# BraveGroup/DCD

Hardware: AMD Instinct MI355X
Metric: images/sec DGDE train step (bs=8, 384x1280) (higher is better)
Workload: dtype f32; 1 GPU; DGDE train bs=8 fp32 on 1xMI355X, synthetic KITTI 384x1280 + random kpts_ann (DGDE.yaml, DLA-34+DCNv2, 6 objects/image); global_batch=8, per_gpu_batch=8, input=384x1280, parallelism=dp1, dcn_precision=f32, step_launch=eager, sync_bn=False

## Files before the change

dcd_amd/_ext.py:

```python
import torch

from . import _lib

import threading

PRECISION = {"f32": 0, "bf16x3": 1, "bf16": 2}
_default_precision = "f32"
_scoped = threading.local()


def set_precision(name):
    global _default_precision
    if name not in PRECISION:
        raise ValueError("precision must be one of %s" % sorted(PRECISION))
    _default_precision = name


def get_precision():
    return getattr(_scoped, "name", None) or _default_precision


class precision_scope:

    def __init__(self, name):
        if name is not None and name not in PRECISION:
            raise ValueError("precision must be one of %s" % sorted(PRECISION))
        self.name = name

    def __enter__(self):
        self.saved = getattr(_scoped, "name", None)
        if self.name is not None:
            _scoped.name = self.name
        return self

    def __exit__(self, *exc):
        _scoped.name = self.saved
        return False


HANDOVER = {"never": 0, "always": 1, "auto": 2, None: -1}


def set_handover(mode):
    if mode not in HANDOVER:
        raise ValueError("handover mode must be one of 'never', 'always', 'auto', None")
    _lib.check(_lib.lib().dcd_dcn_v2_set_handover(HANDOVER[mode]), "dcd_dcn_v2_set_handover")


def _check(input, weight, bias, offset, mask, kernel_h, kernel_w):
    _lib.require_cuda(input, weight, bias, offset, mask)
    for name, t in (("input", input), ("weight", weight), ("bias", bias), ("offset", offset), ("mask", mask)):
        if t.dtype != torch.float32:
            raise RuntimeError("%s must be float32 (the op is fp32-only, like the reference)" % name)
    if input.dim() != 4 or weight.dim() != 4:
        raise RuntimeError("input and weight must be 4-D")
    if weight.shape[2] != kernel_h or weight.shape[3] != kernel_w:
        raise RuntimeError("Input shape and kernel shape wont match: (%d x %d vs %d x %d)." % (
            kernel_h, kernel_w, weight.shape[2], weight.shape[3]))
    if input.shape[1] != weight.shape[1]:
        raise RuntimeError("Input shape and kernel channels wont match: (%d vs %d)." % (input.shape[1], weight.shape[1]))
    if bias.numel() != weight.shape[0]:
        raise RuntimeError("bias must have Cout elements")


def _dims(input, weight, kernel_h, kernel_w, stride_h, stride_w, pad_h, pad_w, dilation_h, dilation_w):
    B, C, H, W = input.shape
    Ho = (H + 2 * pad_h - (dilation_h * (kernel_h - 1) + 1)) // stride_h + 1
    Wo = (W + 2 * pad_w - (dilation_w * (kernel_w - 1) + 1)) // stride_w + 1
    return B, C, H, W, weight.shape[0], Ho, Wo


def _workspace(L, input, geom):
    nbytes = L.dcd_dcn_v2_workspace_bytes(*geom)
    if nbytes == 0:
        raise RuntimeError("dcn_v2: unsupported geometry %s" % (geom,))
    return torch.empty(nbytes, dtype=torch.uint8, device=input.device), nbytes


def dcn_v2_forward(input, weight, bias, offset, mask, kernel_h, kernel_w, stride_h, stride_w,
                   pad_h, pad_w, dilation_h, dilation_w, deformable_group, precision=None):
    _check(input, weight, bias, offset, mask, kernel_h, kernel_w)
    L = _lib.lib()
    B, C, H, W, Co, Ho, Wo = _dims(input, weight, kernel_h, kernel_w, stride_h, stride_w, pad_h, pad_w,
                                   dilation_h, dilation_w)
    if tuple(offset.shape) != (B, 2 * deformable_group * kernel_h * kernel_w, Ho, Wo):
        raise RuntimeError("offset shape %s does not match (B, 2*dg*kh*kw, Ho, Wo)" % (tuple(offset.shape),))
    if tuple(mask.shape) != (B, deformable_group * kernel_h * kernel_w, Ho, Wo):
        raise RuntimeError("mask shape %s does not match (B, dg*kh*kw, Ho, Wo)" % (tuple(mask.shape),))
    input, weight, bias, offset, mask = (t.contiguous() for t in (input, weight, bias, offset, mask))
    geom = (B, C, H, W, Co, kernel_h, kernel_w, stride_h, stride_w, pad_h, pad_w, dilation_h, dilation_w,
            deformable_group)
    ws, nbytes = _workspace(L, input, geom)
    output = torch.empty((B, Co, Ho, Wo), dtype=torch.float32, device=input.device)
    prec = PRECISION[precision or get_precision()]
    st = L.dcd_dcn_v2_forward(_lib.stream_of(input), input.data_ptr(), weight.data_ptr(), bias.data_ptr(),
                              offset.data_ptr(), mask.data_ptr(), output.data_ptr(), *geom, prec,
                              ws.data_ptr(), nbytes)
    _lib.check(st, "dcd_dcn_v2_forward")
    return output


def dcn_v2_backward(input, weight, bias, offset, mask, grad_output, kernel_h, kernel_w, stride_h, stride_w,
                    pad_h, pad_w, dilation_h, dilation_w, deformable_group, precision=None):
    _check(input, weight, bias, offset, mask, kernel_h, kernel_w)
    _lib.require_cuda(grad_output)
    if not input.is_contiguous():
        raise RuntimeError("input tensor has to be contiguous")
    if not weight.is_contiguous():
        raise RuntimeError("weight tensor has to be contiguous")
    L = _lib.lib()
    B, C, H, W, Co, Ho, Wo = _dims(input, weight, kernel_h, kernel_w, stride_h, stride_w, pad_h, pad_w,
                                   dilation_h, dilation_w)
    if tuple(grad_output.shape) != (B, Co, Ho, Wo):
        raise RuntimeError("grad_output shape %s does not match the output" % (tuple(grad_output.shape),))
    if grad_output.dtype != torch.float32:
        raise RuntimeError("grad_output must be float32")
    bias, offset, mask, grad_output = (t.contiguous() for t in (bias, offset, mask, grad_output))
    geom = (B, C, H, W, Co, kernel_h, kernel_w, stride_h, stride_w, pad_h, pad_w, dilation_h, dilation_w,
            deformable_group)
    ws, nbytes = _workspace(L, input, geom)
    grad_input = torch.empty_like(input)
    grad_offset = torch.empty_like(offset)
    grad_mask = torch.empty_like(mask)
    grad_weight = torch.empty_like(weight)
    grad_bias = torch.empty_like(bias)
    prec = PRECISION[precision or get_precision()]
    st = L.dcd_dcn_v2_backward(_lib.stream_of(input), input.data_ptr(), weight.data_ptr(), bias.data_ptr(),
                               offset.data_ptr(), mask.data_ptr(), grad_output.data_ptr(),
                               grad_input.data_ptr(), grad_offset.data_ptr(), grad_mask.data_ptr(),
                               grad_weight.data_ptr(), grad_bias.data_ptr(), *geom, prec, ws.data_ptr(), nbytes)
    _lib.check(st, "dcd_dcn_v2_backward")
    return [grad_input, grad_offset, grad_mask, grad_weight, grad_bias]
```

dcd_amd/_lib.py:

```python
import ctypes
import os

_HERE = os.path.dirname(os.path.abspath(__file__))
LIB_PATH = os.path.join(_HERE, "libdcd_hip.so")
_LIB = None

c_void_p, c_int, c_float, c_size_t, c_int64, c_double = (ctypes.c_void_p, ctypes.c_int, ctypes.c_float,
                                                         ctypes.c_size_t, ctypes.c_int64, ctypes.c_double)


class LossRowsArgs(ctypes.Structure):
    _INTS = ("B", "M", "C", "K", "NP", "num_classes", "ch_box2d", "ch_offset", "ch_corner", "ch_corner_unc", "ch_dims",
             "ch_ori_cls", "ch_ori_off", "ch_depth", "ch_depth_unc", "ch_kpts2d", "ch_kpts3d", "trunc_log")
    _FLOATS = ("depth_lo", "depth_hi", "unc_lo", "unc_hi", "depth_weight")
    _POINTERS = ("pois", "reg_mask", "trunc_mask", "find_pcl", "ori_mask", "cls_ids", "centers", "pad_size", "bboxes",
                 "locations", "rotys", "offset_3D", "dimensions", "orientations", "keypoints", "kp_depth_mask", "kpts2d",
                 "kpts3d", "calib_P", "calib", "dim_mean", "kps_pred", "kps_tgt", "kps3d_pred", "kps3d_tgt", "rot", "P_rows",
                 "kmask", "pair_depth", "pair_mask", "cols", "corners_pred", "corners_tgt", "iou3d", "sums", "grad_sums",
                 "grad_pois", "grad_pair", "grad_kps", "grad_kps3d")
    _fields_ = ([(n, c_int) for n in _INTS] + [(n, c_float) for n in _FLOATS] + [("dim_weight", c_float * 3)]
                + [("down_ratio", c_float), ("kd_eps", c_float)] + [(n, c_void_p) for n in _POINTERS])

HEADS_MAX = 16


class HeadRowsArgs(ctypes.Structure):
    _fields_ = ([(n, c_int) for n in ("n_heads", "T", "R", "K", "C")]
                + [(n, c_int * HEADS_MAX) for n in ("trunk", "ch0", "out")]
                + [("weight", c_void_p * HEADS_MAX), ("bias", c_void_p * HEADS_MAX), ("feat", c_void_p), ("y", c_void_p),
                   ("grad_y", c_void_p), ("grad_feat", c_void_p), ("grad_weight", c_void_p * HEADS_MAX),
                   ("grad_bias", c_void_p * HEADS_MAX)])


class EvalMatchArgs(ctypes.Structure):
    _INTS = ("mode", "n_img", "n_comb", "n_rows", "G", "D", "n_dc", "max_dt", "T", "n_slots")
    _POINTERS = ("gt_off", "dt_off", "dc_off", "pair_off", "overlaps", "ign_gt", "ign_dt", "dt_score", "gt_alpha", "dt_alpha",
                 "dt_box2d", "dc_box", "comb", "min_overlap", "thresholds", "n_thresh", "scores", "counts", "sim_part")
    _fields_ = [(n, c_int) for n in _INTS] + [("P", c_int64)] + [(n, c_void_p) for n in _POINTERS]


DECODE_MAX_CLASSES = 8


class DecodeArgs(ctypes.Structure):
    _INTS = ("B", "K", "C", "nk", "n_bins", "num_classes", "ch_box2d", "ch_offset", "ch_corner", "ch_corner_unc", "ch_dims",
             "ch_ori_cls", "ch_ori_off", "ch_depth", "ch_depth_unc", "ch_kpts2d", "ch_kpts3d", "orientation", "dim_mode",
             "dim_std_on", "depth_mode", "uncertainty_as_conf", "records")
    _FLOATS = ("down_ratio", "depth_lo", "depth_hi", "eps")
    _fields_ = ([(n, c_int) for n in _INTS] + [(n, c_float) for n in _FLOATS] + [("depth_ref", c_float * 2)]
                + [("dim_mean", c_float * 3 * DECODE_MAX_CLASSES), ("dim_std", c_float * 3 * DECODE_MAX_CLASSES)])


class RecordsArgs(ctypes.Structure):
    _INTS = ("B", "M", "C", "nk", "n_bins", "ch_offset", "ch_ori_cls", "ch_ori_off", "ch_kpts2d", "ch_kpts3d")
    _fields_ = [(n, c_int) for n in _INTS] + [("down_ratio", c_float)]


SIGNATURES = {
    "dcd_version": (ctypes.c_char_p, []),
    "dcd_dcn_v2_workspace_bytes": (c_size_t, [c_int] * 14),
    "dcd_dcn_v2_forward": (c_int, [c_void_p] * 7 + [c_int] * 15 + [c_void_p, c_size_t]),
    "dcd_dcn_v2_backward": (c_int, [c_void_p] * 12 + [c_int] * 15 + [c_void_p, c_size_t]),
    "dcd_dcn_v2_forget": (c_int, [c_void_p]),
    "dcd_dcn_v2_policy_state": (c_int, [c_void_p, c_void_p]),
    "dcd_dcn_v2_policy_free": (c_int, []),
    "dcd_dcn_v2_set_handover": (c_int, [c_int]),
    "dcd_edge_depth_forward": (c_int, [c_void_p] * 6 + [c_int, c_int, c_int, c_float, c_float, c_int, c_int]
                               + [c_void_p] * 3),
    "dcd_edge_depth_backward": (c_int, [c_void_p] * 7 + [c_int, c_int, c_int, c_float, c_float, c_int]
                                + [c_void_p] * 2),
    "dcd_focal_loss": (c_int, [c_void_p, c_void_p, c_void_p, c_int64, c_float, c_float, c_void_p, c_void_p]),
    "dcd_giou_loss": (c_int, [c_void_p, c_void_p, c_void_p, c_int, c_void_p, c_void_p, c_void_p]),
    "dcd_nms_hm": (c_int, [c_void_p, c_void_p, c_int, c_int, c_int, c_int, c_void_p]),
    "dcd_heatmap_topk": (c_int, [c_void_p, c_void_p] + [c_int] * 6 + [c_void_p] * 5 + [c_void_p, c_size_t]),
    "dcd_heatmap_topk_workspace_bytes": (c_size_t, [c_int] * 5),
    "dcd_poi_gather": (c_int, [c_void_p, c_void_p, c_void_p] + [c_int] * 5 + [c_void_p]),
    "dcd_poi_scatter_add": (c_int, [c_void_p, c_void_p, c_void_p] + [c_int] * 5 + [c_void_p]),
    "dcd_patch_scatter_add": (c_int, [c_void_p, c_void_p, c_void_p, c_int, c_int, c_int64, c_int, c_int, c_void_p]),
    "dcd_iou3d": (c_int, [c_void_p, c_void_p, c_void_p, c_int, c_void_p]),
    "dcd_conv3x3_workspace_bytes": (c_size_t, [c_int] * 5),
    "dcd_conv3x3": (c_int, [c_void_p] * 6 + [c_int] * 6 + [c_void_p, c_size_t]),
    "dcd_conv3x3_weights_bytes": (c_size_t, [c_int] * 3),
    "dcd_conv3x3_transform_weights": (c_int, [c_void_p, c_void_p, c_int, c_int, c_void_p, c_void_p]),
    "dcd_conv3x3_transform_weights_table": (c_int, [c_void_p, c_void_p, c_int]),
    "dcd_conv3x3_prepared": (c_int, [c_void_p] * 6 + [c_int] * 6 + [c_void_p, c_size_t]),
    "dcd_conv3x3_split_weights_bytes": (c_size_t, [c_int] * 3),
    "dcd_conv3x3_split_transform_weights": (c_int, [c_void_p, c_void_p, c_int, c_int, c_void_p, c_void_p]),
    "dcd_conv3x3_split_transform_weights_table": (c_int, [c_void_p, c_void_p, c_int]),
    "dcd_conv3x3_split_workspace_bytes": (c_size_t, [c_int] * 5),
    "dcd_conv3x3_split_prepared": (c_int, [c_void_p] * 6 + [c_int] * 7 + [c_void_p, c_size_t]),
    "dcd_conv1x1_bf16": (c_int, [c_void_p, c_void_p, c_int, c_int, c_int, c_void_p, c_void_p, c_void_p, c_int, c_int, c_int64]),
    "dcd_conv1x1_wrw_bf16_workspace_bytes": (c_size_t, [c_int, c_int, c_int, c_int64]),
    "dcd_conv1x1_wrw_bf16": (c_int, [c_void_p, c_void_p, c_void_p, c_void_p, c_int, c_int, c_int, c_int, c_int64, c_void_p, c_size_t]),
    "dcd_conv3x3_s2_f32": (c_int, [c_void_p, c_void_p, c_void_p, c_void_p, c_int, c_int, c_int, c_int, c_int]),
    "dcd_conv3x3_s2_f32_backward_data": (c_int, [c_void_p, c_void_p, c_void_p, c_void_p, c_int, c_int, c_int, c_int, c_int]),
    "dcd_conv3x3_s2_f32_wrw_workspace_bytes": (c_size_t, [c_int, c_int, c_int, c_int, c_int]),
    "dcd_conv3x3_s2_f32_wrw": (c_int, [c_void_p, c_void_p, c_void_p, c_void_p, c_int, c_int, c_int, c_int, c_int, c_void_p, c_size_t]),
    "dcd_clip_adamw_workspace_bytes": (c_size_t, [c_int, c_void_p]),
    "dcd_clip_grad_norm_scalars": (c_int, [c_void_p, c_int, c_void_p, c_void_p, c_float, c_void_p, c_size_t, c_void_p]),
    "dcd_adamw_apply": (c_int, [c_void_p, c_int] + [c_void_p] * 7 + [c_double] * 4 + [c_void_p]),
    "dcd_conv1x1_f32": (c_int, [c_void_p, c_void_p, c_int, c_int, c_int, c_void_p, c_void_p, c_void_p, c_int, c_int, c_int64]),
    "dcd_conv1x1_wrw_f32_workspace_bytes": (c_size_t, [c_int, c_int, c_int, c_int64]),
    "dcd_conv1x1_wrw_f32": (c_int, [c_void_p, c_void_p, c_void_p, c_void_p, c_int, c_int, c_int, c_int, c_int64, c_void_p, c_size_t]),
    "dcd_conv3x3_bf16_weights_bytes": (c_size_t, [c_int] * 3),
    "dcd_conv3x3_bf16_transform_weights": (c_int, [c_void_p, c_void_p, c_int, c_int, c_void_p, c_void_p]),
    "dcd_conv3x3_bf16_transform_weights_table": (c_int, [c_void_p, c_void_p, c_int]),
    "dcd_conv3x3_bf16_workspace_bytes": (c_size_t, [c_int] * 5),
    "dcd_conv3x3_bf16_prepared": (c_int, [c_void_p] * 6 + [c_int] * 6 + [c_void_p, c_size_t]),
    "dcd_conv_stem_workspace_bytes": (c_size_t, [c_int] * 3),
    "dcd_conv_stem": (c_int, [c_void_p] * 4 + [c_int] * 7 + [c_void_p, c_size_t]),
    "dcd_conv_stem_wrw_workspace_bytes": (c_size_t, [c_int] * 3),
    "dcd_conv_stem_wrw": (c_int, [c_void_p] * 4 + [c_int] * 6 + [c_void_p, c_size_t]),
    "dcd_context_norm_forward": (c_int, [c_void_p] * 4 + [c_int, c_int, c_float]),
    "dcd_context_norm_backward": (c_int, [c_void_p] * 5 + [c_int, c_int]),
    "dcd_context_norm_relu_add_forward": (c_int, [c_void_p] * 4 + [c_int, c_int, c_float]),
    "dcd_gmw_refine": (c_int, [c_void_p] * 5 + [c_int, c_void_p, c_void_p, c_int, c_int, c_int] + [c_void_p] * 3),
    "dcd_gmw_pack_records": (c_int, [c_void_p] * 4 + [c_int, c_int, c_void_p, c_int, c_int, c_int] + [c_void_p] * 9),
    "dcd_sum_tensors": (c_int, [c_void_p, c_void_p, c_int, c_void_p, c_int64]),
    "dcd_conv3x3_wrw_workspace_bytes": (c_size_t, [c_int] * 5),
    "dcd_conv3x3_wrw": (c_int, [c_void_p] * 4 + [c_int] * 6 + [c_void_p, c_size_t]),
    "dcd_upsample_dw_forward": (c_int, [c_void_p] * 4 + [c_int] * 5),
    "dcd_upsample_dw_forward_add": (c_int, [c_void_p] * 5 + [c_int] * 5),
    "dcd_maxpool2x2_forward": (c_int, [c_void_p, c_void_p, c_void_p, c_int64, c_int, c_int]),
    "dcd_maxpool2x2_backward": (c_int, [c_void_p, c_void_p, c_void_p, c_void_p, c_int64, c_int, c_int]),
    "dcd_upsample_dw_backward": (c_int, [c_void_p] * 6 + [c_int] * 5),
    "dcd_bn_workspace_bytes": (c_size_t, [c_int]),
    "dcd_bn_stats": (c_int, [c_void_p, c_void_p, c_int, c_int, c_int64, c_void_p, c_void_p, c_size_t]),
    "dcd_channel_sums": (c_int, [c_void_p, c_void_p, c_int, c_int, c_int64, c_void_p, c_void_p, c_size_t]),
    "dcd_bn_train_apply": (c_int, [c_void_p] * 6 + [c_double] + [c_void_p] * 3 + [c_float, c_float, c_int] + [c_void_p] * 3
                           + [c_int, c_int, c_int64]),
    "dcd_bn_eval_apply": (c_int, [c_void_p] * 7 + [c_float, c_int, c_void_p, c_int, c_int, c_int64]),
    "dcd_bn_backward_stats": (c_int, [c_void_p] * 5 + [c_int, c_int, c_int64, c_void_p, c_void_p, c_size_t]),
    "dcd_trunk_row_sums": (c_int, [c_void_p, c_void_p, c_void_p, c_int, c_int, c_void_p]),
    "dcd_trunk_finalize_forward": (c_int, [c_void_p, c_void_p, c_void_p, c_void_p, c_double, c_double, c_int, c_void_p, c_void_p, c_void_p]),
    "dcd_trunk_finalize_backward": (c_int, [c_void_p, c_void_p, c_void_p, c_void_p, c_void_p, c_double, c_int, c_void_p, c_void_p, c_void_p]),
    "dcd_trunk_grad_wg": (c_int, [c_void_p, c_void_p, c_void_p, c_int, c_int, c_void_p]),
    "dcd_bn_backward_relu_from_x": (c_int, [c_void_p] * 10 + [c_int, c_int, c_int64, c_void_p, c_size_t]),
    "dcd_bn_backward_stats_params_relu_from_x": (c_int, [c_void_p] * 7 + [c_int, c_int, c_int64, c_void_p, c_void_p, c_void_p, c_void_p, c_size_t]),
    "dcd_bn_backward_apply_relu_from_x": (c_int, [c_void_p] * 8 + [c_double, c_void_p, c_int, c_int, c_int64]),
    "dcd_bn_backward_stats_params": (c_int, [c_void_p] * 6 + [c_int, c_int, c_int64, c_void_p, c_void_p, c_void_p, c_void_p, c_size_t]),
    "dcd_bn_backward_apply": (c_int, [c_void_p] * 8 + [c_double] + [c_void_p] * 4 + [c_int, c_int, c_int64]),
    "dcd_bn_at_forward": (c_int, [c_void_p] * 6 + [c_double] + [c_void_p] * 3 + [c_float, c_float, c_int] + [c_void_p] * 4
                          + [c_int, c_int, c_int64, c_int] + [c_void_p, c_size_t]),
    "dcd_bn_at_backward_sums": (c_int, [c_void_p] * 7 + [c_int, c_int, c_int] + [c_void_p, c_void_p]),
    "dcd_bn_train_forward": (c_int, [c_void_p] * 8 + [c_float, c_float, c_int] + [c_void_p] * 3 + [c_int, c_int, c_int64]
                             + [c_void_p, c_size_t]),
    "dcd_bn_backward": (c_int, [c_void_p] * 11 + [c_int, c_int, c_int64] + [c_void_p, c_size_t]),
    "dcd_dcn_offset_mask_split": (c_int, [c_void_p, c_void_p, c_void_p, c_void_p, c_int, c_int, c_int64]),
    "dcd_dcn_offset_mask_merge": (c_int, [c_void_p, c_void_p, c_void_p, c_void_p, c_void_p, c_int, c_int, c_int64]),
    "dcd_sgemm_shifted": (c_int, [c_void_p, c_void_p, c_int, c_int64, c_void_p, c_void_p, c_int64, c_int, c_void_p, c_void_p, c_int,
                                  c_int64, c_int64, c_int, c_int, c_int, c_int, c_int]),
    "dcd_sgemm": (c_int, [c_void_p, c_void_p, c_int, c_int64, c_int, c_void_p, c_int, c_int64, c_int, c_void_p, c_int, c_int64,
                          c_int, c_int, c_int, c_int, c_float, c_int, c_int]),
    "dcd_spd_solve_workspace_bytes": (c_size_t, [c_int, c_int]),
    "dcd_spd_solve": (c_int, [c_void_p, c_void_p, c_void_p, c_int, c_int, c_int, c_void_p, c_void_p, c_size_t]),
    "dcd_head_rows_forward": (c_int, [c_void_p, ctypes.POINTER(HeadRowsArgs)]),
    "dcd_head_rows_backward": (c_int, [c_void_p, ctypes.POINTER(HeadRowsArgs)]),
    "dcd_loss_rows_prepare": (c_int, [c_void_p, ctypes.POINTER(LossRowsArgs)]),
    "dcd_loss_rows_forward": (c_int, [c_void_p, ctypes.POINTER(LossRowsArgs)]),
    "dcd_loss_rows_backward": (c_int, [c_void_p, ctypes.POINTER(LossRowsArgs)]),
    "dcd_loss_rows_finish": (c_int, [c_void_p, ctypes.POINTER(LossRowsArgs)]),
    "dcd_encode_targets": (c_int, [c_void_p] * 6 + [c_int] * 6 + [c_double] * 3 + [c_int, c_int, c_void_p, c_int]),
    "dcd_preprocess_images": (c_int, [c_void_p, c_void_p, c_int64, c_void_p, c_void_p, c_int, c_int, c_int, c_int, c_void_p]),
    "dcd_eval_overlaps": (c_int, [c_void_p, c_int, c_void_p, c_void_p, c_void_p, c_int, c_int, c_int64] + [c_void_p] * 5),
    "dcd_eval_match": (c_int, [c_void_p, ctypes.POINTER(EvalMatchArgs)]),
    "dcd_eval_sum_similarity": (c_int, [c_void_p, c_void_p, c_int, c_int, c_void_p]),
    "dcd_gather_rows": (c_int, [c_void_p, c_int, c_void_p, c_void_p, c_void_p, c_void_p, c_void_p, c_int]),
    "dcd_sinkhorn_workspace_bytes": (c_size_t, [c_int, c_int, c_int]),
    "dcd_sinkhorn": (c_int, [c_void_p] * 5 + [c_int, c_int, c_int, c_float, c_float, c_float, c_int, c_void_p, c_void_p, c_size_t]),
    "dcd_decode_detections": (c_int, [c_void_p] * 7 + [ctypes.POINTER(DecodeArgs)] + [c_void_p] * 4),
    "dcd_gmw_train_records_workspace_bytes": (c_size_t, [c_int] * 3),
    "dcd_gmw_train_records": (c_int, [c_void_p, c_void_p, ctypes.POINTER(RecordsArgs)] + [c_void_p] * 9 + [c_int] + [c_void_p] * 8
                              + [c_int, c_int, c_void_p, c_size_t]),
    "dcd_depth_estimates": (c_int, [c_void_p] * 8 + [ctypes.POINTER(DecodeArgs), c_void_p]),
    "dcd_depth_accumulate": (c_int, [c_void_p, c_void_p, c_int, ctypes.POINTER(c_float), c_int, c_int, c_void_p, c_void_p]),
    "dcd_dis_iou_estimates": (c_int, [c_void_p] * 9 + [ctypes.POINTER(DecodeArgs), c_void_p, c_void_p]),
    "dcd_dis_iou_accumulate": (c_int, [c_void_p, c_void_p, c_int, ctypes.POINTER(c_float), c_int, c_int, ctypes.POINTER(c_double),
                               c_void_p, c_void_p]),
    "dcd_nms_detections": (c_int, [c_void_p] * 5 + [c_int] * 4 + [c_double, c_double, c_int] + [c_void_p] * 5),
    "dcd_tta_merge_detections": (c_int, [c_void_p] * 6 + [c_int] * 4 + [c_double] * 3 + [c_void_p] * 7),
    "dcd_render_slots": (c_int, [c_int] * 3),
    "dcd_render_detections": (c_int, [c_void_p, c_void_p, c_size_t] + [c_void_p] * 8 + [c_int] * 6 + [c_double, c_double]
                              + [c_void_p] * 4),
    "dcd_render_primitives": (c_int, [c_void_p, c_void_p, c_size_t, c_void_p, c_void_p] + [c_int] * 4 + [c_void_p]),
}

STATUS = {1: "bad argument", 2: "workspace too small", 3: "kernel launch failed"}


class DcdHipError(RuntimeError):
    pass


def lib():
    global _LIB
    if _LIB is None:
        if not os.path.exists(LIB_PATH):
            raise DcdHipError(
                "libdcd_hip.so is not built (%s missing). The DGDE hot path has no CPU fallback; "
                "build it with `make -C dcd_amd/csrc` or `__graft_entry__.build()`." % LIB_PATH)
        import torch
        handle = ctypes.CDLL(LIB_PATH)
        for name, (res, args) in SIGNATURES.items():
            fn = getattr(handle, name)
            fn.restype = res
            fn.argtypes = args
        _LIB = handle
    return _LIB


def check(status, what):
    if status != 0:
        raise DcdHipError("%s failed: %s (status %d)" % (what, STATUS.get(status, "unknown"), status))


def ptr(t):
    return None if t is None else t.data_ptr()


def stream_of(t):
    import torch
    return torch._C._cuda_getCurrentRawStream(t.device.index)


def require_cuda(*tensors):
    for t in tensors:
        if t is not None and not t.is_cuda:
            raise DcdHipError("dcd_amd ops run on the GPU only (got a %s tensor); there is no CPU path" % t.device)
```

dcd_amd/csrc/dcn_bwd_sweep.inc:

```

#ifndef SW_ABL_TAPS
#define SW_ABL_TAPS 9
#endif
#ifdef SW_ABL_NOMFMA
__device__ __forceinline__ f32x4 sw_fake_mfma(float a, float b, f32x4 c) { c.x = fmaf(a, b, c.x); c.y += a; c.z += b; c.w = fmaf(a, b, c.w); return c; }
#define SW_MFMA(a, b, c) sw_fake_mfma(a, b, c)
#else
#define SW_MFMA(a, b, c) __builtin_amdgcn_mfma_f32_16x16x4f32(a, b, c, 0, 0, 0)
#endif
constexpr int SW_PX = 16;
constexpr int SW_WW = 24;
constexpr int SW_RING = 9;
constexpr int SW_CH = 16;
constexpr int SW_CELLS = SW_RING * SW_WW;
constexpr int SW_PLANE = SW_CELLS + 3;
constexpr int SW_ZERO = SW_CELLS;
constexpr int SW_W_FLOATS = 9 * 16 * 64;
constexpr int SW_DW_FLOATS = 9 * 64 * SW_CH;
constexpr int SW_PART_FLOATS = SW_DW_FLOATS + 64;

__device__ __forceinline__ void sweep_prep_weights_body(const float *__restrict__ w, float *__restrict__ wp, const Geom &g, int nck, int nob,
                                                        int bid, int nb)
{
    const int n = nck * SW_W_FLOATS * nob;
// ... 560 lines not shown
            }
            __builtin_amdgcn_sched_barrier(0);
            cp_store(16, sw_reduce4(Ph_p, bit0, bit1));
            cp_store(17, sw_reduce4(Pw_p, bit0, bit1));
            cp_store(26, sw_reduce4(Pm_p, bit0, bit1));
        }
        auto add_dw = [&](int t, const float (&colv)[4]) {
            const f32x4 colv4 = {colv[0], colv[1], colv[2], colv[3]};
            const f32x4 cs = ONE ? sw_round4(colv4) : (SPLIT ? sw_split4(colv4) : f32x4{0.f, 0.f, 0.f, 0.f});
#define SW_FIX_CASE(TT)                                                                                                 \
    case TT:                                                                                                            \
        if (SPLIT) {                                                                                                    \
            _Pragma("unroll") for (int ob = 0; ob < 4; ++ob) accw[TT][ob] = sw_dw_split<ONE>(dyo[ob], cs, accw[TT][ob]); \
        } else {                                                                                                        \
            _Pragma("unroll") for (int r = 0; r < 4; ++r) _Pragma("unroll") for (int ob = 0; ob < 4; ++ob)              \
                accw[TT][ob] = __builtin_amdgcn_mfma_f32_16x16x4f32(dyo[ob][r], colv[r], accw[TT][ob], 0, 0, 0);         \
        }                                                                                                               \
        break;
            switch (t) {
                SW_FIX_CASE(0) SW_FIX_CASE(1) SW_FIX_CASE(2) SW_FIX_CASE(3) SW_FIX_CASE(4) SW_FIX_CASE(5) SW_FIX_CASE(6) SW_FIX_CASE(7)
                SW_FIX_CASE(8)
            }
#undef SW_FIX_CASE
        };
        auto full_dcol = [&](int t) {
            float wt[NS];
            load_w(t, wt);
            f32x4 d4 = {0.f, 0.f, 0.f, 0.f};
            if (TWO) {
                f32x4 d4b = {0.f, 0.f, 0.f, 0.f};
                dcol_part2(d4, d4b, dyp, wt, -1);
                d4 += d4b;
            } else {
                d4 = dcol_part(d4, dyp, wt, -1);
            }
            return d4;
        };
        unsigned tapwork = 0u;
#pragma unroll
        for (int t = 0; t < 9; ++t) {
            const unsigned w_ = ((unsigned)(cmask >> (4 * t)) & 15u) | ((unsigned)(fm[t >> 2] >> (16 * (t & 3))) & 0xffffu);
            tapwork |= (w_ != 0u ? 1u : 0u) << t;
        }
#ifdef SW_ABL_NOAFTER
        tapwork = 0u;
#endif
#pragma unroll 1
        for (unsigned tw = tapwork; tw != 0u; tw &= tw - 1u) {
            const int t = __builtin_ctz(tw);
            const unsigned f4 = (unsigned)(cmask >> (4 * t)) & 15u;
            const unsigned pm16 = (unsigned)(fm[t >> 2] >> (16 * (t & 3))) & 0xffffu;
            const unsigned farq = (pm16 >> (4 * q)) & 15u;
            const f32x4 d4 = full_dcol(t);
            float Pm[4], Ph[4], Pw[4], colv[4];
            char *const dummy = lane_plane + SW_ZERO * 8;
            const bool odd = q & 1;
#pragma unroll
            for (int r = 0; r < 4; ++r) {
                Pm[r] = 0.f; Ph[r] = 0.f; Pw[r] = 0.f; colv[r] = 0.f;
                if ((f4 >> r) & 1u) {
                    const f32x4 e = *reinterpret_cast<const f32x4 *>(stt2 + (t * 16 + 4 * q + r) * 4);
                    const bool isf = (farq >> r) & 1u;
                    const unsigned pp = isf ? ((unsigned)(SW_ZERO * 8) | ((unsigned)(SW_ZERO * 8) << 16)) : __float_as_uint(e.x);
                    const float lh = isf ? 0.f : e.y, lw = isf ? 0.f : e.z, m = isf ? 0.f : e.w;
                    char *const pT = lane_plane + (pp & 0xffffu), *const pB = lane_plane + (pp >> 16);
                    const float v1 = reinterpret_cast<const float *>(pT)[0], v2 = reinterpret_cast<const float *>(pT)[2];
                    const float v3 = reinterpret_cast<const float *>(pB)[0], v4 = reinterpret_cast<const float *>(pB)[2];
                    const float d = d4[r], hh = 1.f - lh, hw = 1.f - lw, dm = d * m;
                    const float ex = v2 - v1, fx = v4 - v3, ay = v3 - v1, by = v4 - v2;
                    const float top = v1 + lw * ex, bot = v3 + lw * fx;
                    const float val = top + lh * (bot - top);
                    Pm[r] = d * val;
                    Ph[r] = dm * (hw * ay + lw * by);
                    Pw[r] = dm * (hh * ex + lh * fx);
                    colv[r] = m * val;
                    const float w1 = dm * (hh * hw), w2 = dm * (hh * lw), w3 = dm * (lh * hw), w4 = dm * (lh * lw);
                    {
                        const float g1 = reinterpret_cast<const float *>(pT)[1], g2 = reinterpret_cast<const float *>(pT)[3];
                        const float g3 = reinterpret_cast<const float *>(pB)[1], g4 = reinterpret_cast<const float *>(pB)[3];
                        char *const aT = odd ? dummy : pT, *const aB = odd ? dummy : pB;
                        reinterpret_cast<float *>(aT)[1] = g1 + w1;
                        reinterpret_cast<float *>(aT)[3] = g2 + w2;
                        reinterpret_cast<float *>(aB)[1] = g3 + w3;
                        reinterpret_cast<float *>(aB)[3] = g4 + w4;
                    }
                    __builtin_amdgcn_wave_barrier();
                    {
                        const float g1 = reinterpret_cast<const float *>(pT)[1], g2 = reinterpret_cast<const float *>(pT)[3];
                        const float g3 = reinterpret_cast<const float *>(pB)[1], g4 = reinterpret_cast<const float *>(pB)[3];
                        char *const cT = odd ? pT : dummy, *const cB = odd ? pB : dummy;
                        reinterpret_cast<float *>(cT)[1] = g1 + w1;
                        reinterpret_cast<float *>(cT)[3] = g2 + w2;
                        reinterpret_cast<float *>(cB)[1] = g3 + w3;
                        reinterpret_cast<float *>(cB)[3] = g4 + w4;
                    }
                    __builtin_amdgcn_wave_barrier();
                }
            }
            if (pm16 != 0u) {
                float cv[4][4], lhv[4], lwv[4], mv[4];
                int gofs[4];
                bool ok[4][4];
#pragma unroll
                for (int r = 0; r < 4; ++r) {
                    const f32x4 e = *reinterpret_cast<const f32x4 *>(stt2 + (t * 16 + 4 * q + r) * 4);
                    const bool isf = ((farq >> r) & 1u) && j < cleft;
                    const unsigned pp = __float_as_uint(e.x);
                    const int yl = (int)(pp & 0xffffu) - 1, xl = (int)(pp >> 16) - 1;
                    lhv[r] = isf ? e.y : 0.f; lwv[r] = isf ? e.z : 0.f; mv[r] = isf ? e.w : 0.f;
                    ok[r][0] = isf && yl >= 0 && xl >= 0;
                    ok[r][1] = isf && yl >= 0 && xl + 1 < W;
                    ok[r][2] = isf && yl + 1 < H && xl >= 0;
                    ok[r][3] = isf && yl + 1 < H && xl + 1 < W;
                    gofs[r] = (j * HW + yl * W + xl) * 4;
                    constexpr int DO[4] = {0, 1, 0, 1};
#pragma unroll
                    for (int c_ = 0; c_ < 4; ++c_)
                        cv[r][c_] = __builtin_bit_cast(float, __builtin_amdgcn_raw_buffer_load_b32(
                                                                  r_in, ok[r][c_] ? gofs[r] + (DO[c_] + (c_ >> 1) * W) * 4 : SW_OOB, 0, 0));
                }
#pragma unroll
                for (int r = 0; r < 4; ++r) {
                    const float v1 = cv[r][0], v2 = cv[r][1], v3 = cv[r][2], v4 = cv[r][3];
                    const float lh = lhv[r], lw = lwv[r], m = mv[r];
                    const float d = d4[r], hh = 1.f - lh, hw = 1.f - lw, dm = d * m;
                    const float ex = v2 - v1, fx = v4 - v3, ay = v3 - v1, by = v4 - v2;
                    const float top = v1 + lw * ex, bot = v3 + lw * fx;
                    const float val = top + lh * (bot - top);
                    Pm[r] += d * val;
                    Ph[r] += dm * (hw * ay + lw * by);
                    Pw[r] += dm * (hh * ex + lh * fx);
                    float *gp = reinterpret_cast<float *>(reinterpret_cast<char *>(gin_c) + gofs[r]);
                    if (ok[r][0]) atomicAdd(gp, dm * (hh * hw));
                    if (ok[r][1]) atomicAdd(gp + 1, dm * (hh * lw));
                    if (ok[r][2]) atomicAdd(gp + W, dm * (lh * hw));
                    if (ok[r][3]) atomicAdd(gp + W + 1, dm * (lh * lw));
                    colv[r] += m * val;
                }
            }
            const unsigned redo = f4 | farq;
            const int cpx = (j < 4 && ((redo >> (j & 3)) & 1u) && x0 + 4 * q + j < W) ? (x0 + 4 * q + j) * 4 : SW_OOB;
            auto cpx_store = [&](int plane, float v) {
                __builtin_amdgcn_raw_buffer_store_b32(__builtin_bit_cast(unsigned, v), r_cp, cpx, (plane * HW + y * W) * 4, 0);
            };
            cpx_store(2 * t, sw_reduce4(Ph, bit0, bit1));
            cpx_store(2 * t + 1, sw_reduce4(Pw, bit0, bit1));
            cpx_store(18 + t, sw_reduce4(Pm, bit0, bit1));
            if (!DWK) {
#pragma unroll
                for (int r = 0; r < 4; ++r)
                    __builtin_amdgcn_raw_buffer_store_b32(__builtin_bit_cast(unsigned, colv[r]), r_col,
                                                          (q4v && ((redo >> r) & 1u)) ? (j * 9 * HW + x0 + 4 * q + r) * 4 : SW_OOB,
                                                          (t * HW + y * W) * 4, 0);
            } else {
                add_dw(t, colv);
            }
        }
        if (DWK && !SPLIT) {
#pragma unroll
            for (int ob = 0; ob < 4; ++ob) dyo_p3[ob] = dyo[ob][3];
        }

        SW_STAMP(prof_slot + 12);
        {
            const int yy = y - 4;
            float *gbase = gin_c + (yy * W + x0 - 4);
#pragma unroll
            for (int k = 0; k < 6; ++k) {
                const int e = lane + 64 * k;
                const int ch = e / SW_WW, col = e - ch * SW_WW;
                float *cell = ring + (ch * SW_PLANE + s0 * SW_WW + col) * 2 + 1;
                const float gv = *cell;
                *cell = 0.f;
                const int xx = x0 - 4 + col;
#ifndef SW_ABL_NOFLUSH
                if (gv != 0.f && ch < cleft && yy >= 0 && xx >= 0 && xx < W)
                    atomicAdd(reinterpret_cast<float *>(reinterpret_cast<char *>(gbase) + (unsigned)(ch * HW + col) * 4u), gv);
#endif
            }
            row_store(s0, rx);
        }
        SW_STAMP(prof_slot + 13);
        s0 = s0 + 1 == SW_RING ? 0 : s0 + 1;
#pragma unroll
        for (int s = 0; s < NS; ++s) dyp[s] = dyp_n[s];
        if (DWK) {
            if (ck == 0) {
#pragma unroll
                for (int ob = 0; ob < 4; ++ob) bsum[ob] += (dyo_n[ob].x + dyo_n[ob].y) + (dyo_n[ob].z + dyo_n[ob].w);
            }
#pragma unroll
            for (int ob = 0; ob < 4; ++ob) dyo[ob] = ONE ? sw_round4(dyo_n[ob]) : (SPLIT ? sw_split4(dyo_n[ob]) : dyo_n[ob]);
        }
        raw = raw_n;
    }

    for (int i = 0; i < SW_RING - 1; ++i) {
        const int yy = y1 - 4 + i;
        int sl = s0 + i;
        sl = sl >= SW_RING ? sl - SW_RING : sl;
        for (int k = 0; k < 6; ++k) {
            const int e = lane + 64 * k;
            const int ch = e / SW_WW, col = e - ch * SW_WW;
            const float gv = ring[(ch * SW_PLANE + sl * SW_WW + col) * 2 + 1];
            const int xx = x0 - 4 + col;
            if (gv != 0.f && ch < cleft && yy >= 0 && yy < H && xx >= 0 && xx < W) atomicAdd(gin_c + (size_t)ch * HW + yy * W + xx, gv);
        }
    }

    if (DWK && !SPLIT) {
#pragma unroll
        for (int ob = 0; ob < 4; ++ob)
            accw[8][ob] = __builtin_amdgcn_mfma_f32_16x16x4f32(dyo_p3[ob], pend_col, accw[8][ob], 0, 0, 0);
    }
    }

    if (DWK) {
        float *dst = a.dwpart + ((size_t)ck * (a.nslot / a.nck) + (id0 / (8 * a.nck)) * 8 + (id0 & 7)) * SW_PART_FLOATS;
#pragma unroll
        for (int t = 0; t < 9; ++t)
#pragma unroll
            for (int ob = 0; ob < 4; ++ob)
#pragma unroll
                for (int i = 0; i < 4; ++i) dst[(t * 64 + 16 * ob + 4 * q + i) * SW_CH + j] = accw[t][ob][i];
#pragma unroll
        for (int ob = 0; ob < 4; ++ob) {
            float v_ = bsum[ob];
            v_ += __shfl_xor(v_, 16);
            v_ += __shfl_xor(v_, 32);
            if (q == 0) dst[SW_DW_FLOATS + 16 * ob + j] = v_;
        }
    }
}

__device__ __forceinline__ void sweep_reduce_coord_body(const float *__restrict__ cpart, float *__restrict__ goff,
                                                        float *__restrict__ gmsk, int B, int HW, int nck,
                                                        const unsigned *__restrict__ far_scal, int total_tiles, int bid, int nb)
{
    const bool zero = far_dominated(far_scal, total_tiles);
    const int64_t n4 = (int64_t)B * 27 * HW / 4, per_b4 = (int64_t)27 * HW / 4, off4 = (int64_t)18 * HW / 4;
    const size_t stride4 = (size_t)B * 27 * HW / 4;
    for (int64_t i = (int64_t)bid * blockDim.x + threadIdx.x; i < n4; i += (int64_t)nb * blockDim.x) {
        f32x4 s = {0.f, 0.f, 0.f, 0.f};
        if (!zero) s = reinterpret_cast<const f32x4 *>(cpart)[i];
        for (int ck = 1; ck < nck && !zero; ++ck) {
            const f32x4 v = reinterpret_cast<const f32x4 *>(cpart)[i + ck * stride4];
            s.x += v.x; s.y += v.y; s.z += v.z; s.w += v.w;
        }
        const int64_t b = i / per_b4, r = i - b * per_b4;
        if (r < off4) reinterpret_cast<f32x4 *>(goff)[b * off4 + r] = s;
        else reinterpret_cast<f32x4 *>(gmsk)[b * (per_b4 - off4) + (r - off4)] = s;
    }
}

__device__ __forceinline__ void sweep_reduce_dw_body(const float *__restrict__ part, float *__restrict__ gw, float *__restrict__ gbias,
                                                     const Geom &g, int nck, int nvp, const unsigned *__restrict__ far_scal,
                                                     int total_tiles, int bx, int nbx, int by, int nby)
{
    if (far_dominated(far_scal, total_tiles)) return;
    const int n = nck * SW_DW_FLOATS + 64;
    const int v0 = (int)((int64_t)by * nvp / nby), v1 = (int)((int64_t)(by + 1) * nvp / nby);
    for (int idx = bx * blockDim.x + threadIdx.x; idx < n; idx += nbx * blockDim.x) {
        const bool is_bias = idx >= nck * SW_DW_FLOATS;
        const int ck = is_bias ? 0 : idx / SW_DW_FLOATS, e = is_bias ? SW_DW_FLOATS + (idx - nck * SW_DW_FLOATS) : idx - ck * SW_DW_FLOATS;
        const int c = e & 15, o = is_bias ? e - SW_DW_FLOATS : (e >> 4) & 63, t = e >> 10;
        const int cc = ck * SW_CH + c;
        if (o >= g.Co || (!is_bias && cc >= g.C)) continue;
        const float *src = part + (size_t)ck * nvp * SW_PART_FLOATS + e;
        float s = 0.f;
#pragma unroll 8
        for (int vv = v0; vv < v1; ++vv) s += src[(size_t)vv * SW_PART_FLOATS];
        if (is_bias) atomicAdd(gbias + o, s);
        else atomicAdd(gw + ((size_t)o * g.C + cc) * 9 + t, s);
    }
}

__device__ __forceinline__ void sweep_reduce_gemm_body(const float *__restrict__ part, float *__restrict__ gw, int n, int S,
                                                       const unsigned *__restrict__ far_scal, int total_tiles, int bid, int nb)
{
    if (far_dominated(far_scal, total_tiles)) return;
    for (int i = (bid * blockDim.x + threadIdx.x) * 4; i < n; i += nb * blockDim.x * 4) {
        if (i + 3 < n) {
            f32x4 acc = {0.f, 0.f, 0.f, 0.f};
            for (int s = 0; s < S; ++s) acc += *reinterpret_cast<const f32x4 *>(part + (size_t)s * n + i);
            *reinterpret_cast<f32x4 *>(gw + i) = acc;
        } else {
            for (int j = 0; i + j < n; ++j) {
                float a = 0.f;
                for (int s = 0; s < S; ++s) a += part[(size_t)s * n + i + j];
                gw[i + j] = a;
            }
        }
    }
}

struct SweepEpilogueArgs {
    const float *cpart, *gy, *dwpart;
    float *goff, *gmsk, *gw, *gbias;
    const unsigned *far_scal, *bias_only_if_far;
    Geom g;
    int nck, nvp, total_tiles, nb_coord, bias_splits, dw_bx, dw_by, gemm_n, gemm_S;
    unsigned *far_report = nullptr;
    unsigned far_base = 0;
};
__global__ __launch_bounds__(256) void dcn_sweep_epilogue(SweepEpilogueArgs a)
{
    int bid = blockIdx.x;
    if (a.far_report && bid == 0 && threadIdx.x == 0) {
        const unsigned c = a.far_scal[3] & ~FAR_BY_COUNT;
        *a.far_report = c >= a.far_base ? c - a.far_base : 0u;
    }
    if (bid < a.nb_coord) {
        sweep_reduce_coord_body(a.cpart, a.goff, a.gmsk, a.g.B, a.g.HoWo, a.nck, a.far_scal, a.total_tiles, bid, a.nb_coord);
        return;
    }
    bid -= a.nb_coord;
    const int nb_bias = a.g.Co * a.bias_splits;
    if (bid < nb_bias) {
        bias_grad_body(a.gy, a.gbias, a.g.B, a.g.Co, a.g.HoWo, a.bias_only_if_far, bid % a.g.Co, bid / a.g.Co, a.bias_splits);
        return;
    }
    bid -= nb_bias;
    if (a.dw_by > 0)
        sweep_reduce_dw_body(a.dwpart, a.gw, a.gbias, a.g, a.nck, a.nvp, a.far_scal, a.total_tiles, bid % a.dw_bx, a.dw_bx, bid / a.dw_bx, a.dw_by);
    else
        sweep_reduce_gemm_body(a.dwpart, a.gw, a.gemm_n, a.gemm_S, a.far_scal, a.total_tiles, bid, (int)gridDim.x - a.nb_coord - nb_bias);
}

struct SweepPlan {
    int nck, nstrip, nseg, seg_rows, nv;
    int nslot;
    int nob;
    int dw_split, dw_kchunk;
    size_t wp_floats, cpart_floats, dw_floats, col_floats;
};
constexpr int SW_GEMM_T = 128, SW_GEMM_K = 16;

__host__ inline SweepPlan sweep_plan(const Geom &g)
{
    SweepPlan p;
    p.nck = (g.C + SW_CH - 1) / SW_CH;
    p.nstrip = (g.W + SW_PX - 1) / SW_PX;
    const int64_t base = (int64_t)g.B * p.nstrip * p.nck;
    static const int min_rows = dcd_env("DCD_SWEEP_MIN_ROWS") && atoi(dcd_env("DCD_SWEEP_MIN_ROWS")) > 0 ? atoi(dcd_env("DCD_SWEEP_MIN_ROWS")) : 3;
    int best = 1;
    int64_t best_cost = -1;
    for (int ns = 1; ns <= g.H; ++ns) {
        const int rows = (g.H + ns - 1) / ns;
        if (rows < min_rows && ns > 1) break;
        const int real_ns = (g.H + rows - 1) / rows;
        const int64_t total = base * real_ns;
        const int64_t cost = ((total + 1023) / 1024) * (rows + 5);
        if (best_cost < 0 || cost < best_cost) { best_cost = cost; best = real_ns; }
    }
    p.seg_rows = (g.H + best - 1) / best;
    p.nseg = (g.H + p.seg_rows - 1) / p.seg_rows;
    p.nv = g.B * p.nstrip * p.nseg;
    const int64_t units = (int64_t)((p.nv + 7) / 8) * 8 * p.nck;
    const int grp = 8 * p.nck;
    int64_t slots = units < 1024 ? units : (1024 / grp) * (int64_t)grp;
    if (slots < grp) slots = grp;
    if (const char *e = dcd_env("DCD_SWEEP_SLOTS")) {
        const int64_t v_ = atoll(e);
        slots = v_ <= 0 ? units : (v_ / grp > 0 ? v_ / grp : 1) * grp;
    }
    if (slots > units) slots = units;
    p.nslot = (int)slots;
    p.nob = g.Co <= 64 ? 1 : (g.Co <= 128 ? 2 : 4);
    p.wp_floats = (size_t)p.nck * SW_W_FLOATS * p.nob;
    p.cpart_floats = (size_t)p.nck * g.B * 27 * g.HoWo;
    p.dw_split = 1;
    p.dw_kchunk = 0;
    if (p.nob == 1) {
        p.dw_floats = (size_t)p.nslot * SW_PART_FLOATS;
        p.col_floats = 0;
    } else {
        const int K9 = g.C * 9;
        const int tiles = ((g.Co + SW_GEMM_T - 1) / SW_GEMM_T) * ((K9 + SW_GEMM_T - 1) / SW_GEMM_T) * g.B;
        int sp = (512 + tiles - 1) / tiles;
        const int smax = g.HoWo / 256 > 1 ? g.HoWo / 256 : 1;
        if (sp > smax) sp = smax;
        if (sp < 1) sp = 1;
        p.dw_kchunk = ((g.HoWo + sp - 1) / sp + SW_GEMM_K - 1) / SW_GEMM_K * SW_GEMM_K;
        p.dw_split = (g.HoWo + p.dw_kchunk - 1) / p.dw_kchunk;
        p.col_floats = (size_t)g.B * K9 * g.HoWo;
        p.dw_floats = (size_t)g.B * p.dw_split * g.Co * K9;
    }
    return p;
}

__host__ inline int sweep_mode()
{
    const char *e = dcd_env("DCD_BWD_SWEEP");
    return !e ? 1 : (atoi(e) == 0 ? 0 : (atoi(e) == 2 ? 2 : 1));
}

__host__ inline bool sweep_ok(const Geom &g)
{
    return sweep_mode() != 0 && g.kh == 3 && g.kw == 3 && g.sh == 1 && g.sw == 1 && g.ph == 1 && g.pw == 1 && g.dh == 1 && g.dw == 1 && g.dg == 1 &&
           (g.W & 3) == 0 && g.H >= 8 && g.W >= 32 && g.Co <= 256 && ((int64_t)g.HoWo * 27 & 3) == 0 &&
           (g.Co <= 64 || (((int64_t)g.C * 9 * g.HoWo < (1ll << 29)) && (int64_t)g.B * g.C * 9 * g.HoWo * 4 <= (1ll << 31)));
}

__host__ inline size_t sweep_workspace_bytes(const Geom &g)
{
    if (!sweep_ok(g)) return 0;
    const SweepPlan p = sweep_plan(g);
    return ((p.wp_floats + p.cpart_floats + p.dw_floats + p.col_floats) * sizeof(float) + 255) / 256 * 256 + 256;
}
```

dcd_amd/csrc/dcn_v2.hip:

```cpp

#include <hip/hip_runtime.h>
#include <stdint.h>
#include <stdlib.h>
#include <string.h>
#include <atomic>
#include <map>
#include <vector>
#include <mutex>
#include <utility>

#include "../../include/dcd_hip.h"
#include "tuning_env.h"
#include "lds_limit.h"

typedef float f32x16 __attribute__((ext_vector_type(16)));
typedef float f32x32 __attribute__((ext_vector_type(32)));

namespace {

template <int N> struct IntC {
    static constexpr int value = N;
};

struct Geom {
// ... 97 lines not shown
    s.w4 = s.c4 ? s.lh * s.lw : 0.f;
    s.m = sv ? m : 0.f;
    s.oh = oh;
    s.ow = ow;
    {
        const int xb = g.W >= 2 ? min(max(wl, 0), g.W - 2) : 0;
        const int ya = min(max(hl, 0), g.H - 1), yb = min(max(hh_i, 0), g.H - 1);
        const int shift = xb - wl;
        s.pt = ya * g.W + xb;
        s.pb = yb * g.W + xb;
        s.shift = shift;
        s.a0 = shift == 0 ? s.w1 : (shift == 1 ? s.w2 : 0.f);
        s.a1 = shift == 0 ? s.w2 : (shift == -1 ? s.w1 : 0.f);
        s.b0 = shift == 0 ? s.w3 : (shift == 1 ? s.w4 : 0.f);
        s.b1 = shift == 0 ? s.w4 : (shift == -1 ? s.w3 : 0.f);
        if (!sv) { s.pt = 0; s.pb = 0; }
    }
    return s;
}

__device__ __forceinline__ Tap make_tap(const float *__restrict__ off_b, const float *__restrict__ msk_b, const Geom &g,
                                        int seg, int t, int ho, int wo, int Pc, bool pv)
{
    return finish_tap(load_tap_raw(off_b, msk_b, g, seg, Pc), g, t, ho, wo, pv);
}

__device__ __forceinline__ void xcd_remap(int &bx, int &by)
{
    const int gx = gridDim.x, NT = gx * gridDim.y;
    const int L = bx + gx * by;
    const int xc = L & 7, slot = L >> 3;
    const int q = NT >> 3, r = NT & 7;
    const int Lp = (xc < r ? xc * (q + 1) : r * (q + 1) + (xc - r) * q) + slot;
    by = Lp / gx;
    bx = Lp - by * gx;
}

__device__ __forceinline__ float ldg(const float *base, unsigned byte_off)
{
    return *(const float *)((const char *)base + byte_off);
}

typedef float f32x2 __attribute__((ext_vector_type(2)));
__device__ __forceinline__ f32x2 ldg2(const float *base, unsigned byte_off)
{
    typedef f32x2 __attribute__((aligned(4))) f32x2_u;
    return *(const f32x2_u *)((const char *)base + byte_off);
}

template <int MB>
__global__ __launch_bounds__(256) void dcn_fwd_f32(const float *__restrict__ in, const float *__restrict__ off,
                                                   const float *__restrict__ msk, const float *__restrict__ wf,
                                                   const float *__restrict__ bias, float *__restrict__ out, Geom g)
{
    const int lane = threadIdx.x & 63, wave = threadIdx.x >> 6;
    const int p = lane & 31, h = lane >> 5;
    int bx = blockIdx.x, b = blockIdx.y;
    xcd_remap(bx, b);
    const int tile = bx * 4 + wave;
    if (tile * 32 >= g.HoWo) return;
    const int ob0 = blockIdx.z * MB;
    const int P = tile * 32 + p;
    const bool pv = P < g.HoWo;
    const int Pc = pv ? P : g.HoWo - 1;
    const int ho = Pc / g.Wo, wo = Pc - ho * g.Wo;
    const unsigned HW4 = (unsigned)(g.H * g.W) * 4u;
    const unsigned Cop4 = (unsigned)g.Cop * 4u;

    f32x16 acc[MB];
#pragma unroll
    for (int mb = 0; mb < MB; ++mb)
#pragma unroll
        for (int r = 0; r < 16; ++r) acc[mb][r] = 0.f;

    const float *in_b = in + (size_t)b * g.C * g.H * g.W;
    const float *off_b = off + (size_t)b * g.dg * 2 * g.KK * g.HoWo;
    const float *msk_b = msk + (size_t)b * g.dg * g.KK * g.HoWo;
    const int npair = g.cpg >> 1;
    const unsigned wlane = ((unsigned)h * (unsigned)g.Cop + (unsigned)(ob0 * 32 + p)) * 4u;

    for (int seg = 0; seg < g.dg * g.KK; ++seg) {
        const int grp = seg / g.KK, t = seg - grp * g.KK;
        const Tap s = make_tap(off_b, msk_b, g, seg, t, ho, wo, Pc, pv);
        const float *ip = in_b + (size_t)grp * g.cpg * g.H * g.W;
        const float *wp = wf + (size_t)seg * g.cpgp * g.Cop;
        const unsigned o1 = (unsigned)s.i1 * 4u + h * HW4, o2 = (unsigned)s.i2 * 4u + h * HW4;
        const unsigned o3 = (unsigned)s.i3 * 4u + h * HW4, o4 = (unsigned)s.i4 * 4u + h * HW4;
        const unsigned opt = (unsigned)s.pt * 4u + h * HW4, opb = (unsigned)s.pb * 4u + h * HW4;
        const bool pairs = g.W >= 2;
        const float q1 = pairs ? s.a0 : s.w1, q2 = pairs ? s.a1 : s.w2, q3 = pairs ? s.b0 : s.w3, q4 = pairs ? s.b1 : s.w4;
#ifndef DCN_FWD_UN
#define DCN_FWD_UN ((MB >= 4) ? 2 : 4)
#endif
        constexpr int UN = DCN_FWD_UN;
        float va[UN][4], vb[UN][4], wa[UN][MB], wb_[UN][MB];
        auto issue = [&](float (&v)[UN][4], float (&a)[UN][MB], int it0) {
#pragma unroll
            for (int u = 0; u < UN; ++u) {
                const float *ipc = (const float *)((const char *)ip + (size_t)(it0 + u) * 2 * HW4);
                const float *wpc = (const float *)((const char *)wp + (size_t)(it0 + u) * 2 * Cop4);
#ifdef DCN_ABL_NOGATHER
                v[u][0] = s.w1 + (float)u; v[u][1] = s.w2; v[u][2] = s.w3; v[u][3] = s.w4; (void)ipc;
#else
                if (pairs) {
                    const f32x2 tp = ldg2(ipc, opt), bt = ldg2(ipc, opb);
                    v[u][0] = tp.x; v[u][1] = tp.y; v[u][2] = bt.x; v[u][3] = bt.y;
                } else {
                    v[u][0] = ldg(ipc, o1); v[u][1] = ldg(ipc, o2); v[u][2] = ldg(ipc, o3); v[u][3] = ldg(ipc, o4);
                }
#endif
#pragma unroll
                for (int mb = 0; mb < MB; ++mb)
#ifdef DCN_ABL_NOWEIGHT
                    a[u][mb] = s.w1 + (float)(mb + u); (void)wpc;
#else
                    a[u][mb] = ldg(wpc, wlane + mb * 128u);
#endif
            }
        };
        auto compute = [&](float (&v)[UN][4], float (&a)[UN][MB]) {
#pragma unroll
            for (int u = 0; u < UN; ++u) {
                const float val = (q1 * v[u][0] + q2 * v[u][1] + q3 * v[u][2] + q4 * v[u][3]) * s.m;
#pragma unroll
                for (int mb = 0; mb < MB; ++mb) acc[mb] = __builtin_amdgcn_mfma_f32_32x32x2f32(a[u][mb], val, acc[mb], 0, 0, 0);
            }
        };
        const int nfull = npair / UN;
        int gq = 0;
        if (nfull > 0) issue(va, wa, 0);
        for (; gq + 1 < nfull; gq += 2) {
            issue(vb, wb_, (gq + 1) * UN);
            compute(va, wa);
            if (gq + 2 < nfull) issue(va, wa, (gq + 2) * UN);
            compute(vb, wb_);
        }
        if (gq < nfull) compute(va, wa);
        for (int it = nfull * UN; it < npair; ++it) {
            const float *ipc = (const float *)((const char *)ip + (size_t)it * 2 * HW4);
            const float *wpc = (const float *)((const char *)wp + (size_t)it * 2 * Cop4);
            const float v1 = ldg(ipc, o1), v2 = ldg(ipc, o2), v3 = ldg(ipc, o3), v4 = ldg(ipc, o4);
            const float val = (s.w1 * v1 + s.w2 * v2 + s.w3 * v3 + s.w4 * v4) * s.m;
#pragma unroll
            for (int mb = 0; mb < MB; ++mb)
                acc[mb] = __builtin_amdgcn_mfma_f32_32x32x2f32(ldg(wpc, wlane + mb * 128u), val, acc[mb], 0, 0, 0);
        }
        ip = (const float *)((const char *)ip + (size_t)npair * 2 * HW4);
        wp = (const float *)((const char *)wp + (size_t)npair * 2 * Cop4);
        if (g.cpg & 1) {
            const float v1 = ldg(ip, (unsigned)s.i1 * 4u), v2 = ldg(ip, (unsigned)s.i2 * 4u);
            const float v3 = ldg(ip, (unsigned)s.i3 * 4u), v4 = ldg(ip, (unsigned)s.i4 * 4u);
            float val = (s.w1 * v1 + s.w2 * v2 + s.w3 * v3 + s.w4 * v4) * s.m;
            val = h ? 0.f : val;
#pragma unroll
            for (int mb = 0; mb < MB; ++mb)
                acc[mb] = __builtin_amdgcn_mfma_f32_32x32x2f32(ldg(wp, wlane + mb * 128u), val, acc[mb], 0, 0, 0);
        }
    }

    float *out_b = out + (size_t)b * g.Co * g.HoWo;
#pragma unroll
    for (int mb = 0; mb < MB; ++mb) {
        const int obase = (ob0 + mb) * 32 + 4 * h;
#pragma unroll
        for (int r = 0; r < 16; ++r) {
            const int o = obase + (r & 3) + 8 * (r >> 2);
            if (pv && o < g.Co) out_b[(size_t)o * g.HoWo + P] = acc[mb][r] + bias[o];
        }
    }
}

constexpr int TL_WW = 40;
constexpr int TL_CH = 8;
constexpr int TL_OB = 64;
constexpr int TL_W_FLOATS = 9 * TL_OB * TL_CH;
constexpr int TL_NW = TL_W_FLOATS / 4;
template <int TR> struct TileCfg {
    static constexpr int WH = TR + 8;
    static constexpr int PLANE = (WH * TL_WW) % 64 == 32 ? WH * TL_WW : WH * TL_WW + 32;
    static constexpr int IN_FLOATS = TL_CH * PLANE;
    static constexpr int BUF = IN_FLOATS + TL_W_FLOATS;
    static constexpr int NIN = TL_CH * WH * (TL_WW / 4);
    static constexpr int NT = TR * 64;
    static constexpr int KIN = (NIN + NT - 1) / NT, KW = (TL_NW + NT - 1) / NT;
};


__global__ void dcn_prep_weights9(const float *__restrict__ w, float *__restrict__ wf9, Geom g)
{
    const int K = g.C * 9, n = K * g.Cop;
    for (int idx = blockIdx.x * blockDim.x + threadIdx.x; idx < n; idx += gridDim.x * blockDim.x) {
        const int k = idx / g.Cop, o = idx - k * g.Cop;
        wf9[idx] = (o < g.Co) ? w[(size_t)o * K + k] : 0.f;
    }
}

template <int MB, bool RESCUE = false>
__global__ __launch_bounds__(256) void dcn_fwd9_f32(const float *__restrict__ in, const float *__restrict__ off,
                                                    const float *__restrict__ msk, const float *__restrict__ wf9,
                                                    const float *__restrict__ bias, float *__restrict__ out, Geom g,
                                                    const unsigned char *__restrict__ rescue_flags = nullptr, int tiles_x = 0,
                                                    int rows_per_region = 0, int nchunk = 0)
{
    const int lane = threadIdx.x & 63, wave = threadIdx.x >> 6;
    const int p = lane & 31, h = lane >> 5;
    int bx = blockIdx.x, b = blockIdx.y;
    xcd_remap(bx, b);
    const int tile = bx * 4 + wave;
    const int ob0 = blockIdx.z * MB;
    int P, ho, wo;
    bool pv;
    if (RESCUE) {
        const int row = tile / tiles_x, cseg = tile - row * tiles_x;
        if (row >= g.Ho) return;
        const int regions_y = (g.Ho + rows_per_region - 1) / rows_per_region;
        if (!rescue_flags[((size_t)b * regions_y + row / rows_per_region) * tiles_x + cseg]) return;
        ho = row;
        wo = cseg * 32 + p;
        pv = wo < g.Wo;
        if (!pv) wo = g.Wo - 1;
        P = ho * g.Wo + wo;
    } else {
        if (tile * 32 >= g.HoWo) return;
        P = tile * 32 + p;
        pv = P < g.HoWo;
        if (!pv) P = g.HoWo - 1;
        ho = P / g.Wo;
        wo = P - ho * g.Wo;
    }
    const int Pc = P;
    const unsigned HW4 = (unsigned)(g.H * g.W) * 4u;
    const unsigned Cop4 = (unsigned)g.Cop * 4u;

    f32x16 acc[MB];
#pragma unroll
    for (int mb = 0; mb < MB; ++mb)
#pragma unroll
        for (int r = 0; r < 16; ++r) acc[mb][r] = 0.f;

    const float *in_b = in + (size_t)b * g.C * g.H * g.W;
    const float *off_b = off + (size_t)b * g.dg * 18 * g.HoWo;
    const float *msk_b = msk + (size_t)b * g.dg * 9 * g.HoWo;
    const unsigned wlane = (unsigned)(ob0 * 32 + p) * 4u;
    const int npair = g.cpg >> 1;

    for (int grp = 0; grp < g.dg; ++grp) {
        unsigned to[9][2];
        float tw[9][4];
#pragma unroll
        for (int t = 0; t < 9; ++t) {
            const Tap s = make_tap(off_b, msk_b, g, grp * 9 + t, t, ho, wo, Pc, pv);
            to[t][0] = (unsigned)s.pt * 4u; to[t][1] = (unsigned)s.pb * 4u;
            tw[t][0] = s.a0 * s.m; tw[t][1] = s.a1 * s.m; tw[t][2] = s.b0 * s.m; tw[t][3] = s.b1 * s.m;
        }
        const float *ip = in_b + ((size_t)grp * g.cpg + h) * g.H * g.W;
        const float *wp = wf9 + ((size_t)grp * g.cpg + h) * 9 * g.Cop;
        auto pair_step = [&](const float *ipc, const float *wpc, bool live) {
#pragma unroll
            for (int t0 = 0; t0 < 9; t0 += 3) {
                f32x2 vt[3], vb[3];
                float a[3][MB];
#pragma unroll
                for (int u = 0; u < 3; ++u) {
                    vt[u] = ldg2(ipc, to[t0 + u][0]);
                    vb[u] = ldg2(ipc, to[t0 + u][1]);
#pragma unroll
                    for (int mb = 0; mb < MB; ++mb) a[u][mb] = ldg(wpc, wlane + (unsigned)(t0 + u) * Cop4 + mb * 128u);
                }
#pragma unroll
                for (int u = 0; u < 3; ++u) {
                    float val = tw[t0 + u][0] * vt[u].x + tw[t0 + u][1] * vt[u].y + tw[t0 + u][2] * vb[u].x + tw[t0 + u][3] * vb[u].y;
                    val = live ? val : 0.f;
#pragma unroll
                    for (int mb = 0; mb < MB; ++mb)
                        acc[mb] = __builtin_amdgcn_mfma_f32_32x32x2f32(a[u][mb], val, acc[mb], 0, 0, 0);
                }
            }
        };
        for (int it = 0; it < npair; ++it)
            pair_step((const float *)((const char *)ip + (size_t)it * 2 * HW4),
                      (const float *)((const char *)wp + (size_t)it * 18 * Cop4), true);
        if (g.cpg & 1) {
            const size_t back = h ? (size_t)g.H * g.W : 0;
            const size_t wback = h ? (size_t)9 * g.Cop : 0;
            pair_step((const float *)((const char *)ip + (size_t)npair * 2 * HW4) - back,
                      (const float *)((const char *)wp + (size_t)npair * 18 * Cop4) - wback, h == 0);
        }
    }

    float *out_b = out + (size_t)b * g.Co * g.HoWo;
#pragma unroll
    for (int mb = 0; mb < MB; ++mb) {
        const int obase = (ob0 + mb) * 32 + 4 * h;
#pragma unroll
        for (int r = 0; r < 16; ++r) {
            const int o = obase + (r & 3) + 8 * (r >> 2);
            if (pv && o < g.Co) out_b[(size_t)o * g.HoWo + Pc] = acc[mb][r] + bias[o];
        }
    }
}

typedef float f32x4 __attribute__((ext_vector_type(4)));

__global__ void dcn_prep_weights_tile(const float *__restrict__ w, float *__restrict__ wl, Geom g, int nchunk, int nz,
                                      unsigned *__restrict__ flags, int nflag_words, float *__restrict__ wf9)
{
    for (int i = blockIdx.x * blockDim.x + threadIdx.x; i < nflag_words; i += gridDim.x * blockDim.x) flags[i] = 0u;
    if (wf9) {
        const int K = g.C * 9, n9 = K * g.Cop;
        for (int idx = blockIdx.x * blockDim.x + threadIdx.x; idx < n9; idx += gridDim.x * blockDim.x) {
            const int k = idx / g.Cop, o = idx - k * g.Cop;
            wf9[idx] = (o < g.Co) ? w[(size_t)o * K + k] : 0.f;
        }
    }
    const int n = nz * nchunk * TL_W_FLOATS;
    for (int idx = blockIdx.x * blockDim.x + threadIdx.x; idx < n; idx += gridDim.x * blockDim.x) {
        int r = idx;
        const int s = r & 3; r >>= 2;
        const int h = r & 1; r >>= 1;
        const int o = r % TL_OB; r /= TL_OB;
        const int t = r % 9; r /= 9;
        const int ck = r % nchunk, z = r / nchunk;
        const int oo = z * TL_OB + o, c = ck * TL_CH + 2 * s + h;
        wl[idx] = (oo < g.Co && c < g.C) ? w[((size_t)oo * g.C + c) * 9 + t] : 0.f;
    }
}

constexpr float TL_NEAR_F = 3.f;
__global__ __launch_bounds__(256) void dcn_fwd_far_count(const float *__restrict__ off, int64_t n, unsigned *__restrict__ counter)
{
    unsigned c = 0;
    const int64_t n4 = ((uintptr_t)off & 15) == 0 ? n >> 2 : 0;
    for (int64_t i = (int64_t)blockIdx.x * blockDim.x + threadIdx.x; i < n4; i += (int64_t)gridDim.x * blockDim.x) {
        const f32x4 v = *reinterpret_cast<const f32x4 *>(off + 4 * i);
        c += (!(fabsf(v.x) < TL_NEAR_F)) + (!(fabsf(v.y) < TL_NEAR_F)) + (!(fabsf(v.z) < TL_NEAR_F)) + (!(fabsf(v.w) < TL_NEAR_F));
    }
    for (int64_t i = 4 * n4 + (int64_t)blockIdx.x * blockDim.x + threadIdx.x; i < n; i += (int64_t)gridDim.x * blockDim.x)
        c += !(fabsf(off[i]) < TL_NEAR_F);
#pragma unroll
    for (int o = 32; o > 0; o >>= 1) c += __shfl_xor(c, o);
    __shared__ unsigned part[4];
    if ((threadIdx.x & 63) == 0) part[threadIdx.x >> 6] = c;
    __syncthreads();
    if (threadIdx.x == 0 && part[0] + part[1] + part[2] + part[3]) atomicAdd(counter, part[0] + part[1] + part[2] + part[3]);
}

template <int TR>
__global__ __launch_bounds__(TR * 64) void dcn_fwd_tile_f32(const float *__restrict__ in, const float *__restrict__ off,
                                                        const float *__restrict__ msk, const float *__restrict__ wl,
                                                        const float *__restrict__ bias, float *__restrict__ out, Geom g,
                                                        int tiles_x, int nchunk, unsigned char *__restrict__ rescue_flags,
                                                        const float *__restrict__ wf9, int rescue_taps,
                                                        const unsigned *__restrict__ far_count, unsigned far_limit)
{
    typedef TileCfg<TR> T;
    constexpr int TL_ROWS = TR, TL_WH = T::WH, TL_PLANE = T::PLANE, TL_IN_FLOATS = T::IN_FLOATS, TL_BUF = T::BUF,
                  TL_NIN = T::NIN, NT = T::NT, KIN = T::KIN, KW = T::KW;
    extern __shared__ __attribute__((aligned(16))) float lds[];
    const int tid = threadIdx.x;
    const int lane = tid & 63, wave = tid >> 6;
    const int p = lane & 31, h = lane >> 5;
    int bx = blockIdx.x, b = blockIdx.y;
    xcd_remap(bx, b);
    if (*far_count > far_limit) {
        if (tid == 0) rescue_flags[(size_t)b * gridDim.x + bx] = 1;
        return;
    }
    const int ty = bx / tiles_x, tx = bx - ty * tiles_x;
    const int r0 = ty * TL_ROWS, c0 = tx * 32;
    const int ho = r0 + wave, wo = c0 + p;
    const bool pv = ho < g.Ho && wo < g.Wo;
    const int Pc = pv ? ho * g.Wo + wo : 0;
    const int z = blockIdx.z;
    const int HW = g.H * g.W;
    const int Y0 = r0 - 4, X0 = c0 - 4;

    const float *in_b = in + (size_t)b * g.C * HW;
    const float *off_b = off + (size_t)b * 18 * g.HoWo;
    const float *msk_b = msk + (size_t)b * 9 * g.HoWo;
    const float *wl_z = wl + (size_t)z * nchunk * TL_W_FLOATS;

    int sg[KIN], sl[KIN];
    bool sv_[KIN];
#pragma unroll
    for (int k = 0; k < KIN; ++k) {
        const int e = tid + NT * k;
        const int ch = e / (TL_WH * 10), rem = e - ch * (TL_WH * 10);
        const int row = rem / 10, q = rem - row * 10;
        const int y = Y0 + row, x = X0 + 4 * q;
        sv_[k] = e < TL_NIN;
        sg[k] = (sv_[k] && y >= 0 && y < g.H && x >= 0 && x < g.W) ? ch * HW + y * g.W + x : -1;
        sl[k] = ch * TL_PLANE + row * TL_WW + 4 * q;
    }
    f32x4 rin[KIN];
    auto issue_w = [&](int ck, float *buf) {
        const float *src = wl_z + (size_t)ck * TL_W_FLOATS + 4 * tid;
        float *dst = buf + TL_IN_FLOATS + 4 * 64 * __builtin_amdgcn_readfirstlane(wave);
#pragma unroll
        for (int k = 0; k < KW; ++k)
            if (64 * __builtin_amdgcn_readfirstlane(wave) + NT * k < TL_NW)
                __builtin_amdgcn_global_load_lds(src + 4 * NT * k, (__attribute__((address_space(3))) void *)(dst + 4 * NT * k), 16, 0, 0);
    };
    auto issue = [&](int ck) {
        const float *src = in_b + (size_t)ck * TL_CH * HW;
        const int cleft = g.C - ck * TL_CH;
#pragma unroll
        for (int k = 0; k < KIN; ++k) {
            const f32x4 zero4 = {0.f, 0.f, 0.f, 0.f};
            rin[k] = zero4;
            if (sv_[k] && sg[k] >= 0 && (tid + NT * k) / (TL_WH * 10) < cleft) rin[k] = *reinterpret_cast<const f32x4 *>(src + sg[k]);
        }
    };
    auto commit = [&](float *buf) {
#pragma unroll
        for (int k = 0; k < KIN; ++k)
            if (sv_[k]) *reinterpret_cast<f32x4 *>(buf + sl[k]) = rin[k];
    };

    issue(0);

    int lo[9];
    float wq[9][4];
    unsigned farbits = 0;
#pragma unroll
    for (int t = 0; t < 9; ++t) {
        const TapRaw raw = load_tap_raw(off_b, msk_b, g, t, Pc);
        const float hf = (float)(ho - 1 + t / 3) + raw.oh, wf_ = (float)(wo - 1 + t % 3) + raw.ow;
        const bool sv = pv && hf > -1.f && wf_ > -1.f && hf < (float)g.H && wf_ < (float)g.W;
        const float hlf = floorf(hf), wlf = floorf(wf_);
        const int ly = sv ? (int)hlf - Y0 : 0, lx = sv ? (int)wlf - X0 : 0;
        const bool inside = ly >= 0 && lx >= 0 && ly <= TL_WH - 2 && lx <= TL_WW - 2;
        farbits |= (sv && !inside) ? (1u << t) : 0u;
        lo[t] = (inside ? ly * TL_WW + lx : 0) + h * TL_PLANE;
        const float lh = hf - hlf, lw = wf_ - wlf;
        const float m = (sv && inside) ? raw.m : 0.f;
        wq[t][0] = (1.f - lh) * (1.f - lw) * m; wq[t][1] = (1.f - lh) * lw * m;
        wq[t][2] = lh * (1.f - lw) * m;         wq[t][3] = lh * lw * m;
    }

    f32x16 acc[2];
#pragma unroll
    for (int mb = 0; mb < 2; ++mb)
#pragma unroll
        for (int r = 0; r < 16; ++r) acc[mb][r] = 0.f;

    int wave_far_taps = 0;
#pragma unroll
    for (int t = 0; t < 9; ++t) wave_far_taps += __any((farbits >> t) & 1u) ? 1 : 0;
    __shared__ int far_worst;
    if (tid == 0) far_worst = 0;
    __syncthreads();
    if (lane == 0) atomicMax(&far_worst, wave_far_taps);
    __syncthreads();
    if (far_worst >= rescue_taps) {
        if (tid == 0) rescue_flags[(size_t)b * gridDim.x + bx] = 1;
        return;
    }

    issue_w(0, lds);
    commit(lds);
    asm volatile("s_waitcnt vmcnt(0)" ::: "memory");
    __syncthreads();

    for (int ck = 0; ck < nchunk; ++ck) {
        const float *buf = lds + (ck & 1) * TL_BUF;
#ifndef TL_ABL_NOSTAGE
        if (ck + 1 < nchunk) {
            issue_w(ck + 1, lds + ((ck + 1) & 1) * TL_BUF);
            issue(ck + 1);
        }
#endif
        const float *wb_ = buf + TL_IN_FLOATS + (p * 2 + h) * 4;
#pragma unroll
        for (int t = 0; t < 9; ++t) {
#ifdef TL_ABL_NOW
            const f32x4 a0 = {wq[t][0], wq[t][1], wq[t][2], wq[t][3]}, a1 = {wq[t][1], wq[t][0], wq[t][3], wq[t][2]};
            (void)wb_;
#else
            const f32x4 a0 = *reinterpret_cast<const f32x4 *>(wb_ + (t * TL_OB) * 8);
            const f32x4 a1 = *reinterpret_cast<const f32x4 *>(wb_ + (t * TL_OB + 32) * 8);
#endif
            const float *cp = buf + lo[t];
            const float q0 = wq[t][0], q1 = wq[t][1], q2 = wq[t][2], q3 = wq[t][3];
#pragma unroll
            for (int s = 0; s < 4; ++s) {
                const float *c2 = cp + 2 * s * TL_PLANE;
#ifdef TL_ABL_NOLDS
                const float val = q0 * (float)s + q1 + q2 * (float)ck + q3;
                (void)c2;
#else
                const float val = q0 * c2[0] + q1 * c2[1] + q2 * c2[TL_WW] + q3 * c2[TL_WW + 1];
#endif
                acc[0] = __builtin_amdgcn_mfma_f32_32x32x2f32(a0[s], val, acc[0], 0, 0, 0);
                acc[1] = __builtin_amdgcn_mfma_f32_32x32x2f32(a1[s], val, acc[1], 0, 0, 0);
            }
        }
#ifndef TL_ABL_NOSTAGE
        if (ck + 1 < nchunk) commit(lds + ((ck + 1) & 1) * TL_BUF);
#endif
        asm volatile("s_waitcnt vmcnt(0)" ::: "memory");
#ifndef TL_ABL_NOBAR
        __syncthreads();
#endif
    }

    if (__any(farbits != 0u)) {
#pragma unroll 1
        for (int t = 0; t < 9; ++t) {
            if (!__any((farbits >> t) & 1u)) continue;
            const bool mine = (farbits >> t) & 1u;
            const Tap s = make_tap(off_b, msk_b, g, t, t, ho, wo, Pc, pv);
            const float *w9 = wf9 + (size_t)t * g.Cop + z * TL_OB + p;
            const bool second = z * TL_OB + 32 < g.Cop;
            const int cend = (g.C + 1) & ~1;
            for (int c0 = h; c0 < cend; c0 += 8) {
                f32x2 gt[4], gb[4];
                float wa[4], wb2[4];
#pragma unroll
                for (int u = 0; u < 4; ++u) {
                    const int c = c0 + 2 * u;
                    const int cc = c < g.C ? c : g.C - 1;
                    const float *gp = in_b + (size_t)cc * HW;
                    gt[u] = ldg2(gp, (unsigned)s.pt * 4u);
                    gb[u] = ldg2(gp, (unsigned)s.pb * 4u);
                    const float *wr = w9 + (size_t)cc * 9 * g.Cop;
                    wa[u] = wr[0];
                    wb2[u] = second ? wr[32] : 0.f;
                }
#pragma unroll
                for (int u = 0; u < 4; ++u) {
                    const int c = c0 + 2 * u;
                    const bool live = mine && c < g.C;
                    const float val = live ? (s.a0 * gt[u].x + s.a1 * gt[u].y + s.b0 * gb[u].x + s.b1 * gb[u].y) * s.m : 0.f;
                    acc[0] = __builtin_amdgcn_mfma_f32_32x32x2f32(wa[u], val, acc[0], 0, 0, 0);
                    acc[1] = __builtin_amdgcn_mfma_f32_32x32x2f32(wb2[u], val, acc[1], 0, 0, 0);
                }
            }
        }
    }

    float *out_b = out + (size_t)b * g.Co * g.HoWo;
#pragma unroll
    for (int mb = 0; mb < 2; ++mb) {
        const int obase = z * TL_OB + mb * 32 + 4 * h;
#pragma unroll
        for (int r = 0; r < 16; ++r) {
            const int o = obase + (r & 3) + 8 * (r >> 2);
            if (pv && o < g.Co) out_b[(size_t)o * g.HoWo + ho * g.Wo + wo] = acc[mb][r] + bias[o];
        }
    }
}

constexpr float TL_NEAR = 3.f;
constexpr unsigned FAR_BY_COUNT = 0x80000000u;
constexpr unsigned FAR_COUNT_PIVOT = 0x40000000u;
__device__ __forceinline__ bool far_dominated(const unsigned *far_scal, int total_tiles)
{
    if (!far_scal) return false;
    const unsigned c = far_scal[3];
    if (c & FAR_BY_COUNT) return (c & ~FAR_BY_COUNT) > FAR_COUNT_PIVOT;
    return (int64_t)far_scal[1] * 2 > (int64_t)total_tiles;
}

inline unsigned far_count_limit(const Geom &g, bool wide)
{
    static const int div = dcd_env("DCD_FAR_DIV") ? atoi(dcd_env("DCD_FAR_DIV")) : 0;
    static const int div_wide = dcd_env("DCD_FAR_DIV_WIDE") ? atoi(dcd_env("DCD_FAR_DIV_WIDE")) : 0;
    int d = wide ? div_wide : div;
    if (d <= 0) d = wide ? (g.B >= 4 ? 16 : 8) : (g.B >= 4 ? 24 : 12);
    const int64_t total = (int64_t)g.B * 18 * g.HoWo;
    int64_t lim = total / d;
    if (lim > (int64_t)FAR_COUNT_PIVOT - 1) lim = FAR_COUNT_PIVOT - 1;
    return (unsigned)lim;
}

struct HandoverState {
    unsigned *host = nullptr;
    unsigned *dev = nullptr;
};
static std::mutex g_handover_mu;
static std::map<std::pair<int, const void *>, HandoverState> g_handover;
static std::map<int, std::vector<HandoverState>> g_handover_free;
constexpr unsigned HANDOVER_UNKNOWN = 0xffffffffu;

static std::atomic<int> g_handover_pin{-1};
static int handover_mode()
{
    const int pin = g_handover_pin.load(std::memory_order_relaxed);
    if (pin >= 0) return pin;
    static const int m = [] {
        const char *e = dcd_env("DCD_DCN_HANDOVER");
        if (e && !strcmp(e, "always")) return 1;
        if (e && !strcmp(e, "never")) return 0;
        return 2;
    }();
    return m;
}

static bool stream_is_capturing(hipStream_t stream)
{
    hipStreamCaptureStatus st = hipStreamCaptureStatusNone;
    return hipStreamIsCapturing(stream, &st) == hipSuccess && st != hipStreamCaptureStatusNone;
}

static int handover_decide(hipStream_t stream, const void *weight, unsigned real_limit, unsigned **report)
{
    *report = nullptr;
    const int mode = handover_mode();
    if (mode != 2) return mode;
    int dev = 0;
    (void)hipGetDevice(&dev);
    std::lock_guard<std::mutex> lock(g_handover_mu);
    HandoverState &h = g_handover[std::make_pair(dev, weight)];
    if (!h.host) {
        std::vector<HandoverState> &fl = g_handover_free[dev];
        if (!fl.empty()) {
            h = fl.back();
            fl.pop_back();
            *report = h.dev;
            return 1;
        }
        if (stream_is_capturing(stream)) return 1;
        unsigned *hp = nullptr, *dp = nullptr;
        if (hipHostMalloc((void **)&hp, sizeof(unsigned), hipHostMallocMapped) != hipSuccess ||
            hipHostGetDevicePointer((void **)&dp, hp, 0) != hipSuccess) {
            (void)hipGetLastError();
            if (hp) (void)hipHostFree(hp);
            return 1;
// ... 962 lines not shown
        stage_gather(t0, stage_raw(t0));
        act_cur = act_next;
        if (t0 + 1 < t1) raw_next = stage_raw(t0 + 1);
    }
    for (int ti = t0; ti < t1; ++ti) {
        const bool act = act_cur;
        any_act |= act;
        if (act)
#pragma unroll
        for (int q = 0; q < 16; ++q) {
            const int row = 2 * q + h;
            const bool pr = g.W >= 2;
            const float val = ((pr ? s.a0 : s.w1) * v[q][0] + (pr ? s.a1 : s.w2) * v[q][1] + (pr ? s.b0 : s.w3) * v[q][2] +
                               (pr ? s.b1 : s.w4) * v[q][3]) * s.m;
            myT[row * 33 + p] = (blk * 32 + row < g.cpg) ? val : 0.f;
        }
#pragma unroll
        for (int q = 0; q < MB * 4; ++q) dyT[(q * 8 + wave * 2 + h) * 33 + p] = dyr[q];
        __syncthreads();
        if (ti + 1 < t1) {
            const TapRaw raw = raw_next;
            if (ti + 2 < t1) raw_next = stage_raw(ti + 2);
            stage_gather(ti + 1, raw);
            act_cur = act_next;
        }
#ifdef DW_ABL_NOMFMA
        if (ti < 0)
#endif
        if (act)
#pragma unroll 4
        for (int k = 0; k < 16; ++k) {
            const float a = myT[p * 33 + 2 * k + h];
#pragma unroll
            for (int mb = 0; mb < MB; ++mb)
                acc[mb] = __builtin_amdgcn_mfma_f32_32x32x2f32(a, dyT[(mb * 32 + p) * 33 + 2 * k + h], acc[mb], 0, 0, 0);
        }
        __syncthreads();
    }

#pragma unroll
    for (int mb = 0; mb < MB; ++mb) {
        __syncthreads();
#pragma unroll
        for (int r = 0; r < 16; ++r) myT[((r & 3) + 8 * (r >> 2) + 4 * h) * 33 + p] = acc[mb][r];
        __syncthreads();
        const int cc = blk * 32 + p;
#pragma unroll 4
        for (int it = 0; it < 16; ++it) {
            const int ol = 2 * it + h;
            const int o = (ob0 + mb) * 32 + ol;
            if (any_act && rbv && o < g.Co && cc < g.cpg)
                atomicAdd(gw + ((size_t)o * g.C + grp * g.cpg + cc) * g.KK + t, myT[p * 33 + ol]);
        }
    }
}

constexpr int DW_TR = 2;
constexpr int DW_WH = DW_TR + 8;
constexpr int DW_PLANE = DW_WH * TL_WW + 2;
constexpr int DW_CB = 32;
constexpr int DW_IN_FLOATS = DW_CB * DW_PLANE;
constexpr int DW_DYS = DW_TR * 32 + 1;
constexpr int DW_DY_FLOATS = TL_OB * DW_DYS;
constexpr int DW_NT = DW_TR * 3 * 64;

__global__ __launch_bounds__(DW_NT, 3) void dcn_bwd_weight_tile_f32(const float *__restrict__ in, const float *__restrict__ off,
                                                                const float *__restrict__ msk, const float *__restrict__ gy,
                                                                float *__restrict__ part, Geom g, int tiles_x, int tiles_y,
                                                                int nsplit, const unsigned *__restrict__ far_scal)
{
    if (far_dominated(far_scal, g.B * ((g.HoWo + 31) / 32))) return;
    extern __shared__ __attribute__((aligned(16))) float lds[];
    float *win = lds, *dyt = lds + DW_IN_FLOATS;
    const int tid = threadIdx.x;
    const int lane = tid & 63, wave = tid >> 6;
    const int i = lane & 31, h = lane >> 5;
    const int row = wave & 1, ky = wave >> 1;
    const int cb = blockIdx.x, zo = blockIdx.z;
    const int HW = g.H * g.W;
    const int total = g.B * tiles_x * tiles_y;
    const int t0 = (int)((int64_t)blockIdx.y * total / nsplit), t1 = (int)((int64_t)(blockIdx.y + 1) * total / nsplit);

    f32x16 acc[3][2];
#pragma unroll
    for (int a = 0; a < 3; ++a)
#pragma unroll
        for (int mb = 0; mb < 2; ++mb)
#pragma unroll
            for (int r = 0; r < 16; ++r) acc[a][mb][r] = 0.f;

    constexpr int KIN = (DW_CB * DW_WH * 10 + DW_NT - 1) / DW_NT;
    constexpr int KDY = (TL_OB * DW_TR * 8 + DW_NT - 1) / DW_NT;

    for (int ti = t0; ti < t1; ++ti) {
        const int b = ti / (tiles_x * tiles_y);
        const int rem = ti - b * (tiles_x * tiles_y);
        const int ty = rem / tiles_x, tx = rem - ty * tiles_x;
        const int r0 = ty * DW_TR, c0 = tx * 32;
        const int Y0 = r0 - 4, X0 = c0 - 4;
        const float *in_b = in + ((size_t)b * g.C + (size_t)cb * DW_CB) * HW;
        const float *gy_b = gy + ((size_t)b * g.Co + (size_t)zo * TL_OB) * g.HoWo;
        const int cleft = g.C - cb * DW_CB, oleft = g.Co - zo * TL_OB;

        const int ho = r0 + row, wo = c0 + i;
        const bool pv = ho < g.Ho && wo < g.Wo;
        const int Pc = pv ? ho * g.Wo + wo : 0;
        const float *off_b = off + (size_t)b * 18 * g.HoWo;
        const float *msk_b = msk + (size_t)b * 9 * g.HoWo;
        int posv[3];
        float wv[3][4];
#pragma unroll
        for (int kx = 0; kx < 3; ++kx) {
            const int t = ky * 3 + kx;
#ifdef DWT_ABL_NOTAP
            const TapRaw raw = {0.1f * (float)t, 0.2f, 0.5f};
            (void)off_b; (void)msk_b;
#else
            const TapRaw raw = load_tap_raw(off_b, msk_b, g, t, Pc);
#endif
            const float hf = (float)(ho - 1 + ky) + raw.oh, wf_ = (float)(wo - 1 + kx) + raw.ow;
            const bool sv = pv && hf > -1.f && wf_ > -1.f && hf < (float)g.H && wf_ < (float)g.W &&
                            fabsf(raw.oh) < TL_NEAR && fabsf(raw.ow) < TL_NEAR;
            const float hlf = floorf(hf), wlf = floorf(wf_);
            const int ly = sv ? (int)hlf - Y0 : 0, lx = sv ? (int)wlf - X0 : 0;
            posv[kx] = ly * TL_WW + lx;
            const float lh = hf - hlf, lw = wf_ - wlf;
            const float m = sv ? raw.m : 0.f;
            wv[kx][0] = (1.f - lh) * (1.f - lw) * m; wv[kx][1] = (1.f - lh) * lw * m;
            wv[kx][2] = lh * (1.f - lw) * m;         wv[kx][3] = lh * lw * m;
        }

#ifndef DWT_ABL_NOBAR
        __syncthreads();
#endif
#ifdef DWT_ABL_NOSTAGE
        if (ti == t0)
#endif
        {
        const f32x4 zero4 = {0.f, 0.f, 0.f, 0.f};
        typedef float f32x2_ __attribute__((ext_vector_type(2)));
#pragma unroll 1
        for (int k0 = 0; k0 < KIN; k0 += 3) {
            f32x4 rin[3];
#pragma unroll
            for (int k = 0; k < 3; ++k) {
                const int e = tid + DW_NT * (k0 + k);
                const int ch = e / (DW_WH * 10), rm = e - ch * (DW_WH * 10);
                const int wr = rm / 10, q = rm - wr * 10;
                const int y = Y0 + wr, x = X0 + 4 * q;
                rin[k] = zero4;
                if (e < DW_CB * DW_WH * 10 && ch < cleft && y >= 0 && y < g.H && x >= 0 && x < g.W)
                    rin[k] = *reinterpret_cast<const f32x4 *>(in_b + (size_t)ch * HW + y * g.W + x);
            }
#pragma unroll
            for (int k = 0; k < 3; ++k) {
                const int e = tid + DW_NT * (k0 + k);
                const int ch = e / (DW_WH * 10), rm = e - ch * (DW_WH * 10);
                if (e < DW_CB * DW_WH * 10) {
                    float *d = win + ch * DW_PLANE + rm * 4;
                    *reinterpret_cast<f32x2_ *>(d) = f32x2_{rin[k].x, rin[k].y};
                    *reinterpret_cast<f32x2_ *>(d + 2) = f32x2_{rin[k].z, rin[k].w};
                }
            }
        }
        {
            f32x4 rdy[KDY];
#pragma unroll
            for (int k = 0; k < KDY; ++k) {
                const int e = tid + DW_NT * k;
                const int o = e / (DW_TR * 8), rm = e - o * (DW_TR * 8);
                const int wr = rm / 8, q = rm - wr * 8;
                const int y = r0 + wr, x = c0 + 4 * q;
                rdy[k] = zero4;
                if (e < TL_OB * DW_TR * 8 && o < oleft && y < g.Ho && x < g.Wo)
                    rdy[k] = *reinterpret_cast<const f32x4 *>(gy_b + (size_t)o * g.HoWo + y * g.Wo + x);
            }
#pragma unroll
            for (int k = 0; k < KDY; ++k) {
                const int e = tid + DW_NT * k;
                const int o = e / (DW_TR * 8), rm = e - o * (DW_TR * 8);
                if (e < TL_OB * DW_TR * 8) {
                    float *d = dyt + o * DW_DYS + rm * 4;
                    d[0] = rdy[k].x; d[1] = rdy[k].y; d[2] = rdy[k].z; d[3] = rdy[k].w;
                }
            }
        }
        }
#ifndef DWT_ABL_NOBAR
        __syncthreads();
#endif

        const float *wl_ = win + i * DW_PLANE;
        const float *dl0 = dyt + i * DW_DYS + row * 32 + h, *dl1 = dl0 + 32 * DW_DYS;
#pragma unroll 2
        for (int s = 0; s < 16; ++s) {
            const int src = 2 * s + h;
            const float d0 = dl0[2 * s], d1 = dl1[2 * s];
#pragma unroll
            for (int kx = 0; kx < 3; ++kx) {
#ifdef DWT_ABL_NOSHFL
                const int pos = posv[kx] + (src & 1);
                const float q0 = wv[kx][0], q1 = wv[kx][1], q2 = wv[kx][2], q3 = wv[kx][3];
#else
                const int pos = __shfl(posv[kx], src);
                const float q0 = __shfl(wv[kx][0], src), q1 = __shfl(wv[kx][1], src);
                const float q2 = __shfl(wv[kx][2], src), q3 = __shfl(wv[kx][3], src);
#endif
                const float *cp = wl_ + pos;
#ifdef DWT_ABL_NOGATHER
                const float val = q0 + q1 * (float)pos + q2 + q3 * (float)s;
                (void)cp;
#else
                const float val = q0 * cp[0] + q1 * cp[1] + q2 * cp[TL_WW] + q3 * cp[TL_WW + 1];
#endif
#ifdef DWT_ABL_NOMFMA
                acc[kx][0][s] += val * d0;
                acc[kx][1][s] += val * d1;
#else
                acc[kx][0] = __builtin_amdgcn_mfma_f32_32x32x2f32(val, d0, acc[kx][0], 0, 0, 0);
                acc[kx][1] = __builtin_amdgcn_mfma_f32_32x32x2f32(val, d1, acc[kx][1], 0, 0, 0);
#endif
            }
        }
    }

    constexpr int STG = DW_CB * 9 + 1;
    float *stage = lds;
    float *mine = part + ((size_t)(cb * gridDim.z + zo) * nsplit + blockIdx.y) * (2 * 32 * DW_CB * 9);
#pragma unroll
    for (int mb = 0; mb < 2; ++mb) {
        __syncthreads();
        if (row == 0) {
#pragma unroll
            for (int kx = 0; kx < 3; ++kx)
#pragma unroll
                for (int r = 0; r < 16; ++r)
                    stage[i * STG + ((r & 3) + 8 * (r >> 2) + 4 * h) * 9 + ky * 3 + kx] = acc[kx][mb][r];
        }
        __syncthreads();
        if (row == 1) {
#pragma unroll
            for (int kx = 0; kx < 3; ++kx)
#pragma unroll
                for (int r = 0; r < 16; ++r)
                    stage[i * STG + ((r & 3) + 8 * (r >> 2) + 4 * h) * 9 + ky * 3 + kx] += acc[kx][mb][r];
        }
        __syncthreads();
        for (int e = tid; e < 32 * DW_CB * 9; e += DW_NT) {
            const int ol = e / (DW_CB * 9), j = e - ol * (DW_CB * 9);
            mine[mb * (32 * DW_CB * 9) + e] = stage[ol * STG + j];
        }
    }
}

__global__ void dcn_dw_reduce(const float *__restrict__ part, float *__restrict__ gw, Geom g, int ncb, int nzo, int nsplit,
                              const unsigned *__restrict__ far_scal)
{
    if (far_dominated(far_scal, g.B * ((g.HoWo + 31) / 32))) return;
    constexpr int PER = 2 * 32 * DW_CB * 9;
    const int n = ncb * nzo * PER;
    const int s0 = (int)((int64_t)blockIdx.y * nsplit / gridDim.y), s1 = (int)((int64_t)(blockIdx.y + 1) * nsplit / gridDim.y);
    for (int idx = blockIdx.x * blockDim.x + threadIdx.x; idx < n; idx += gridDim.x * blockDim.x) {
        const int blk = idx / PER, e = idx - blk * PER;
        const int cb = blk / nzo, zo = blk - cb * nzo;
        const int mb = e / (32 * DW_CB * 9), e2 = e - mb * (32 * DW_CB * 9);
        const int ol = e2 / (DW_CB * 9), j = e2 - ol * (DW_CB * 9);
        const int o = zo * TL_OB + mb * 32 + ol, c = cb * DW_CB + j / 9;
        if (o >= g.Co || c >= g.C) continue;
        const float *src = part + (size_t)blk * nsplit * PER + e;
        float sum = 0.f;
#pragma unroll 8
        for (int sp = s0; sp < s1; ++sp) sum += src[(size_t)sp * PER];
        atomicAdd(gw + ((size_t)o * g.C + (size_t)cb * DW_CB) * 9 + j, sum);
    }
}

struct ZeroRanges {
    unsigned *p[8];
    unsigned n[8];
    unsigned *mark_p = nullptr;
    unsigned mark_v = 0u;
};
__device__ __forceinline__ void zero_ranges_body(const ZeroRanges &z, unsigned bid, unsigned nb)
{
    if (z.mark_p && bid == 0 && threadIdx.x == 0) *z.mark_p = z.mark_v;
#pragma unroll
    for (int r = 0; r < 8; ++r) {
        unsigned *p = z.p[r];
        const unsigned n = z.n[r];
        for (unsigned i = bid * blockDim.x + threadIdx.x; i < n; i += nb * blockDim.x) p[i] = 0u;
    }
}
__global__ void dcn_zero_ranges(ZeroRanges z) { zero_ranges_body(z, blockIdx.x, gridDim.x); }

inline int pick_mb(int nb, int tiles_total)
{
    for (int mb = 8; mb > 1; mb >>= 1) {
        if (mb > nb) continue;
        if ((int64_t)tiles_total * ((nb + mb - 1) / mb) >= 1024) return mb;
    }
    return 1;
}

#include "dcn_v2_bf16x3.inc"
#include "dcn_bwd_sweep.inc"

}

namespace {

template <int V>
__global__ void dcn_offset_mask_split(const float *__restrict__ out, float *__restrict__ offset, float *__restrict__ mask, int B, int T,
                                      int64_t HW)
{
    const int64_t per_img = (int64_t)3 * T * HW / V, n = (int64_t)B * per_img;
    for (int64_t i = (int64_t)blockIdx.x * blockDim.x + threadIdx.x; i < n; i += (int64_t)gridDim.x * blockDim.x) {
        const int64_t b = i / per_img, r = (i - b * per_img) * V;
        const bool is_off = r < (int64_t)2 * T * HW;
        float *dst = is_off ? offset + b * 2 * T * HW + r : mask + b * T * HW + (r - (int64_t)2 * T * HW);
        if (V == 4) {
            f32x4 v = *reinterpret_cast<const f32x4 *>(out + b * 3 * T * HW + r);
            if (!is_off) {
#pragma unroll
                for (int j = 0; j < 4; ++j) v[j] = 1.f / (1.f + __expf(-v[j]));
            }
            *reinterpret_cast<f32x4 *>(dst) = v;
        } else {
            const float v = out[b * 3 * T * HW + r];
            *dst = is_off ? v : 1.f / (1.f + __expf(-v));
        }
    }
}

template <int V>
__global__ void dcn_offset_mask_merge(const float *__restrict__ goff, const float *__restrict__ gmask, const float *__restrict__ mask,
                                      float *__restrict__ gout, int B, int T, int64_t HW)
{
    const int64_t per_img = (int64_t)3 * T * HW / V, n = (int64_t)B * per_img;
    for (int64_t i = (int64_t)blockIdx.x * blockDim.x + threadIdx.x; i < n; i += (int64_t)gridDim.x * blockDim.x) {
        const int64_t b = i / per_img, r = (i - b * per_img) * V;
        const bool is_off = r < (int64_t)2 * T * HW;
        const int64_t rm = r - (int64_t)2 * T * HW;
        if (V == 4) {
            f32x4 v;
            if (is_off) v = *reinterpret_cast<const f32x4 *>(goff + b * 2 * T * HW + r);
            else {
                const f32x4 g = *reinterpret_cast<const f32x4 *>(gmask + b * T * HW + rm);
                const f32x4 m = *reinterpret_cast<const f32x4 *>(mask + b * T * HW + rm);
#pragma unroll
                for (int j = 0; j < 4; ++j) v[j] = g[j] * m[j] * (1.f - m[j]);
            }
            *reinterpret_cast<f32x4 *>(gout + b * 3 * T * HW + r) = v;
        } else {
            float v;
            if (is_off) v = goff[b * 2 * T * HW + r];
            else {
                const float m = mask[b * T * HW + rm];
                v = gmask[b * T * HW + rm] * m * (1.f - m);
            }
            gout[b * 3 * T * HW + r] = v;
        }
    }
}

}

#include "dcn_dense.inc"

extern "C" {

static size_t dw_partial_floats(int Cin, int Cout)
{
    const size_t nb = (size_t)((Cin + DW_CB - 1) / DW_CB) * ((Cout + TL_OB - 1) / TL_OB);
    return (nb > 512 ? nb : 512) * (size_t)(2 * 32 * DW_CB * 9);
}

static size_t tileflag_bytes(const Geom &g) { return ((size_t)g.B * ((g.H + 3) / 4) * ((g.W + 31) / 32) + 255) / 256 * 256; }

static size_t blockmax_bytes(const Geom &g)
{
    return ((size_t)g.B * g.dg * g.KK * ((g.Ho + 7) / 8) * ((g.Wo + 7) / 8) + 255) / 256 * 256 + tileflag_bytes(g);
}

static size_t base_workspace_bytes(const Geom &g)
{
    const size_t cells = (size_t)g.B * g.dg * g.KK * g.H * g.W;
    const size_t ntile = (size_t)g.B * ((g.HoWo + 31) / 32);
    const size_t n = (size_t)g.Kp * g.Cop * sizeof(float) * 2 + 256 + ((cells + 255) / 256 * 256) + cells * INV_CAP * 8 + 256 +
                     ((ntile + 255) / 256 * 256) + (ntile + 63) / 64 * 64 * sizeof(int) + dw_partial_floats(g.C, g.Co) * sizeof(float);
    return (n + 255) / 256 * 256 + blockmax_bytes(g);
}

size_t dcd_dcn_v2_workspace_bytes(int B, int Cin, int H, int W, int Cout, int kh, int kw, int sh, int sw, int ph,
                                  int pw, int dh, int dw, int dg)
{
    Geom g;
    if (!make_geom(g, B, Cin, H, W, Cout, kh, kw, sh, sw, ph, pw, dh, dw, dg)) return 0;
    return base_workspace_bytes(g) + dense_workspace_bytes(g) + sweep_workspace_bytes(g);
}

int dcd_dcn_v2_forward(void *stream_, const float *input, const float *weight, const float *bias,
                       const float *offset, const float *mask, float *output, int B, int Cin, int H, int W,
                       int Cout, int kh, int kw, int sh, int sw, int ph, int pw, int dh, int dw, int dg,
                       int precision, void *workspace, size_t workspace_bytes)
{
    hipStream_t stream = (hipStream_t)stream_;
    (void)hipGetLastError();
    Geom g;
    if (!input || !weight || !bias || !offset || !mask || !output || !workspace) return DCD_ERR_BAD_ARG;
    if (!make_geom(g, B, Cin, H, W, Cout, kh, kw, sh, sw, ph, pw, dh, dw, dg)) return DCD_ERR_BAD_ARG;
    if (precision != DCD_PREC_F32 && precision != DCD_PREC_BF16X3 && precision != DCD_PREC_BF16) return DCD_ERR_BAD_ARG;
    const bool split = precision != DCD_PREC_F32;
    const bool one = precision == DCD_PREC_BF16;
    const size_t nw = (size_t)g.Kp * g.Cop;
    if (workspace_bytes < nw * sizeof(float) * 2) return DCD_ERR_WORKSPACE;
    if (dense_ok(g, false)) {
        if (workspace_bytes < base_workspace_bytes(g) + dense_workspace_bytes(g)) return DCD_ERR_WORKSPACE;
        dense_forward(stream, input, weight, bias, offset, mask, output, g, (float *)((char *)workspace + base_workspace_bytes(g)),
                      precision);
        return hipGetLastError() == hipSuccess ? DCD_OK : DCD_ERR_LAUNCH;
    }
    float *wf = (float *)workspace, *wb = wf + nw;

    const int tiles = (g.HoWo + 31) / 32;
    const int nb = g.Cop / 32;
    const int mb = pick_mb(nb, tiles * B);
    dim3 grid((tiles + 3) / 4, B, (nb + mb - 1) / mb), block(256);
#ifndef DCN_NO_FWD_TILE
    if (kh == 3 && kw == 3 && sh == 1 && sw == 1 && ph == 1 && pw == 1 && dh == 1 && dw == 1 && dg == 1 && (W & 3) == 0 &&
        H >= 8 && W >= 32 && dcd_env("DCD_NO_TILE") == nullptr) {
        const int nz = (Cout + TL_OB - 1) / TL_OB;
        const int nchunk = split ? (Cin + TB_CH - 1) / TB_CH : (Cin + TL_CH - 1) / TL_CH;
        const size_t nwl = (size_t)nz * nchunk * (split ? TB_W_FLOATS : TL_W_FLOATS);
        if (nwl <= 2 * nw) {
            static LdsLimit lds_limit8, lds_limit4, lds_limit8b, lds_limit4b;
            static int tile_rows = 0;
            if (tile_rows == 0) {
                const char *e = dcd_env("DCD_TILE_ROWS");
                tile_rows = (e && atoi(e) == 4) ? 4 : 8;
            }
            if (!lds_limit8.raise((int)(2 * TileCfg<8>::BUF * sizeof(float)), dcn_fwd_tile_f32<8>) ||
                !lds_limit4.raise((int)(2 * TileCfg<4>::BUF * sizeof(float)), dcn_fwd_tile_f32<4>))
                return DCD_ERR_LAUNCH;
            if (split && (!lds_limit8b.raise((int)(TileCfgB<8>::NBUF * TileCfgB<8>::BUF * sizeof(float)), dcn_fwd_tile_bf16x3<8, 3>,
                                             dcn_fwd_tile_bf16x3<8, 1>) ||
                          !lds_limit4b.raise((int)(TileCfgB<4>::NBUF * TileCfgB<4>::BUF * sizeof(float)), dcn_fwd_tile_bf16x3<4, 3>,
                                             dcn_fwd_tile_bf16x3<4, 1>)))
                return DCD_ERR_LAUNCH;
            static int rescue_taps = 0;
            if (rescue_taps == 0) {
                const char *e = dcd_env("DCD_FWD_RESCUE_TAPS");
                rescue_taps = (e && atoi(e) >= 1 && atoi(e) <= 10) ? atoi(e) : 5;
            }
            const int tiles_x = (g.Wo + 31) / 32;
            const bool rows8 = tile_rows == 8 && (int64_t)tiles_x * ((g.Ho + 7) / 8) * B * nz >= 512;
            const int TRr = rows8 ? 8 : 4;
            const int regions = tiles_x * ((g.Ho + TRr - 1) / TRr);
            const int nflag_words = (B * regions + 3) / 4 + 1;
            unsigned char *flags = (unsigned char *)(wf + 2 * nw);
            unsigned *far_count = (unsigned *)flags + (nflag_words - 1);
            const int64_t ncoord = (int64_t)B * 18 * g.HoWo;
            const bool keeps = forward_keeps_far_samples(weight, ncoord);
            const unsigned far_limit = keeps ? 0xffffffffu : (unsigned)(ncoord / 32 < 0xffffffffll ? ncoord / 32 : 0xffffffffll);
            const int rescue_taps_call = keeps ? 10 : rescue_taps;
            const size_t n9 = (size_t)Cin * 9 * g.Cop;
            if (nwl <= nw && n9 <= nw && workspace_bytes >= 2 * nw * sizeof(float) + (size_t)nflag_words * 4) {
                float *wf9 = wf + nw;
                if (split)
                    hipLaunchKernelGGL(dcn_prep_weights_tile_bf16, dim3((unsigned)((nwl + 255) / 256 < 2048 ? (nwl + 255) / 256 : 2048)),
                                       dim3(256), 0, stream, weight, (unsigned short *)wf, g, nchunk, nz, (unsigned *)flags, nflag_words, wf9);
                else
                    hipLaunchKernelGGL(dcn_prep_weights_tile, dim3((unsigned)((nwl + 255) / 256 < 2048 ? (nwl + 255) / 256 : 2048)),
                                       dim3(256), 0, stream, weight, wf, g, nchunk, nz, (unsigned *)flags, nflag_words, wf9);
                if (!keeps) {
                    int gsz = (int)((ncoord + 4095) / 4096);
                    if (gsz > 512) gsz = 512;
                    hipLaunchKernelGGL(dcn_fwd_far_count, dim3(gsz), dim3(256), 0, stream, offset, ncoord, far_count);
                }
#define DCD_FWD_TILE_B(TRV, NPV)                                                                                                      \
    hipLaunchKernelGGL((dcn_fwd_tile_bf16x3<TRV, NPV>), dim3(regions, B, nz), dim3(TRV * 64),                                         \
                       TileCfgB<TRV>::NBUF * TileCfgB<TRV>::BUF * sizeof(float), stream, input, offset, mask, (const float *)wf, bias, \
                       output, g, tiles_x, nchunk, flags, (const float *)wf9, rescue_taps_call, (const unsigned *)far_count, far_limit)
                if (split && rows8) {
                    if (one) DCD_FWD_TILE_B(8, 1); else DCD_FWD_TILE_B(8, 3);
                } else if (split) {
                    if (one) DCD_FWD_TILE_B(4, 1); else DCD_FWD_TILE_B(4, 3);
                }
#undef DCD_FWD_TILE_B
                else if (rows8)
                    hipLaunchKernelGGL(dcn_fwd_tile_f32<8>, dim3(regions, B, nz), dim3(512), 2 * TileCfg<8>::BUF * sizeof(float), stream,
                                       input, offset, mask, wf, bias, output, g, tiles_x, nchunk, flags, (const float *)wf9, rescue_taps_call,
                                       (const unsigned *)far_count, far_limit);
                else
                    hipLaunchKernelGGL(dcn_fwd_tile_f32<4>, dim3(regions, B, nz), dim3(256), 2 * TileCfg<4>::BUF * sizeof(float), stream,
                                       input, offset, mask, wf, bias, output, g, tiles_x, nchunk, flags, (const float *)wf9, rescue_taps_call,
                                       (const unsigned *)far_count, far_limit);
                if (keeps) return hipGetLastError() == hipSuccess ? DCD_OK : DCD_ERR_LAUNCH;
                const int nb9 = g.Cop / 32, mb9 = nb9 >= 4 ? 4 : nb9 >= 2 ? 2 : 1;
                dim3 gridr((tiles_x * g.Ho + 3) / 4, B, (nb9 + mb9 - 1) / mb9);
                if (mb9 == 4)
                    hipLaunchKernelGGL((dcn_fwd9_f32<4, true>), gridr, dim3(256), 0, stream, input, offset, mask, wf9, bias, output, g,
                                       (const unsigned char *)flags, tiles_x, TRr, nchunk);
                else if (mb9 == 2)
                    hipLaunchKernelGGL((dcn_fwd9_f32<2, true>), gridr, dim3(256), 0, stream, input, offset, mask, wf9, bias, output, g,
                                       (const unsigned char *)flags, tiles_x, TRr, nchunk);
                else
                    hipLaunchKernelGGL((dcn_fwd9_f32<1, true>), gridr, dim3(256), 0, stream, input, offset, mask, wf9, bias, output, g,
                                       (const unsigned char *)flags, tiles_x, TRr, nchunk);
                return hipGetLastError() == hipSuccess ? DCD_OK : DCD_ERR_LAUNCH;
            }
        }
    }
#endif
#ifndef DCN_NO_FWD9
    if (g.KK == 9 && W >= 2 && (size_t)Cin * 9 * g.Cop <= nw) {
        const size_t n9 = (size_t)Cin * 9 * g.Cop;
        hipLaunchKernelGGL(dcn_prep_weights9, dim3((unsigned)((n9 + 255) / 256 < 2048 ? (n9 + 255) / 256 : 2048)), dim3(256), 0,
                           stream, weight, wf, g);
        const int mb9 = mb > 4 ? 4 : mb;
        dim3 grid9((tiles + 3) / 4, B, (nb + mb9 - 1) / mb9);
        switch (mb9) {
            case 4: hipLaunchKernelGGL(dcn_fwd9_f32<4>, grid9, block, 0, stream, input, offset, mask, wf, bias, output, g); break;
            case 2: hipLaunchKernelGGL(dcn_fwd9_f32<2>, grid9, block, 0, stream, input, offset, mask, wf, bias, output, g); break;
            default: hipLaunchKernelGGL(dcn_fwd9_f32<1>, grid9, block, 0, stream, input, offset, mask, wf, bias, output, g); break;
        }
        return hipGetLastError() == hipSuccess ? DCD_OK : DCD_ERR_LAUNCH;
    }
#endif
    hipLaunchKernelGGL(dcn_prep_weights, dim3((unsigned)((nw + 255) / 256 < 2048 ? (nw + 255) / 256 : 2048)), dim3(256),
                       0, stream, weight, wf, wb, g);
    switch (mb) {
        case 8: hipLaunchKernelGGL(dcn_fwd_f32<8>, grid, block, 0, stream, input, offset, mask, wf, bias, output, g); break;
        case 4: hipLaunchKernelGGL(dcn_fwd_f32<4>, grid, block, 0, stream, input, offset, mask, wf, bias, output, g); break;
        case 2: hipLaunchKernelGGL(dcn_fwd_f32<2>, grid, block, 0, stream, input, offset, mask, wf, bias, output, g); break;
        default: hipLaunchKernelGGL(dcn_fwd_f32<1>, grid, block, 0, stream, input, offset, mask, wf, bias, output, g); break;
    }
    return hipGetLastError() == hipSuccess ? DCD_OK : DCD_ERR_LAUNCH;
}

int dcd_dcn_v2_backward(void *stream_, const float *input, const float *weight, const float *bias,
                        const float *offset, const float *mask, const float *grad_output, float *grad_input,
                        float *grad_offset, float *grad_mask, float *grad_weight, float *grad_bias, int B,
                        int Cin, int H, int W, int Cout, int kh, int kw, int sh, int sw, int ph, int pw, int dh,
                        int dw, int dg, int precision, void *workspace, size_t workspace_bytes)
{
    (void)bias;
    hipStream_t stream = (hipStream_t)stream_;
    (void)hipGetLastError();
    Geom g;
    if (!input || !weight || !offset || !mask || !grad_output || !grad_input || !grad_offset || !grad_mask ||
        !grad_weight || !grad_bias || !workspace)
        return DCD_ERR_BAD_ARG;
    if (!make_geom(g, B, Cin, H, W, Cout, kh, kw, sh, sw, ph, pw, dh, dw, dg)) return DCD_ERR_BAD_ARG;
    if (precision != DCD_PREC_F32 && precision != DCD_PREC_BF16X3 && precision != DCD_PREC_BF16) return DCD_ERR_BAD_ARG;
    const bool split = precision != DCD_PREC_F32;
    const bool one = precision == DCD_PREC_BF16;
    const size_t nw = (size_t)g.Kp * g.Cop;
    if (workspace_bytes + 256 < dcd_dcn_v2_workspace_bytes(B, Cin, H, W, Cout, kh, kw, sh, sw, ph, pw, dh, dw, dg))
        return DCD_ERR_WORKSPACE;
    float *wf = (float *)workspace, *wb = wf + nw;
    const size_t cells = (size_t)B * dg * g.KK * H * W;
    InvLists inv;
    unsigned *absmax = (unsigned *)(wb + nw);
    inv.absmax_bits = absmax;
    inv.cnt = (unsigned char *)absmax + 256;
    inv.idx = (int *)(inv.cnt + (cells + 255) / 256 * 256);
    inv.w = (float *)(inv.idx + cells * INV_CAP);
    inv.packed = 0;
    const size_t ntile = (size_t)B * ((g.HoWo + 31) / 32);
    unsigned char *far_flag = (unsigned char *)(((uintptr_t)(inv.w + cells * INV_CAP) + 255) / 256 * 256);
    int *far_list = (int *)(far_flag + (ntile + 255) / 256 * 256);
    float *dw_part = (float *)(far_list + (ntile + 63) / 64 * 64);
    unsigned char *blockmax = (unsigned char *)workspace + (base_workspace_bytes(g) - blockmax_bytes(g));
    inv.blockmax = blockmax;
    unsigned char *tileflag = (unsigned char *)workspace + (base_workspace_bytes(g) - tileflag_bytes(g));
    inv.tileflag = nullptr;
    inv.flag_tx = (W + 31) / 32;
    inv.flag_ty = (H + 3) / 4;
    const dim3 bm_grid(((g.Ho + 7) / 8) * ((g.Wo + 7) / 8), dg * g.KK, B);

    const char *sw_e = dcd_env("DCD_SWEEP_WIDE");
    const bool sweep_wide = !(sw_e && atoi(sw_e) == 0);
    const bool use_sweep = sweep_ok(g) && (g.Cop <= 64 || (sweep_wide && (g.Cop <= 128 || !dense_ok(g, true)))) && dense_mode() != 1 &&
                           (sweep_mode() == 1 || !dense_ok(g, true));
    unsigned *dense_report = nullptr;
    const bool far_to_dense = use_sweep && dense_ok(g, true) &&
                              handover_far_dominated(weight, far_count_limit(g, g.Co > 64), &dense_report);
    if ((!use_sweep || far_to_dense) && dense_ok(g, true)) {
        ZeroRanges z;
        for (int r = 0; r < 8; ++r) { z.p[r] = nullptr; z.n[r] = 0; }
        z.p[0] = absmax; z.n[0] = 4;
        z.p[1] = (unsigned *)far_flag; z.n[1] = (unsigned)((ntile + 3) / 4);
        z.p[3] = (unsigned *)grad_bias; z.n[3] = (unsigned)Cout;
        hipLaunchKernelGGL(dcn_zero_ranges, dim3(8), dim3(256), 0, stream, z);
        hipLaunchKernelGGL(dcn_prep_weights, dim3((unsigned)((nw + 255) / 256 < 2048 ? (nw + 255) / 256 : 2048)), dim3(256),
                           0, stream, weight, wf, wb, g);
        const int64_t noff = (int64_t)B * dg * 2 * g.KK * g.HoWo;
        int gsz = (int)((noff + 4095) / 4096);
        if (gsz > 512) gsz = 512;
        hipLaunchKernelGGL(dcn_offset_absmax, dim3(gsz), dim3(256), 0, stream, offset, noff, absmax, g.HoWo, dg * 2 * g.KK,
                           (g.HoWo + 31) / 32, far_flag, far_list);
        if (dense_report) hipLaunchKernelGGL(dcn_far_report, dim3(1), dim3(64), 0, stream, (const unsigned *)absmax, dense_report);
        hipLaunchKernelGGL(dcn_offset_blockmax, bm_grid, dim3(64), 0, stream, offset, g, blockmax);
        hipLaunchKernelGGL(dcn_build_inverse, dim3((H * W + 255) / 256, dg * g.KK, B), dim3(256), 0, stream, offset, mask, inv, g);
        int splits = (int)(((int64_t)g.HoWo + 4095) / 4096);
        if (splits > 32) splits = 32;
        hipLaunchKernelGGL(dcn_bias_grad, dim3(Cout, splits), dim3(256), 0, stream, grad_output, grad_bias, B, Cout, g.HoWo);
        dense_backward(stream, input, wb, offset, mask, grad_output, grad_input, grad_offset, grad_mask, grad_weight, g, inv,
                       (float *)((char *)workspace + base_workspace_bytes(g)), precision);
        return hipGetLastError() == hipSuccess ? DCD_OK : DCD_ERR_LAUNCH;
    }
    const int tiles = (g.HoWo + 31) / 32;
    const int nblk = g.cpgp / 32;
    if (!use_sweep)
        hipLaunchKernelGGL(dcn_prep_weights, dim3((unsigned)((nw + 255) / 256 < 2048 ? (nw + 255) / 256 : 2048)), dim3(256),
                           0, stream, weight, wf, wb, g);
    if (use_sweep) {
        const SweepPlan sp = sweep_plan(g);
        float *swp = (float *)((char *)workspace + base_workspace_bytes(g) + dense_workspace_bytes(g));
        float *cpart = swp + sp.wp_floats, *dwpart = cpart + sp.cpart_floats;
        const unsigned *fs = (const unsigned *)absmax;
        int nsplit = 1;
        while (nsplit * 2 <= nblk) nsplit *= 2;
        unsigned *far_report = nullptr;
        const unsigned real_limit = far_count_limit(g, sp.nob > 1);
        const int handover = handover_decide(stream, weight, real_limit, &far_report);
        const unsigned far_limit = handover ? real_limit : FAR_COUNT_PIVOT - 1;
        {
            const int nb_gen = handover ? (int)((nw + 255) / 256 < 1024 ? (nw + 255) / 256 : 1024) : 0;
            const int nb_sw = (int)((sp.wp_floats + 255) / 256 < 2048 ? (sp.wp_floats + 255) / 256 : 2048);
            hipLaunchKernelGGL(dcn_sweep_prologue_a, dim3(nb_gen + nb_sw), dim3(256), 0, stream, weight, wf, wb, swp, absmax, g, sp.nck, sp.nob,
                               split ? 1 : 0, nb_gen, far_limit);
        }
        {
            ZeroRanges z;
            for (int r = 0; r < 8; ++r) { z.p[r] = nullptr; z.n[r] = 0; }
            z.p[2] = (unsigned *)grad_weight; z.n[2] = (unsigned)((size_t)Cout * Cin * g.KK);
            z.p[3] = (unsigned *)grad_bias; z.n[3] = (unsigned)Cout;
            z.p[4] = (unsigned *)grad_input; z.n[4] = (unsigned)((size_t)B * Cin * H * W);
            const int nb_zero = (int)(z.n[4] / 1024 + 1 < 4096 ? z.n[4] / 1024 + 1 : 4096);
            const int64_t noff = (int64_t)B * 18 * g.HoWo;
            int nb_scan = (int)((noff + 4095) / 4096);
            if (nb_scan > 512) nb_scan = 512;
            hipLaunchKernelGGL(dcn_sweep_prologue_b, dim3(nb_zero + nb_scan), dim3(256), 0, stream, z, nb_zero, offset, noff, absmax, g.HoWo,
                               (g.HoWo + 31) / 32);
        }
        {
            SweepArgs a;
            a.in = input; a.off = offset; a.msk = mask; a.wp = swp; a.gy = grad_output; a.gin = grad_input; a.cpart = cpart;
            a.dwpart = dwpart; a.far_scal = fs; a.g = g; a.nstrip = sp.nstrip; a.nseg = sp.nseg; a.seg_rows = sp.seg_rows;
            a.nck = sp.nck; a.nv = sp.nv; a.nslot = sp.nslot;
            a.col = dwpart + sp.dw_floats;
            static LdsLimit sw_lds_limit;
            const int ldsb = SW_WAVES * SW_LDS_FLOATS * (int)sizeof(float);
            if (!sw_lds_limit.raise(ldsb, dcn_bwd_sweep<DCD_PREC_F32, 1, true>, dcn_bwd_sweep<DCD_PREC_BF16X3, 1, true>,
                                    dcn_bwd_sweep<DCD_PREC_F32, 2, false>, dcn_bwd_sweep<DCD_PREC_BF16X3, 2, false>,
                                    dcn_bwd_sweep<DCD_PREC_F32, 4, false>, dcn_bwd_sweep<DCD_PREC_BF16X3, 4, false>,
                                    dcn_bwd_sweep<DCD_PREC_BF16, 1, true>, dcn_bwd_sweep<DCD_PREC_BF16, 2, false>,
                                    dcn_bwd_sweep<DCD_PREC_BF16, 4, false>))
                return DCD_ERR_LAUNCH;
            const dim3 sgrid(sp.nslot / SW_WAVES), sblock(64 * SW_WAVES);
#define DCD_LAUNCH_SWEEP(NOBV, DWKV)                                                                                     \
    do {                                                                                                                \
        if (one) hipLaunchKernelGGL((dcn_bwd_sweep<DCD_PREC_BF16, NOBV, DWKV>), sgrid, sblock, ldsb, stream, a);        \
        else if (split) hipLaunchKernelGGL((dcn_bwd_sweep<DCD_PREC_BF16X3, NOBV, DWKV>), sgrid, sblock, ldsb, stream, a); \
        else hipLaunchKernelGGL((dcn_bwd_sweep<DCD_PREC_F32, NOBV, DWKV>), sgrid, sblock, ldsb, stream, a);             \
    } while (0)
            if (sp.nob == 1) DCD_LAUNCH_SWEEP(1, true);
            else if (sp.nob == 2) DCD_LAUNCH_SWEEP(2, false);
            else DCD_LAUNCH_SWEEP(4, false);
#undef DCD_LAUNCH_SWEEP
        }
        {
            SweepEpilogueArgs e;
            e.cpart = cpart; e.gy = grad_output; e.dwpart = dwpart; e.goff = grad_offset; e.gmsk = grad_mask; e.gw = grad_weight;
            e.gbias = grad_bias; e.far_scal = fs; e.g = g; e.nck = sp.nck; e.total_tiles = B * tiles;
            e.far_report = far_report; e.far_base = FAR_COUNT_PIVOT - far_limit;
            e.bias_only_if_far = sp.nob == 1 ? fs : (const unsigned *)nullptr;
            const int64_t n4 = (int64_t)B * 27 * g.HoWo / 4;
            e.nb_coord = (int)((n4 + 255) / 256 < 4096 ? (n4 + 255) / 256 : 4096);
            int splits = (int)(((int64_t)g.HoWo + 4095) / 4096);
            if (splits > 32) splits = 32;
            if (splits < 1) splits = 1;
            e.bias_splits = splits;
            int nb_dw;
            if (sp.nob == 1) {
                const int nred = sp.nck * SW_DW_FLOATS + 64;
                e.nvp = sp.nslot / sp.nck;
                e.dw_bx = (nred + 255) / 256;
                e.dw_by = e.nvp >= 64 ? 16 : (e.nvp >= 8 ? 4 : 1);
                e.gemm_n = 0; e.gemm_S = 0;
                nb_dw = e.dw_bx * e.dw_by;
            } else {
                static_assert(SW_GEMM_T == SG_T && SW_GEMM_K == SG_K, "sweep_plan sizes the product's partials with these");
                const int K9 = Cin * 9, n = Cout * K9;
                SgemmArgs ga;
                ga.A = grad_output; ga.B = dwpart + sp.dw_floats; ga.C = dwpart; ga.bias = nullptr; ga.M = Cout; ga.N = K9; ga.K = g.HoWo;
                ga.lda = g.HoWo; ga.ldb = g.HoWo; ga.ldc = K9;
                ga.strideA = (long long)Cout * g.HoWo; ga.strideB = (long long)K9 * g.HoWo;
                ga.strideC = (long long)sp.dw_split * n; ga.strideCs = n;
                ga.nsplit = sp.dw_split; ga.kchunk = sp.dw_kchunk; ga.ct = 0; ga.b_off = nullptr;
                ga.skip_count = fs + 3; ga.skip_above = FAR_COUNT_PIVOT;
                if (split) sgemm_bf16x3(stream, true, true, ga, B, one);
                else sgemm_f32(stream, true, true, ga, B);
                e.nvp = 0; e.dw_bx = 0; e.dw_by = 0;
                e.gemm_n = n; e.gemm_S = B * sp.dw_split;
                nb_dw = (n / 4 + 255) / 256 < 512 ? (n / 4 + 255) / 256 : 512;
            }
            hipLaunchKernelGGL(dcn_sweep_epilogue, dim3(e.nb_coord + Cout * splits + nb_dw), dim3(256), 0, stream, e);
        }
        if (!handover) return hipGetLastError() == hipSuccess ? DCD_OK : DCD_ERR_LAUNCH;
        inv.packed = 0;
        inv.tileflag = nullptr;
        hipLaunchKernelGGL(dcn_offset_blockmax, bm_grid, dim3(64), 0, stream, offset, g, blockmax, fs);
        hipLaunchKernelGGL(dcn_build_inverse, dim3((H * W + 255) / 256, 9, B), dim3(256), 0, stream, offset, mask, inv, g, fs);
        {
            const int in_tiles = (H * W + 31) / 32;
            int mbi = nblk >= 8 ? 8 : nblk >= 4 ? 4 : nblk >= 2 ? 2 : 1;
            while (mbi > 1 && (int64_t)in_tiles * B * ((nblk + mbi - 1) / mbi) < 1024) mbi >>= 1;
            dim3 grid((in_tiles + 3) / 4, B, (nblk + mbi - 1) / mbi), block(256);
            if (mbi == 8) hipLaunchKernelGGL(dcn_bwd_input_f32<8>, grid, block, 0, stream, grad_output, wb, inv, grad_input, g, 0, fs);
            else if (mbi == 4) hipLaunchKernelGGL(dcn_bwd_input_f32<4>, grid, block, 0, stream, grad_output, wb, inv, grad_input, g, 0, fs);
            else if (mbi == 2) hipLaunchKernelGGL(dcn_bwd_input_f32<2>, grid, block, 0, stream, grad_output, wb, inv, grad_input, g, 0, fs);
            else hipLaunchKernelGGL(dcn_bwd_input_f32<1>, grid, block, 0, stream, grad_output, wb, inv, grad_input, g, 0, fs);
        }
        {
            dim3 grid((tiles + 3) / 4, B, nsplit), block(256);
#define DCD_LAUNCH_BD_FAR(NS)                                                                                            \
    hipLaunchKernelGGL(dcn_bwd_data_f32<NS>, grid, block, 0, stream, input, offset, mask, wb, grad_output, grad_input,  \
                       grad_offset, grad_mask, grad_bias, g, nsplit, inv, fs, (const int *)far_list, 1)
            if (g.Cop == 32) DCD_LAUNCH_BD_FAR(16);
            else if (g.Cop == 64) DCD_LAUNCH_BD_FAR(32);
            else if (g.Cop == 128) DCD_LAUNCH_BD_FAR(64);
            else if (g.Cop == 256) DCD_LAUNCH_BD_FAR(128);
            else DCD_LAUNCH_BD_FAR(0);
#undef DCD_LAUNCH_BD_FAR
        }
        {
            const int RB = 9 * nblk;
            const int nb = g.Cop / 32;
            const int mb = nb >= 8 ? 8 : nb >= 4 ? 4 : nb >= 2 ? 2 : 1;
            const int gx = (RB + 3) / 4, gz = (nb + mb - 1) / mb;
            const int total = B * tiles;
            int S = 512 / (gx * gz);
            if (S < 1) S = 1;
            if (S > total) S = total;
            dim3 grid(gx, S, gz), block(256);
            const size_t lds = (size_t)(4 * 32 * 33 + mb * 32 * 33) * sizeof(float);
#define DCD_LAUNCH_BW_FAR(MBV)                                                                                           \
    hipLaunchKernelGGL(dcn_bwd_weight_f32<MBV>, grid, block, lds, stream, input, offset, mask, grad_output, grad_weight, g, \
                       tiles, S, fs, (const int *)far_list)
            if (mb == 8) DCD_LAUNCH_BW_FAR(8);
            else if (mb == 4) DCD_LAUNCH_BW_FAR(4);
            else if (mb == 2) DCD_LAUNCH_BW_FAR(2);
            else DCD_LAUNCH_BW_FAR(1);
#undef DCD_LAUNCH_BW_FAR
        }
        return hipGetLastError() == hipSuccess ? DCD_OK : DCD_ERR_LAUNCH;
    }
    int nsplit = 1;
    while ((int64_t)tiles * B * nsplit < 1536 && nsplit * 2 <= nblk) nsplit *= 2;

    const bool tile_shape = kh == 3 && kw == 3 && sh == 1 && sw == 1 && ph == 1 && pw == 1 && dh == 1 && dw == 1 && dg == 1 &&
                            (W & 3) == 0 && H >= 8 && W >= 32 && dcd_env("DCD_NO_TILE") == nullptr;
    static int bd128 = -1;
    if (bd128 < 0) {
        const char *e = dcd_env("DCD_BD_TILE128");
        bd128 = (e && atoi(e) == 1) ? 1 : 0;
    }
    const bool bd_tile_ok = tile_shape && (g.Cop == 64 || (g.Cop == 128 && bd128));
    {
        ZeroRanges z;
        for (int r = 0; r < 8; ++r) { z.p[r] = nullptr; z.n[r] = 0; }
        z.p[0] = absmax; z.n[0] = 4;
        z.p[1] = (unsigned *)far_flag; z.n[1] = (unsigned)((ntile + 3) / 4);
        z.p[2] = (unsigned *)grad_weight; z.n[2] = (unsigned)((size_t)Cout * Cin * g.KK);
        z.p[3] = (unsigned *)grad_bias; z.n[3] = (unsigned)Cout;
        if (nsplit > 1 || (bd_tile_ok && nblk > 1)) {
            z.p[4] = (unsigned *)grad_offset; z.n[4] = (unsigned)((size_t)B * dg * 2 * g.KK * g.HoWo);
            z.p[5] = (unsigned *)grad_mask; z.n[5] = (unsigned)((size_t)B * dg * g.KK * g.HoWo);
        }
        z.p[6] = (unsigned *)tileflag; z.n[6] = (unsigned)(tileflag_bytes(g) / 4);
        const size_t most = (size_t)z.n[2] > (size_t)z.n[4] ? z.n[2] : z.n[4];
        hipLaunchKernelGGL(dcn_zero_ranges, dim3((unsigned)(most / 1024 + 1 < 2048 ? most / 1024 + 1 : 2048)), dim3(256), 0, stream, z);
    }

    {
        const int64_t noff = (int64_t)B * dg * 2 * g.KK * g.HoWo;
        int gsz = (int)((noff + 4095) / 4096);
        if (gsz > 512) gsz = 512;
        hipLaunchKernelGGL(dcn_offset_absmax, dim3(gsz), dim3(256), 0, stream, offset, noff, absmax, g.HoWo, dg * 2 * g.KK,
                           (g.HoWo + 31) / 32, far_flag, far_list);
        const int HWin = H * W;
#ifndef DCN_NO_BWD_TILE
        static int bi_nblk = 0;
        if (bi_nblk == 0) {
            const char *e = dcd_env("DCD_BI_TILE_NBLK");
            bi_nblk = e ? atoi(e) : 2;
            if (bi_nblk < 1) bi_nblk = 2;
        }
        const bool bi_tile_ok = tile_shape && nblk <= bi_nblk && (nblk <= 2 || g.Cop <= 64) && H < 65536 && W < 65536 &&
                                dcd_env("DCD_NO_BI_TILE") == nullptr;
#else
        const bool bi_tile_ok = false;
#endif
        inv.packed = bi_tile_ok ? 1 : 0;
        static int bi_hybrid = -1;
        if (bi_hybrid < 0) {
            const char *e = dcd_env("DCD_BI_HYBRID");
            bi_hybrid = (e && atoi(e) == 0) ? 0 : 1;
        }
        inv.tileflag = (bi_tile_ok && bi_hybrid) ? tileflag : nullptr;
        hipLaunchKernelGGL(dcn_offset_blockmax, bm_grid, dim3(64), 0, stream, offset, g, blockmax);
        hipLaunchKernelGGL(dcn_build_inverse, dim3((HWin + 255) / 256, dg * g.KK, B), dim3(256), 0, stream, offset, mask, inv, g);
        bool bi_tiled = false;
#ifndef DCN_NO_BWD_TILE
        if (bi_tile_ok) {
            static LdsLimit lds_limit;
            const size_t ldsb = (size_t)(BI_OC * BI_PLANE + (BI_OC / 2) * 9 * 2 * 2 * 32) * sizeof(float);
            if (!lds_limit.raise((int)ldsb, dcn_bwd_input_tile_f32<2>)) return DCD_ERR_LAUNCH;
            const int tiles_x = (W + 31) / 32, tiles_y = (H + BI_TR - 1) / BI_TR;
            hipLaunchKernelGGL(dcn_bwd_input_tile_f32<2>, dim3(tiles_x * tiles_y, B, (nblk + 1) / 2), dim3(BI_TR * 64), ldsb, stream,
                               grad_output, wb, inv, grad_input, g, tiles_x);
            bi_tiled = true;
        }
#endif
        const int in_tiles = (HWin + 31) / 32;
        const int total_blocks = dg * nblk;
        int mbi = total_blocks >= 8 ? 8 : total_blocks >= 4 ? 4 : total_blocks >= 2 ? 2 : 1;
        while (mbi > 1 && (int64_t)in_tiles * B * ((total_blocks + mbi - 1) / mbi) < 1024) mbi >>= 1;
        if (const char *e = dcd_env("DCD_BI_MB")) {
            const int v = atoi(e);
            if ((v == 1 || v == 2 || v == 4 || v == 8) && v <= total_blocks) mbi = v;
        }
        dim3 grid((in_tiles + 3) / 4, B, (total_blocks + mbi - 1) / mbi), block(256);
        const int partner = bi_tiled ? 1 : 0;
        if (mbi == 8) hipLaunchKernelGGL(dcn_bwd_input_f32<8>, grid, block, 0, stream, grad_output, wb, inv, grad_input, g, partner);
        else if (mbi == 4) hipLaunchKernelGGL(dcn_bwd_input_f32<4>, grid, block, 0, stream, grad_output, wb, inv, grad_input, g, partner);
        else if (mbi == 2) hipLaunchKernelGGL(dcn_bwd_input_f32<2>, grid, block, 0, stream, grad_output, wb, inv, grad_input, g, partner);
        else hipLaunchKernelGGL(dcn_bwd_input_f32<1>, grid, block, 0, stream, grad_output, wb, inv, grad_input, g, partner);
    }
    {
        int splits = (int)(((int64_t)g.HoWo + 4095) / 4096);
        if (splits > 32) splits = 32;
        if (splits < 1) splits = 1;
        hipLaunchKernelGGL(dcn_bias_grad, dim3(Cout, splits), dim3(256), 0, stream, grad_output, grad_bias, B, Cout, g.HoWo);
    }
    bool bd_tiled = false;
#ifndef DCN_NO_BWD_TILE
    if (bd_tile_ok) {
        static LdsLimit lds_limit;
        const size_t ldsb = (size_t)(BD_CB * BD_PLANE + 2 * g.Cop * 32) * sizeof(float);
        if (!lds_limit.raise((int)((BD_CB * BD_PLANE + 2 * 128 * 32) * sizeof(float)), dcn_bwd_data_tile_f32<32>, dcn_bwd_data_tile_f32<64>))
            return DCD_ERR_LAUNCH;
        const int tiles_x = (g.Wo + 31) / 32, tiles_y = (g.Ho + BD_TR - 1) / BD_TR;
        const int nsp = nblk;
        dim3 gridt(tiles_x * tiles_y, B, nsp), blockt(BD_TR * 64);
        if (g.Cop == 64)
            hipLaunchKernelGGL(dcn_bwd_data_tile_f32<32>, gridt, blockt, ldsb, stream, input, offset, mask, wb, grad_output, grad_input,
                               grad_offset, grad_mask, g, tiles_x, nsp, inv, (const unsigned *)absmax);
        else
            hipLaunchKernelGGL(dcn_bwd_data_tile_f32<64>, gridt, blockt, ldsb, stream, input, offset, mask, wb, grad_output, grad_input,
                               grad_offset, grad_mask, g, tiles_x, nsp, inv, (const unsigned *)absmax);
        bd_tiled = true;
    }
#endif
    {
        dim3 grid((tiles + 3) / 4, B, nsplit), block(256);
        const int ns = g.Cop / 2;
#define DCD_LAUNCH_BD(NS)                                                                                          \
    hipLaunchKernelGGL(dcn_bwd_data_f32<NS>, grid, block, 0, stream, input, offset, mask, wb, grad_output, grad_input, \
                       grad_offset, grad_mask, grad_bias, g, nsplit, inv, bd_tiled ? (const unsigned *)absmax : (const unsigned *)nullptr, \
                       (const int *)far_list)
        if (ns == 16) DCD_LAUNCH_BD(16);
        else if (ns == 32) DCD_LAUNCH_BD(32);
        else if (ns == 64) DCD_LAUNCH_BD(64);
        else if (ns == 128) DCD_LAUNCH_BD(128);
        else DCD_LAUNCH_BD(0);
#undef DCD_LAUNCH_BD
    }
    bool dw_tiled = false;
#ifndef DCN_NO_BWD_TILE
    if (tile_shape) {
        static LdsLimit lds_limit, lds_limit2, lds_limit2b;
        const size_t ldsb = (size_t)(DW_IN_FLOATS + DW_DY_FLOATS) * sizeof(float);
        if (!lds_limit.raise((int)ldsb, dcn_bwd_weight_tile_f32) ||
            !lds_limit2.raise((int)(Dw2Cfg<DCD_PREC_F32>::FLOATS * sizeof(float)), dcn_bwd_weight_tile_v2<DCD_PREC_F32>) ||
            !lds_limit2b.raise((int)(Dw2Cfg<DCD_PREC_BF16X3>::FLOATS * sizeof(float)), dcn_bwd_weight_tile_v2<DCD_PREC_BF16X3>))
            return DCD_ERR_LAUNCH;
        static int dw_gen = 0;
        if (dw_gen == 0) {
            const char *e = dcd_env("DCD_DW_GEN");
            dw_gen = (e && atoi(e) == 1) ? 1 : 2;
        }
        static int dw_colmajor = -1;
        if (dw_colmajor < 0) {
            const char *e = dcd_env("DCD_DW_ORDER");
            dw_colmajor = (e && atoi(e) == 0) ? 0 : 1;
        }
        const int tiles_x = (g.Wo + 31) / 32, tiles_y = (g.Ho + DW_TR - 1) / DW_TR;
        const int ncb = (Cin + DW_CB - 1) / DW_CB, nzo = (Cout + TL_OB - 1) / TL_OB;
        const int total = B * tiles_x * tiles_y;
        int S = 512 / (ncb * nzo);
        if (S < 1) S = 1;
        if (S > total) S = total;
        if (split)
            hipLaunchKernelGGL(dcn_bwd_weight_tile_v2<DCD_PREC_BF16X3>, dim3(ncb, S, nzo), dim3(DW_NT),
                               Dw2Cfg<DCD_PREC_BF16X3>::FLOATS * sizeof(float), stream, input, offset, mask, grad_output, dw_part, g,
                               tiles_x, tiles_y, S, (const unsigned *)absmax, dw_colmajor);
        else if (dw_gen == 2)
            hipLaunchKernelGGL(dcn_bwd_weight_tile_v2<DCD_PREC_F32>, dim3(ncb, S, nzo), dim3(DW_NT),
                               Dw2Cfg<DCD_PREC_F32>::FLOATS * sizeof(float), stream, input, offset, mask, grad_output, dw_part, g,
                               tiles_x, tiles_y, S, (const unsigned *)absmax, dw_colmajor);
        else
            hipLaunchKernelGGL(dcn_bwd_weight_tile_f32, dim3(ncb, S, nzo), dim3(DW_NT), ldsb, stream, input, offset, mask, grad_output,
                               dw_part, g, tiles_x, tiles_y, S, (const unsigned *)absmax);
        const int nred = ncb * nzo * 2 * 32 * DW_CB * 9;
        const int rgroups = S >= 16 ? 16 : S;
        hipLaunchKernelGGL(dcn_dw_reduce, dim3((nred + 255) / 256, rgroups), dim3(256), 0, stream, dw_part, grad_weight, g, ncb, nzo, S,
                           (const unsigned *)absmax);
        dw_tiled = true;
    }
#endif
    {
        const int RB = dg * g.KK * nblk;
        const int nb = g.Cop / 32;
        const int mb = nb >= 8 ? 8 : nb >= 4 ? 4 : nb >= 2 ? 2 : 1;
        const int gx = (RB + 3) / 4, gz = (nb + mb - 1) / mb;
        const int total = B * tiles;
        int S = 512 / (gx * gz);
        if (S < 1) S = 1;
        if (S > total) S = total;
        dim3 grid(gx, S, gz), block(256);
        const size_t lds = (size_t)(4 * 32 * 33 + mb * 32 * 33) * sizeof(float);
#define DCD_LAUNCH_BW(MBV)                                                                                        \
    hipLaunchKernelGGL(dcn_bwd_weight_f32<MBV>, grid, block, lds, stream, input, offset, mask, grad_output, grad_weight, g, \
                       tiles, S, dw_tiled ? (const unsigned *)absmax : (const unsigned *)nullptr, (const int *)far_list)
        if (mb == 8) DCD_LAUNCH_BW(8);
        else if (mb == 4) DCD_LAUNCH_BW(4);
        else if (mb == 2) DCD_LAUNCH_BW(2);
        else DCD_LAUNCH_BW(1);
#undef DCD_LAUNCH_BW
    }
    return hipGetLastError() == hipSuccess ? DCD_OK : DCD_ERR_LAUNCH;
}

#ifdef SW_PROFILE
int dcd_debug_sweep_profile(unsigned long long *host_out)
{
    return hipMemcpyFromSymbol(host_out, HIP_SYMBOL(sw_prof_buf), sizeof(unsigned long long) * 2048) == hipSuccess ? 0 : 1;
}
#endif

int dcd_dcn_v2_forget(const float *weight)
{
    int dev = 0;
    if (hipGetDevice(&dev) != hipSuccess) return DCD_ERR_LAUNCH;
    std::lock_guard<std::mutex> lock(g_handover_mu);
    int n = 0;
    for (auto it = g_handover.begin(); it != g_handover.end();) {
        if (it->first.first == dev && (!weight || it->first.second == (const void *)weight)) {
            if (it->second.host) {
                *(volatile unsigned *)it->second.host = HANDOVER_UNKNOWN;
                g_handover_free[dev].push_back(it->second);
            }
            it = g_handover.erase(it);
            ++n;
        } else {
            ++it;
        }
    }
    (void)n;
    return DCD_OK;
}

int dcd_dcn_v2_policy_state(const float *weight, unsigned *far_count)
{
    int dev = 0;
    if (!weight || hipGetDevice(&dev) != hipSuccess) return -1;
    std::lock_guard<std::mutex> lock(g_handover_mu);
    auto it = g_handover.find(std::make_pair(dev, (const void *)weight));
    if (it == g_handover.end() || !it->second.host) return 0;
    const unsigned far = *(volatile unsigned *)it->second.host;
    if (far == HANDOVER_UNKNOWN) return 1;
    if (far_count) *far_count = far;
    return 2;
}

int dcd_dcn_v2_set_handover(int mode)
{
    if (mode < -1 || mode > 2) return DCD_ERR_BAD_ARG;
    g_handover_pin.store(mode, std::memory_order_relaxed);
    return DCD_OK;
}

int dcd_dcn_v2_policy_free(void)
{
    std::lock_guard<std::mutex> lock(g_handover_mu);
    for (auto &kv : g_handover)
        if (kv.second.host) (void)hipHostFree(kv.second.host);
    g_handover.clear();
    for (auto &kv : g_handover_free)
        for (HandoverState &h : kv.second)
            if (h.host) (void)hipHostFree(h.host);
    g_handover_free.clear();
    (void)hipGetLastError();
    return DCD_OK;
}

int dcd_dcn_offset_mask_split(void *stream_, const float *out, float *offset, float *mask, int B, int taps, int64_t HW)
{
    (void)hipGetLastError();
    if (!out || !offset || !mask || B <= 0 || taps <= 0 || HW <= 0) return DCD_ERR_BAD_ARG;
    const bool v4 = (HW & 3) == 0 && (((uintptr_t)out | (uintptr_t)offset | (uintptr_t)mask) & 15) == 0;
    const int64_t n = (int64_t)B * 3 * taps * HW / (v4 ? 4 : 1);
    const unsigned grid = (unsigned)((n + 255) / 256 < 8192 ? (n + 255) / 256 : 8192);
    if (v4) hipLaunchKernelGGL(dcn_offset_mask_split<4>, dim3(grid), dim3(256), 0, (hipStream_t)stream_, out, offset, mask, B, taps, HW);
    else hipLaunchKernelGGL(dcn_offset_mask_split<1>, dim3(grid), dim3(256), 0, (hipStream_t)stream_, out, offset, mask, B, taps, HW);
    return hipGetLastError() == hipSuccess ? DCD_OK : DCD_ERR_LAUNCH;
}

int dcd_dcn_offset_mask_merge(void *stream_, const float *grad_offset, const float *grad_mask, const float *mask, float *grad_out, int B,
                              int taps, int64_t HW)
{
    (void)hipGetLastError();
    if (!grad_offset || !grad_mask || !mask || !grad_out || B <= 0 || taps <= 0 || HW <= 0) return DCD_ERR_BAD_ARG;
    const bool v4 = (HW & 3) == 0 &&
                    (((uintptr_t)grad_offset | (uintptr_t)grad_mask | (uintptr_t)mask | (uintptr_t)grad_out) & 15) == 0;
    const int64_t n = (int64_t)B * 3 * taps * HW / (v4 ? 4 : 1);
    const unsigned grid = (unsigned)((n + 255) / 256 < 8192 ? (n + 255) / 256 : 8192);
    if (v4)
        hipLaunchKernelGGL(dcn_offset_mask_merge<4>, dim3(grid), dim3(256), 0, (hipStream_t)stream_, grad_offset, grad_mask, mask, grad_out,
                           B, taps, HW);
    else
        hipLaunchKernelGGL(dcn_offset_mask_merge<1>, dim3(grid), dim3(256), 0, (hipStream_t)stream_, grad_offset, grad_mask, mask, grad_out,
                           B, taps, HW);
    return hipGetLastError() == hipSuccess ? DCD_OK : DCD_ERR_LAUNCH;
}

int dcd_sgemm_shifted(void *stream_, const float *A, int lda, long long strideA, const float *Bbase, const long long *b_off,
                      long long strideB, int b_kcontig, const float *bias, float *C, int ldc, long long strideC,
                      long long strideCs, int M, int N, int K, int Z, int nsplit)
{
    (void)hipGetLastError();
    if (!A || !Bbase || !b_off || !C || M <= 0 || N <= 0 || K <= 0 || Z <= 0 || nsplit <= 0 || (lda & 3) || ((uintptr_t)A & 15) ||
        (strideA & 3) || (bias && nsplit != 1))
        return DCD_ERR_BAD_ARG;
    SgemmArgs a;
    a.A = A; a.B = Bbase; a.C = C; a.bias = bias; a.M = M; a.N = N; a.K = K; a.lda = lda; a.ldb = 0; a.ldc = ldc;
    a.strideA = strideA; a.strideB = strideB; a.strideC = strideC; a.strideCs = strideCs;
    a.nsplit = nsplit; a.kchunk = ((K + nsplit - 1) / nsplit + SG_K - 1) / SG_K * SG_K; a.ct = 0; a.b_off = b_off;
    if ((long long)a.kchunk * (nsplit - 1) >= K) return DCD_ERR_BAD_ARG;
    sgemm_f32_rows64((hipStream_t)stream_, b_kcontig != 0, a, Z);
    return hipGetLastError() == hipSuccess ? DCD_OK : DCD_ERR_LAUNCH;
}

}
```

dcd_amd/model/backbone/DCNv2/dcn_v2.py:

```python
import math
import os

import torch
from torch import nn
from torch.autograd import Function
from torch.autograd.function import once_differentiable
from torch.nn.modules.utils import _pair

from dcd_amd import _ext as _backend
from dcd_amd.model.layers.conv import Conv2d


def _precision_scope():
    from dcd_amd import _ext
    return _ext.get_precision()


class _DCNv2(Function):

    @staticmethod
    def forward(ctx, input, offset, mask, weight, bias, stride, padding, dilation, deformable_groups, precision=None):
        kernel = tuple(weight.shape[2:4])
        ctx.geometry = (*kernel, *_pair(stride), *_pair(padding), *_pair(dilation), int(deformable_groups))
        p = _precision_scope() if precision is None else precision
        ctx.precision = {} if p == "f32" else {"precision": p}
        ctx.save_for_backward(input, offset, mask, weight, bias)
        return _backend.dcn_v2_forward(input, weight, bias, offset, mask, *ctx.geometry, **ctx.precision)

    @staticmethod
    @once_differentiable
    def backward(ctx, grad_output):
        input, offset, mask, weight, bias = ctx.saved_tensors
        grads = _backend.dcn_v2_backward(input.contiguous(), weight.contiguous(), bias, offset, mask, grad_output.contiguous(),
                                         *ctx.geometry, **ctx.precision)
        grad_input, grad_offset, grad_mask, grad_weight, grad_bias = grads
        return (grad_input, grad_offset, grad_mask, grad_weight, grad_bias) + (None,) * 5


_FUSED_GLUE = os.environ.get("DCD_OFFSET_MASK_FUSED", "1") != "0"


def _offset_mask_split(out):
    from dcd_amd import _lib
    B, C3, H, W = out.shape
    T = C3 // 3
    offset = torch.empty((B, 2 * T, H, W), dtype=out.dtype, device=out.device)
    mask = torch.empty((B, T, H, W), dtype=out.dtype, device=out.device)
    st = _lib.lib().dcd_dcn_offset_mask_split(_lib.stream_of(out), out.data_ptr(), offset.data_ptr(), mask.data_ptr(), B, T, H * W)
    _lib.check(st, "dcd_dcn_offset_mask_split")
    return offset, mask


def _offset_mask_merge(goff, gmask, mask):
    from dcd_amd import _lib
    B, T, H, W = mask.shape
    goff, gmask = goff.contiguous(), gmask.contiguous()
    gout = torch.empty((B, 3 * T, H, W), dtype=mask.dtype, device=mask.device)
    st = _lib.lib().dcd_dcn_offset_mask_merge(_lib.stream_of(mask), goff.data_ptr(), gmask.data_ptr(), mask.data_ptr(),
                                              gout.data_ptr(), B, T, H * W)
    _lib.check(st, "dcd_dcn_offset_mask_merge")
    return gout


class _OffsetMask(torch.autograd.Function):

    @staticmethod
    def forward(ctx, out):
        offset, mask = _offset_mask_split(out)
        ctx.save_for_backward(mask)
        return offset, mask

    @staticmethod
    @torch.autograd.function.once_differentiable
    def backward(ctx, goff, gmask):
        (mask,) = ctx.saved_tensors
        return _offset_mask_merge(goff, gmask, mask)


_ONE_NODE = os.environ.get("DCD_DCN_NODE", "1") != "0"


class _DCNWithOffsets(Function):

    @staticmethod
    def forward(ctx, input, w_off, b_off, weight, bias, geometry):
        from dcd_amd import ops
        input, w_off, weight = input.contiguous(), w_off.contiguous(), weight.contiguous()
        p = _precision_scope()
        ctx.precision = {} if p == "f32" else {"precision": p}
        out = ops._conv3x3_forward(ctx, input, w_off, b_off.contiguous())
        offset, mask = _offset_mask_split(out)
        ctx.geometry = geometry
        ctx.save_for_backward(input, offset, mask, weight, bias, w_off)
        return _backend.dcn_v2_forward(input, weight, bias, offset, mask, *geometry, **ctx.precision)

    @staticmethod
    @once_differentiable
    def backward(ctx, grad_output):
        from dcd_amd import ops
        input, offset, mask, weight, bias, w_off = ctx.saved_tensors
        grad_input, grad_offset, grad_mask, grad_weight, grad_bias = _backend.dcn_v2_backward(
            input, weight, bias, offset, mask, grad_output.contiguous(), *ctx.geometry, **ctx.precision)
        gout = _offset_mask_merge(grad_offset, grad_mask, mask)
        if ctx.needs_input_grad[0]:
            grad_input = ops._conv3x3_call(gout, w_off, w_off.shape[1], True, residual=grad_input.contiguous(), transformed=ctx.tw_back,
                                           prec=ctx.prec)
        gw_off = ops._conv3x3_wrw_call(input, gout, w_off.shape, ctx.prec) if ctx.needs_input_grad[1] else None
        gb_off = ops.channel_sums(gout) if ctx.needs_input_grad[2] else None
        return grad_input, gw_off, gb_off, grad_weight, grad_bias, None


def dcn_v2_conv(input, offset, mask, weight, bias, stride, padding, dilation, deformable_groups):
    dev = input.device.type
    if torch.is_autocast_enabled(dev):
        with torch.autocast(device_type=dev, enabled=False):
            args = (input.float(), offset.float(), mask.float(), weight.float(), bias.float(), stride, padding, dilation,
                    deformable_groups)
            return _DCNv2.apply(*args, "bf16") if input.is_cuda else _DCNv2.apply(*args)
    return _DCNv2.apply(input, offset, mask, weight, bias, stride, padding, dilation, deformable_groups)


class DCNv2(nn.Module):
    def __init__(self, in_channels, out_channels, kernel_size, stride, padding, dilation=1, deformable_groups=1):
        super().__init__()
        self.in_channels = in_channels
        self.out_channels = out_channels
        self.kernel_size = _pair(kernel_size)
        self.stride = _pair(stride)
        self.padding = _pair(padding)
        self.dilation = _pair(dilation)
        self.deformable_groups = deformable_groups
        self.weight = nn.Parameter(torch.empty(out_channels, in_channels, *self.kernel_size))
        self.bias = nn.Parameter(torch.empty(out_channels))
        self.reset_parameters()

    def reset_parameters(self):
        fan_in = self.in_channels * self.kernel_size[0] * self.kernel_size[1]
        bound = 1.0 / math.sqrt(fan_in)
        self.weight.data.uniform_(-bound, bound)
        self.bias.data.zero_()

    def _forget_policy(self):
        w = self._parameters.get("weight") if hasattr(self, "_parameters") else None
        if w is None or not w.is_cuda:
            return
        try:
            from dcd_amd import _lib
            with torch.cuda.device(w.device):
                _lib.lib().dcd_dcn_v2_forget(w.data_ptr())
        except Exception:
            pass

    def _apply(self, fn, *args, **kwargs):
        self._forget_policy()
        return super()._apply(fn, *args, **kwargs)

    def __del__(self):
        self._forget_policy()

    def forward(self, input, offset, mask):
        taps = self.deformable_groups * self.kernel_size[0] * self.kernel_size[1]
        assert offset.shape[1] == 2 * taps and mask.shape[1] == taps
        return dcn_v2_conv(input, offset, mask, self.weight, self.bias, self.stride, self.padding, self.dilation,
                           self.deformable_groups)


class DCN(DCNv2):

    def __init__(self, in_channels, out_channels, kernel_size, stride, padding, dilation=1, deformable_groups=1):
        super().__init__(in_channels, out_channels, kernel_size, stride, padding, dilation, deformable_groups)
        taps = self.deformable_groups * self.kernel_size[0] * self.kernel_size[1]
        self.conv_offset_mask = Conv2d(self.in_channels, 3 * taps, kernel_size=self.kernel_size,
                                       stride=self.stride, padding=self.padding, bias=True)
        self.init_offset()

    def init_offset(self):
        self.conv_offset_mask.weight.data.zero_()
        self.conv_offset_mask.bias.data.zero_()

    def forward(self, input):
        from dcd_amd import ops
        com = self.conv_offset_mask
        if (_ONE_NODE and _FUSED_GLUE and input.dtype == torch.float32 and not torch.is_autocast_enabled(input.device.type)
                and ops.offset_conv_in_dcn_node(input, com)):
            geometry = (*self.kernel_size, *self.stride, *self.padding, *self.dilation, int(self.deformable_groups))
            return _DCNWithOffsets.apply(input, com.weight, com.bias, self.weight, self.bias, geometry)
        out = com(input)
        taps2 = out.shape[1] // 3 * 2
        if out.is_cuda and out.dtype == torch.float32 and out.is_contiguous() and _FUSED_GLUE:
            offset, mask = _OffsetMask.apply(out)
        else:
            offset = out[:, :taps2]
            mask = torch.sigmoid(out[:, taps2:])
        return dcn_v2_conv(input, offset, mask, self.weight, self.bias, self.stride, self.padding, self.dilation,
                           self.deformable_groups)
```

include/dcd_hip.h:

```cpp
#ifndef DCD_HIP_H
#define DCD_HIP_H

#include <stddef.h>
#include <stdint.h>

#ifdef __cplusplus
extern "C" {
#endif

#define DCD_OK 0
#define DCD_ERR_BAD_ARG 1
#define DCD_ERR_WORKSPACE 2
#define DCD_ERR_LAUNCH 3

const char *dcd_version(void);


#define DCD_PREC_F32 0
#define DCD_PREC_BF16X3 1
#define DCD_PREC_BF16 2

size_t dcd_dcn_v2_workspace_bytes(int B, int Cin, int H, int W, int Cout, int kh, int kw, int sh, int sw,
                                  int ph, int pw, int dh, int dw, int dg);

int dcd_dcn_v2_forward(void *stream, const float *input, const float *weight, const float *bias,
                       const float *offset, const float *mask, float *output, int B, int Cin, int H, int W,
                       int Cout, int kh, int kw, int sh, int sw, int ph, int pw, int dh, int dw, int dg,
                       int precision, void *workspace, size_t workspace_bytes);

int dcd_dcn_v2_backward(void *stream, const float *input, const float *weight, const float *bias,
                        const float *offset, const float *mask, const float *grad_output, float *grad_input,
                        float *grad_offset, float *grad_mask, float *grad_weight, float *grad_bias, int B,
                        int Cin, int H, int W, int Cout, int kh, int kw, int sh, int sw, int ph, int pw, int dh,
                        int dw, int dg, int precision, void *workspace, size_t workspace_bytes);

int dcd_dcn_v2_forget(const float *weight);
int dcd_dcn_v2_policy_state(const float *weight, unsigned *far_count);
int dcd_dcn_v2_policy_free(void);
int dcd_dcn_v2_set_handover(int mode);

int dcd_edge_depth_forward(void *stream, const float *kps, const float *kps3d, const float *rot_y,
                           const float *P, const uint8_t *kmask, int N, int K, int topk, float zmin,
                           float zmax, int normalized, int sub_b3, float *depth, int32_t *pair_idx,
                           float *pair_mask);

int dcd_edge_depth_backward(void *stream, const float *kps, const float *kps3d, const float *rot_y,
                            const float *P, const float *grad_depth, const int32_t *pair_idx, int N, int K,
                            int topk, float zmin, float zmax, int normalized, float *grad_kps,
                            float *grad_kps3d);

int dcd_focal_loss(void *stream, const float *pred, const float *target, int64_t n, float alpha, float beta,
                   float *out, float *grad_pred);

int dcd_giou_loss(void *stream, const float *pred, const float *target, int N, float *losses, float *ious,
                  float *grad_pred);

int dcd_nms_hm(void *stream, const float *heat, int B, int C, int H, int W, float *out);
int dcd_heatmap_topk(void *stream, const float *heat, int B, int C, int H, int W, int K, int fuse_nms,
                     float *scores, int64_t *inds, float *clses, float *ys, float *xs, void *workspace,
                     size_t workspace_bytes);
size_t dcd_heatmap_topk_workspace_bytes(int B, int C, int H, int W, int K);

int dcd_poi_gather(void *stream, const float *feat, const int64_t *index, int B, int C, int H, int W, int M,
                   float *out);
int dcd_poi_scatter_add(void *stream, const float *grad_out, const int64_t *index, int B, int C, int H, int W,
                        int M, float *grad_feat);
int dcd_patch_scatter_add(void *stream, const float *grad_patches, const int64_t *base, int B, int C, int64_t plane, int pitch, int M,
                          float *out);

int dcd_iou3d(void *stream, const float *pred_corners, const float *target_corners, int N, float *iou);

#define DCD_HEADS_MAX 16
typedef struct dcd_head_rows_args {
    int n_heads, T, R, K, C;
    int trunk[DCD_HEADS_MAX], ch0[DCD_HEADS_MAX], out[DCD_HEADS_MAX];
    const float *weight[DCD_HEADS_MAX];
    const float *bias[DCD_HEADS_MAX];
    const float *feat;
    float *y;
    const float *grad_y;
    float *grad_feat;
    float *grad_weight[DCD_HEADS_MAX];
    float *grad_bias[DCD_HEADS_MAX];
} dcd_head_rows_args;

int dcd_head_rows_forward(void *stream, const dcd_head_rows_args *args);
int dcd_head_rows_backward(void *stream, const dcd_head_rows_args *args);

#define DCD_LOSS_ROWS_NCOL 25
typedef struct dcd_loss_rows_args {
    int B, M, C, K, NP, num_classes;
    int ch_box2d, ch_offset, ch_corner, ch_corner_unc, ch_dims, ch_ori_cls, ch_ori_off, ch_depth, ch_depth_unc,
        ch_kpts2d, ch_kpts3d;
    int trunc_log;
    float depth_lo, depth_hi, unc_lo, unc_hi;
    float depth_weight;
    float dim_weight[3];
    float down_ratio, kd_eps;
    const float *pois;
    const uint8_t *reg_mask, *trunc_mask, *find_pcl, *ori_mask;
    const int32_t *cls_ids, *centers;
    const int64_t *pad_size;
    const float *bboxes, *locations, *rotys, *offset_3D, *dimensions, *orientations;
    const float *keypoints, *kp_depth_mask;
    const float *kpts2d, *kpts3d;
    const float *calib_P;
    const float *calib;
    const float *dim_mean;
    float *kps_pred, *kps_tgt, *kps3d_pred, *kps3d_tgt, *rot, *P_rows;
    uint8_t *kmask;
    const float *pair_depth, *pair_mask;
    float *cols, *corners_pred, *corners_tgt, *iou3d, *sums;
    const float *grad_sums;
    float *grad_pois, *grad_pair;
    const float *grad_kps, *grad_kps3d;
} dcd_loss_rows_args;

int dcd_loss_rows_prepare(void *stream, const dcd_loss_rows_args *args);
int dcd_loss_rows_forward(void *stream, const dcd_loss_rows_args *args);
int dcd_loss_rows_backward(void *stream, const dcd_loss_rows_args *args);
int dcd_loss_rows_finish(void *stream, const dcd_loss_rows_args *args);

int dcd_sum_tensors(void *stream, const float *const *srcs, int n, float *out, int64_t numel);

int dcd_dcn_offset_mask_split(void *stream, const float *out, float *offset, float *mask, int B, int taps, int64_t HW);
int dcd_dcn_offset_mask_merge(void *stream, const float *grad_offset, const float *grad_mask, const float *mask, float *grad_out, int B,
                              int taps, int64_t HW);

int dcd_sgemm_shifted(void *stream, const float *A, int lda, long long strideA, const float *Bbase, const long long *b_off,
                      long long strideB, int b_kcontig, const float *bias, float *C, int ldc, long long strideC,
                      long long strideCs, int M, int N, int K, int Z, int nsplit);

int dcd_sgemm(void *stream, const float *A, int lda, long long strideA, int a_kcontig, const float *B, int ldb, long long strideB,
              int b_kcontig, float *C, int ldc, long long strideC, int M, int N, int K, int Z, float alpha, int accumulate,
              int lower_only);

size_t dcd_spd_solve_workspace_bytes(int batch, int n);
int dcd_spd_solve(void *stream, float *S, float *y, int batch, int n, int rows, int *info, void *workspace, size_t workspace_bytes);

int dcd_context_norm_forward(void *stream, const float *x, float *y, float *inv, int rows, int K, float eps);
int dcd_context_norm_backward(void *stream, const float *grad_y, const float *y, const float *inv, float *grad_x, int rows, int K);

int dcd_context_norm_relu_add_forward(void *stream, const float *x, const float *residual, float *y, int rows, int K, float eps);

int dcd_gmw_refine(void *stream, const float *f4, const float *f6, const float *depths, const long long *good_idx, int num_k,
                   const float *raw_location, const float *dim, int B, int C, int K, float *weights, float *pred_depth,
                   float *pred_location);

int dcd_gmw_pack_records(void *stream, const float *rows, const float *k2, const float *k3, int n_rows, int nk, const int *src, int n,
                         int dst0, int cap, const int *pair_i, const int *pair_j, float *e4, float *e6, float *k2_out, float *k3_out,
                         float *rot, float *loc, float *dim);

size_t dcd_bn_workspace_bytes(int C);
int dcd_bn_stats(void *stream, const float *x, int B, int C, int64_t HW, double *stats, void *workspace,
                 size_t workspace_bytes);

int dcd_channel_sums(void *stream, const float *x, int B, int C, int64_t HW, float *sums, void *workspace, size_t workspace_bytes);
int dcd_bn_train_apply(void *stream, const float *x, const float *residual, const float *weight, const float *bias,
                       const double *stats, double count, float *running_mean, float *running_var,
                       int64_t *num_batches_tracked, float momentum, float eps, int relu, float *y, float *save_mean,
                       float *save_invstd, int B, int C, int64_t HW);
int dcd_bn_eval_apply(void *stream, const float *x, const float *residual, const float *weight, const float *bias,
                      const float *running_mean, const float *running_var, float eps, int relu, float *y, int B, int C,
                      int64_t HW);
int dcd_bn_backward_stats(void *stream, const float *grad_y, const float *y, const float *x, const float *save_mean,
                          int B, int C, int64_t HW, double *sums, void *workspace, size_t workspace_bytes);
int dcd_bn_backward_relu_from_x(void *stream, const float *grad_y, const float *x, const float *weight, const float *bias,
                                const float *save_mean, const float *save_invstd, float *grad_x, float *grad_weight, float *grad_bias,
                                int B, int C, int64_t HW, void *workspace, size_t workspace_bytes);
int dcd_bn_backward_stats_params_relu_from_x(void *stream, const float *grad_y, const float *x, const float *weight, const float *bias,
                                             const float *save_mean, const float *save_invstd, int B, int C, int64_t HW, double *sums,
                                             float *grad_weight, float *grad_bias, void *workspace, size_t workspace_bytes);
int dcd_bn_backward_apply_relu_from_x(void *stream, const float *grad_y, const float *x, const float *weight, const float *bias,
                                      const float *save_mean, const float *save_invstd, const double *sums, double count, float *grad_x,
                                      int B, int C, int64_t HW);
int dcd_bn_backward_stats_params(void *stream, const float *grad_y, const float *y, const float *x, const float *save_mean,
                                 const float *save_invstd, int B, int C, int64_t HW, double *sums, float *grad_weight,
                                 float *grad_bias, void *workspace, size_t workspace_bytes);
int dcd_bn_backward_apply(void *stream, const float *grad_y, const float *y, const float *x, const float *weight,
                          const float *save_mean, const float *save_invstd, const double *sums, double count,
                          float *grad_x, float *grad_residual, float *grad_weight, float *grad_bias, int B, int C,
                          int64_t HW);
int dcd_trunk_row_sums(void *stream, const double *WG, const double *Wd, int R, int K, double *sums);
int dcd_trunk_finalize_forward(void *stream, const double *sums, const float *gamma, const float *beta, double count, double eps, int R,
                               float *scale, float *shift, double *stats);
int dcd_trunk_finalize_backward(void *stream, const float *grad_scale, const float *grad_shift, const float *gamma, const double *stats,
                                double count, int R, double *grad_sums, float *grad_gamma, float *grad_beta);
int dcd_trunk_grad_wg(void *stream, const double *grad_sums, const double *Wd, int R, int K, double *grad_WG);

int dcd_bn_at_forward(void *stream, const float *x, const int64_t *pos, const float *weight, const float *bias,
                      const double *stats, double count, float *running_mean, float *running_var,
                      int64_t *num_batches_tracked, float momentum, float eps, int relu, float *x_at, float *y_at,
                      float *save_mean, float *save_invstd, int B, int C, int64_t HW, int N, void *workspace,
                      size_t workspace_bytes);
int dcd_bn_at_backward_sums(void *stream, const float *grad_at, const float *x_at, const float *y_at, const float *weight,
                            const float *save_mean, const float *save_invstd, int relu, int total, int C, double *sums,
                            float *dzk);
int dcd_bn_train_forward(void *stream, const float *x, const float *residual, const float *weight, const float *bias,
                         float *running_mean, float *running_var, int64_t *num_batches_tracked, float momentum, float eps,
                         int relu, float *y, float *save_mean, float *save_invstd, int B, int C, int64_t HW,
                         void *workspace, size_t workspace_bytes);
int dcd_bn_backward(void *stream, const float *grad_y, const float *y, const float *x, const float *weight,
                    const float *save_mean, const float *save_invstd, float *grad_x, float *grad_residual,
                    float *grad_weight, float *grad_bias, int B, int C, int64_t HW, void *workspace,
                    size_t workspace_bytes);

size_t dcd_conv3x3_workspace_bytes(int B, int Cin, int H, int W, int Cout);
int dcd_conv3x3(void *stream, const float *input, const float *weight, const float *bias, const float *residual, float *output,
                int B, int Cin, int H, int W, int Cout, int backward_data, void *workspace, size_t workspace_bytes);

size_t dcd_conv3x3_weights_bytes(int Cin, int Cout, int backward_data);
int dcd_conv3x3_transform_weights(void *stream, const float *weight, int Cin, int Cout, float *forward_out, float *backward_out);
int dcd_conv3x3_transform_weights_table(void *stream, const long long *table, int entries);
int dcd_conv3x3_prepared(void *stream, const float *input, const float *transformed, const float *bias, const float *residual,
                         float *output, int B, int Cin, int H, int W, int Cout, int backward_data, void *workspace,
                         size_t workspace_bytes);

size_t dcd_conv3x3_split_weights_bytes(int Cin, int Cout, int backward_data);
int dcd_conv3x3_split_transform_weights(void *stream, const float *weight, int Cin, int Cout, void *forward_out, void *backward_out);
int dcd_conv3x3_split_transform_weights_table(void *stream, const long long *table, int entries);
size_t dcd_conv3x3_split_workspace_bytes(int B, int Cin, int H, int W, int Cout);
int dcd_conv3x3_split_prepared(void *stream, const float *input, const void *transformed, const float *bias, const float *residual,
                               float *output, int B, int Cin, int H, int W, int Cout, int backward_data, int precision, void *workspace,
                               size_t workspace_bytes);

size_t dcd_conv3x3_bf16_weights_bytes(int Cin, int Cout, int backward_data);
int dcd_conv3x3_bf16_transform_weights(void *stream, const float *weight, int Cin, int Cout, void *forward_out, void *backward_out);
int dcd_conv3x3_bf16_transform_weights_table(void *stream, const long long *table, int entries);
size_t dcd_conv3x3_bf16_workspace_bytes(int B, int Cin, int H, int W, int Cout);
int dcd_conv3x3_bf16_prepared(void *stream, const float *input, const void *transformed, const float *bias, const float *residual,
                              float *output, int B, int Cin, int H, int W, int Cout, int backward_data, void *workspace,
                              size_t workspace_bytes);

int dcd_conv1x1_bf16(void *stream, const float *weight, int ldw, int transposed, int n_inputs, const float *const *inputs,
                     const int *channels, float *output, int B, int M, long long HW);
size_t dcd_conv1x1_wrw_bf16_workspace_bytes(int B, int O, int C, long long HW);
int dcd_conv1x1_wrw_bf16(void *stream, const float *grad_output, const float *input, float *grad_weight, int ldw, int B, int O, int C,
                         long long HW, void *workspace, size_t workspace_bytes);

int dcd_conv1x1_f32(void *stream, const float *weight, int ldw, int transposed, int n_inputs, const float *const *inputs,
                    const int *channels, float *output, int B, int M, long long HW);
size_t dcd_conv1x1_wrw_f32_workspace_bytes(int B, int O, int C, long long HW);
int dcd_conv1x1_wrw_f32(void *stream, const float *grad_output, const float *input, float *grad_weight, int ldw, int B, int O, int C,
                        long long HW, void *workspace, size_t workspace_bytes);

int dcd_conv3x3_s2_f32(void *stream, const float *input, const float *weight, float *output, int B, int Cin, int H, int W, int Cout);
int dcd_conv3x3_s2_f32_backward_data(void *stream, const float *grad_output, const float *weight, float *grad_input, int B, int Cin, int H,
                                     int W, int Cout);
size_t dcd_conv3x3_s2_f32_wrw_workspace_bytes(int B, int Cin, int H, int W, int Cout);
int dcd_conv3x3_s2_f32_wrw(void *stream, const float *input, const float *grad_output, float *grad_weight, int B, int Cin, int H, int W,
                           int Cout, void *workspace, size_t workspace_bytes);

size_t dcd_conv3x3_wrw_workspace_bytes(int B, int Cin, int H, int W, int Cout);
int dcd_conv3x3_wrw(void *stream, const float *input, const float *grad_output, float *grad_weight, int B, int Cin, int H, int W,
                    int Cout, int precision, void *workspace, size_t workspace_bytes);

size_t dcd_conv_stem_workspace_bytes(int Cin, int Cout, int ksize);
int dcd_conv_stem(void *stream, const float *input, const float *weight, float *output, int B, int Cin, int H, int W, int Cout,
                  int ksize, int backward_data, void *workspace, size_t workspace_bytes);
size_t dcd_conv_stem_wrw_workspace_bytes(int Cin, int Cout, int ksize);
int dcd_conv_stem_wrw(void *stream, const float *input, const float *grad_output, float *grad_weight, int B, int Cin, int H, int W,
                      int Cout, int ksize, void *workspace, size_t workspace_bytes);

int dcd_upsample_dw_forward(void *stream, const float *x, const float *weight, float *y, int B, int C, int H, int W, int f);
int dcd_upsample_dw_forward_add(void *stream, const float *x, const float *weight, const float *skip, float *y, int B, int C, int H,
                                int W, int f);

int dcd_maxpool2x2_forward(void *stream, const float *x, float *y, int64_t planes, int H, int W);
int dcd_maxpool2x2_backward(void *stream, const float *x, const float *grad_y, float *grad_x, int64_t planes, int H, int W);
int dcd_upsample_dw_backward(void *stream, const float *x, const float *weight, const float *grad_y, float *grad_x,
                             float *grad_weight, int B, int C, int H, int W, int f);

int dcd_encode_targets(void *stream, const double *objs, const double *kpts3d, const double *P, const int32_t *img_size,
                       const int32_t *n_obj, int B, int M, int n_extra, int in_w, int in_h, int down_ratio, double filter_trunc,
                       double filter_size, double edge_heatmap_ratio, int num_bin, int n_classes, void *const *outputs,
                       int n_outputs);

int dcd_preprocess_images(void *stream, const uint8_t *src, int64_t src_bytes, const int64_t *images, const float *table, int B,
                          int in_h, int in_w, int to_bgr, float *out);

#define DCD_EVAL_MATCH_SCORES 0
#define DCD_EVAL_MATCH_COUNTS 1
#define DCD_EVAL_MAX_THRESHOLDS 41
typedef struct {
    int mode, n_img, n_comb, n_rows, G, D, n_dc, max_dt, T, n_slots;
    int64_t P;
    const int32_t *gt_off, *dt_off, *dc_off;
    const int64_t *pair_off;
    const double *overlaps;
    const int8_t *ign_gt, *ign_dt;
    const double *dt_score, *gt_alpha, *dt_alpha, *dt_box2d, *dc_box;
    const int32_t *comb;
    const double *min_overlap, *thresholds;
    const int32_t *n_thresh;
    double *scores;
    int32_t *counts;
    double *sim_part;
} dcd_eval_match_args;
int dcd_eval_overlaps(void *stream, int n_img, const int32_t *gt_off, const int32_t *dt_off, const int64_t *pair_off, int G, int D,
                      int64_t P, const double *gt_box2d, const double *dt_box2d, const double *gt_box3d, const double *dt_box3d,
                      double *out);
int dcd_eval_match(void *stream, const dcd_eval_match_args *args);
int dcd_eval_sum_similarity(void *stream, const double *part, int n_img, int n, double *out);

size_t dcd_clip_adamw_workspace_bytes(int ntensors, const int64_t *numel);
int dcd_clip_grad_norm_scalars(void *stream, int ntensors, const void *const *grads, const int64_t *numel, float max_norm, void *workspace,
                               size_t workspace_bytes, float *scal);
int dcd_adamw_apply(void *stream, int ntensors, void *const *params, void *const *grads, void *const *exp_avg, void *const *exp_avg_sq,
                    void *const *steps, const int64_t *numel, const float *lr, double beta1, double beta2, double eps, double weight_decay,
                    const float *scal);

int dcd_gather_rows(void *stream, int n_tables, const void *const *src, void *const *dst, const int64_t *row_bytes,
                    const int64_t *src_rows, const int32_t *index, int B);

size_t dcd_sinkhorn_workspace_bytes(int batch, int m, int n);
int dcd_sinkhorn(void *stream, const float *M, const float *r, const float *c, float *P, int batch, int m, int n, float lambda,
                 float max_distance, float tolerance, int max_iterations, int *iterations, void *workspace, size_t workspace_bytes);

#define DCD_DECODE_MAX_CLASSES 8
#define DCD_DECODE_ORI_MULTIBIN 0
#define DCD_DECODE_ORI_HEAD_AXIS 1
#define DCD_DECODE_DIM_NONE 0
#define DCD_DECODE_DIM_EXP 1
#define DCD_DECODE_DIM_LINEAR 2
#define DCD_DECODE_DEPTH_INV_SIGMOID 0
#define DCD_DECODE_DEPTH_EXP 1
#define DCD_DECODE_DEPTH_LINEAR 2
typedef struct {
    int B, K, C, nk, n_bins, num_classes;
    int ch_box2d, ch_offset, ch_corner, ch_corner_unc, ch_dims, ch_ori_cls, ch_ori_off, ch_depth, ch_depth_unc, ch_kpts2d, ch_kpts3d;
    int orientation, dim_mode, dim_std_on, depth_mode;
    int uncertainty_as_conf, records;
    float down_ratio, depth_lo, depth_hi, eps;
    float depth_ref[2];
    float dim_mean[DCD_DECODE_MAX_CLASSES][3], dim_std[DCD_DECODE_MAX_CLASSES][3];
} dcd_decode_args;
int dcd_decode_detections(void *stream, const float *vectors, const float *scores, const float *classes, const float *ys,
// ... 51 lines not shown
```

Baseline: 217.3 images/s.

## Fuse offset/mask split and merge into DCNv2 forward and backward kernels

```diff
diff --git a/dcd_amd/_ext.py b/dcd_amd/_ext.py
--- a/dcd_amd/_ext.py
+++ b/dcd_amd/_ext.py
@@ -78,11 +78,18 @@
 
 
 def dcn_v2_forward(input, weight, bias, offset, mask, kernel_h, kernel_w, stride_h, stride_w,
-                   pad_h, pad_w, dilation_h, dilation_w, deformable_group, precision=None):
+                   pad_h, pad_w, dilation_h, dilation_w, deformable_group, conv_out=None, precision=None):
     _check(input, weight, bias, offset, mask, kernel_h, kernel_w)
     L = _lib.lib()
     B, C, H, W, Co, Ho, Wo = _dims(input, weight, kernel_h, kernel_w, stride_h, stride_w, pad_h, pad_w,
                                    dilation_h, dilation_w)
+    if conv_out is not None:
+        _lib.require_cuda(conv_out)
+        if (tuple(conv_out.shape) != (B, 3 * deformable_group * kernel_h * kernel_w, Ho, Wo) or conv_out.dtype != torch.float32
+                or not (offset.is_contiguous() and mask.is_contiguous())):
+            raise RuntimeError("conv_out %s %s must be float32 (B, 3*dg*kh*kw, Ho, Wo); offset and mask contiguous outputs" % (
+                conv_out.dtype, tuple(conv_out.shape)))
+        conv_out = conv_out.contiguous()
     if tuple(offset.shape) != (B, 2 * deformable_group * kernel_h * kernel_w, Ho, Wo):
         raise RuntimeError("offset shape %s does not match (B, 2*dg*kh*kw, Ho, Wo)" % (tuple(offset.shape),))
     if tuple(mask.shape) != (B, deformable_group * kernel_h * kernel_w, Ho, Wo):
@@ -93,6 +100,12 @@
     ws, nbytes = _workspace(L, input, geom)
     output = torch.empty((B, Co, Ho, Wo), dtype=torch.float32, device=input.device)
     prec = PRECISION[precision or get_precision()]
+    if conv_out is not None:
+        st = L.dcd_dcn_v2_forward_conv(_lib.stream_of(input), input.data_ptr(), weight.data_ptr(), bias.data_ptr(),
+                                       conv_out.data_ptr(), offset.data_ptr(), mask.data_ptr(), output.data_ptr(), *geom, prec,
+                                       ws.data_ptr(), nbytes)
+        _lib.check(st, "dcd_dcn_v2_forward_conv")
+        return output
     st = L.dcd_dcn_v2_forward(_lib.stream_of(input), input.data_ptr(), weight.data_ptr(), bias.data_ptr(),
                               offset.data_ptr(), mask.data_ptr(), output.data_ptr(), *geom, prec,
                               ws.data_ptr(), nbytes)
@@ -101,7 +114,7 @@
 
 
 def dcn_v2_backward(input, weight, bias, offset, mask, grad_output, kernel_h, kernel_w, stride_h, stride_w,
-                    pad_h, pad_w, dilation_h, dilation_w, deformable_group, precision=None):
+                    pad_h, pad_w, dilation_h, dilation_w, deformable_group, merged=False, precision=None):
     _check(input, weight, bias, offset, mask, kernel_h, kernel_w)
     _lib.require_cuda(grad_output)
     if not input.is_contiguous():
@@ -120,11 +133,25 @@
             deformable_group)
     ws, nbytes = _workspace(L, input, geom)
     grad_input = torch.empty_like(input)
-    grad_offset = torch.empty_like(offset)
+    if merged:
+        taps = deformable_group * kernel_h * kernel_w
+        if tuple(offset.shape) != (B, 2 * taps, Ho, Wo) or tuple(mask.shape) != (B, taps, Ho, Wo):
+            raise RuntimeError("offset / mask shapes %s / %s do not match (B, 2*dg*kh*kw, Ho, Wo) / (B, dg*kh*kw, Ho, Wo)" % (
+                tuple(offset.shape), tuple(mask.shape)))
     grad_mask = torch.empty_like(mask)
     grad_weight = torch.empty_like(weight)
     grad_bias = torch.empty_like(bias)
     prec = PRECISION[precision or get_precision()]
+    if merged:
+        grad_conv = torch.empty((B, 3 * taps, Ho, Wo), dtype=torch.float32, device=input.device)
+        grad_conv_bias = torch.empty(3 * taps, dtype=torch.float32, device=input.device)
+        st = L.dcd_dcn_v2_backward_merged(_lib.stream_of(input), input.data_ptr(), weight.data_ptr(), bias.data_ptr(),
+                                          offset.data_ptr(), mask.data_ptr(), grad_output.data_ptr(),
+                                          grad_input.data_ptr(), grad_conv.data_ptr(), grad_conv_bias.data_ptr(), grad_mask.data_ptr(),
+                                          grad_weight.data_ptr(), grad_bias.data_ptr(), *geom, prec, ws.data_ptr(), nbytes)
+        _lib.check(st, "dcd_dcn_v2_backward_merged")
+        return [grad_input, grad_conv[:, :2 * taps], grad_mask, grad_weight, grad_bias, grad_conv, grad_conv_bias]
+    grad_offset = torch.empty_like(offset)
     st = L.dcd_dcn_v2_backward(_lib.stream_of(input), input.data_ptr(), weight.data_ptr(), bias.data_ptr(),
                                offset.data_ptr(), mask.data_ptr(), grad_output.data_ptr(),
                                grad_input.data_ptr(), grad_offset.data_ptr(), grad_mask.data_ptr(),
diff --git a/dcd_amd/_lib.py b/dcd_amd/_lib.py
--- a/dcd_amd/_lib.py
+++ b/dcd_amd/_lib.py
@@ -60,7 +60,9 @@
     "dcd_version": (ctypes.c_char_p, []),
     "dcd_dcn_v2_workspace_bytes": (c_size_t, [c_int] * 14),
     "dcd_dcn_v2_forward": (c_int, [c_void_p] * 7 + [c_int] * 15 + [c_void_p, c_size_t]),
+    "dcd_dcn_v2_forward_conv": (c_int, [c_void_p] * 8 + [c_int] * 15 + [c_void_p, c_size_t]),
     "dcd_dcn_v2_backward": (c_int, [c_void_p] * 12 + [c_int] * 15 + [c_void_p, c_size_t]),
+    "dcd_dcn_v2_backward_merged": (c_int, [c_void_p] * 13 + [c_int] * 15 + [c_void_p, c_size_t]),
     "dcd_dcn_v2_forget": (c_int, [c_void_p]),
     "dcd_dcn_v2_policy_state": (c_int, [c_void_p, c_void_p]),
     "dcd_dcn_v2_policy_free": (c_int, []),
diff --git a/dcd_amd/csrc/dcn_bwd_sweep.inc b/dcd_amd/csrc/dcn_bwd_sweep.inc
--- a/dcd_amd/csrc/dcn_bwd_sweep.inc
+++ b/dcd_amd/csrc/dcn_bwd_sweep.inc
@@ -886,6 +886,8 @@
     int nck, nvp, total_tiles, nb_coord, bias_splits, dw_bx, dw_by, gemm_n, gemm_S;
     unsigned *far_report = nullptr;
     unsigned far_base = 0;
+    int merged = 0;
+    TailArgs tail;
 };
 __global__ __launch_bounds__(256) void dcn_sweep_epilogue(SweepEpilogueArgs a)
 {
@@ -895,6 +897,10 @@
         *a.far_report = c >= a.far_base ? c - a.far_base : 0u;
     }
     if (bid < a.nb_coord) {
+        if (a.merged) {
+            tail_body(a.tail, bid);
+            return;
+        }
         sweep_reduce_coord_body(a.cpart, a.goff, a.gmsk, a.g.B, a.g.HoWo, a.nck, a.far_scal, a.total_tiles, bid, a.nb_coord);
         return;
     }
diff --git a/dcd_amd/csrc/dcn_v2.hip b/dcd_amd/csrc/dcn_v2.hip
--- a/dcd_amd/csrc/dcn_v2.hip
+++ b/dcd_amd/csrc/dcn_v2.hip
@@ -423,19 +423,20 @@
 
 typedef float f32x4 __attribute__((ext_vector_type(4)));
 
-__global__ void dcn_prep_weights_tile(const float *__restrict__ w, float *__restrict__ wl, Geom g, int nchunk, int nz,
-                                      unsigned *__restrict__ flags, int nflag_words, float *__restrict__ wf9)
-{
-    for (int i = blockIdx.x * blockDim.x + threadIdx.x; i < nflag_words; i += gridDim.x * blockDim.x) flags[i] = 0u;
+__device__ __forceinline__ void prep_weights_tile_body(const float *__restrict__ w, float *__restrict__ wl, const Geom &g, int nchunk, int nz,
+                                                       unsigned *__restrict__ flags, int nflag_words, float *__restrict__ wf9, int bid,
+                                                       int nb)
+{
+    for (int i = bid * blockDim.x + threadIdx.x; i < nflag_words; i += nb * blockDim.x) flags[i] = 0u;
     if (wf9) {
         const int K = g.C * 9, n9 = K * g.Cop;
-        for (int idx = blockIdx.x * blockDim.x + threadIdx.x; idx < n9; idx += gridDim.x * blockDim.x) {
+        for (int idx = bid * blockDim.x + threadIdx.x; idx < n9; idx += nb * blockDim.x) {
             const int k = idx / g.Cop, o = idx - k * g.Cop;
             wf9[idx] = (o < g.Co) ? w[(size_t)o * K + k] : 0.f;
         }
     }
     const int n = nz * nchunk * TL_W_FLOATS;
-    for (int idx = blockIdx.x * blockDim.x + threadIdx.x; idx < n; idx += gridDim.x * blockDim.x) {
+    for (int idx = bid * blockDim.x + threadIdx.x; idx < n; idx += nb * blockDim.x) {
         int r = idx;
         const int s = r & 3; r >>= 2;
         const int h = r & 1; r >>= 1;
@@ -445,6 +446,11 @@
         const int oo = z * TL_OB + o, c = ck * TL_CH + 2 * s + h;
         wl[idx] = (oo < g.Co && c < g.C) ? w[((size_t)oo * g.C + c) * 9 + t] : 0.f;
     }
+}
+__global__ void dcn_prep_weights_tile(const float *__restrict__ w, float *__restrict__ wl, Geom g, int nchunk, int nz,
+                                      unsigned *__restrict__ flags, int nflag_words, float *__restrict__ wf9)
+{
+    prep_weights_tile_body(w, wl, g, nchunk, nz, flags, nflag_words, wf9, blockIdx.x, gridDim.x);
 }
 
 constexpr float TL_NEAR_F = 3.f;
@@ -2013,6 +2019,125 @@
     return 1;
 }
 
+constexpr int TAIL_BT = 256;
+constexpr int TAIL_CH = 4096;
+constexpr int TAIL_SMAX = 256;
+
+struct TailArgs {
+    const float *planes;
+    const float *goff, *gmsk;
+    const float *mask;
+    float *gout;
+    float *gmsk_out;
+    double *partial;
+    unsigned *arrivals;
+    float *sums;
+    size_t plane_stride;
+    int B, T, HW, nplane, S, cpp, vec;
+};
+
+__device__ __forceinline__ double tail_wave_sum(double v)
+{
+#pragma unroll
+    for (int o = 32; o; o >>= 1) v += __shfl_down(v, o);
+    return v;
+}
+
+__device__ __forceinline__ void tail_body(const TailArgs &a, int bid)
+{
+    const int c = bid / a.S, s = bid - c * a.S;
+    const int C3 = 3 * a.T, P = a.B * a.cpp;
+    const bool is_msk = c >= 2 * a.T;
+    double ds = 0.0;
+    for (int j = s; j < P; j += a.S) {
+        const int b = j / a.cpp, k = j - b * a.cpp;
+        const int lo = k * TAIL_CH, hi = min(a.HW, lo + TAIL_CH);
+        const float *src = a.planes ? a.planes + ((size_t)b * C3 + c) * a.HW
+                                    : (is_msk ? a.gmsk + ((size_t)b * a.T + (c - 2 * a.T)) * a.HW : a.goff + ((size_t)b * 2 * a.T + c) * a.HW);
+        const float *mp = a.mask + ((size_t)b * a.T + (is_msk ? c - 2 * a.T : 0)) * a.HW;
+        float *dst = a.gout + ((size_t)b * C3 + c) * a.HW;
+        float fs = 0.f;
+        if (a.vec) {
+            for (int i = lo + 4 * (int)threadIdx.x; i < hi; i += 4 * TAIL_BT) {
+                f32x4 v = *reinterpret_cast<const f32x4 *>(src + i);
+                for (int q = 1; q < a.nplane; ++q) {
+                    const f32x4 u = *reinterpret_cast<const f32x4 *>(src + (size_t)q * a.plane_stride + i);
+                    v.x += u.x; v.y += u.y; v.z += u.z; v.w += u.w;
+                }
+                if (is_msk) {
+                    if (a.gmsk_out) *reinterpret_cast<f32x4 *>(a.gmsk_out + (mp - a.mask) + i) = v;
+                    const f32x4 m = *reinterpret_cast<const f32x4 *>(mp + i);
+#pragma unroll
+                    for (int e = 0; e < 4; ++e) v[e] = v[e] * m[e] * (1.f - m[e]);
+                }
+                *reinterpret_cast<f32x4 *>(dst + i) = v;
+                fs += (v.x + v.y) + (v.z + v.w);
+            }
+        } else {
+            for (int i = lo + (int)threadIdx.x; i < hi; i += TAIL_BT) {
+                float v = src[i];
+                for (int q = 1; q < a.nplane; ++q) v += src[(size_t)q * a.plane_stride + i];
+                if (is_msk) {
+                    if (a.gmsk_out) a.gmsk_out[(mp - a.mask) + i] = v;
+                    const float m = mp[i];
+                    v = v * m * (1.f - m);
+                }
+                dst[i] = v;
+                fs += v;
+            }
+        }
+        ds += (double)fs;
+    }
+    __shared__ double tail_sh[TAIL_BT / 64];
+    __shared__ int tail_last;
+    ds = tail_wave_sum(ds);
+    if ((threadIdx.x & 63) == 0) tail_sh[threadIdx.x >> 6] = ds;
+    __syncthreads();
+    if (threadIdx.x == 0) {
+        ds = tail_sh[0];
+#pragma unroll
+        for (int i = 1; i < TAIL_BT / 64; ++i) ds += tail_sh[i];
+        a.partial[(size_t)c * a.S + s] = ds;
+        if (a.arrivals) {
+            __threadfence();
+            tail_last = atomicAdd(&a.arrivals[c], 1u) == (unsigned)(a.S - 1);
+        }
+    }
+    if (!a.arrivals) return;
+    __syncthreads();
+    if (!tail_last || threadIdx.x >= 64) return;
+    __threadfence();
+    double t = 0.0;
+    for (int q = threadIdx.x; q < a.S; q += 64) t += __builtin_nontemporal_load(a.partial + (size_t)c * a.S + q);
+    t = tail_wave_sum(t);
+    if (threadIdx.x == 0) {
+        a.sums[c] = (float)t;
+        a.arrivals[c] = 0u;
+    }
+}
+
+__global__ __launch_bounds__(TAIL_BT) void dcn_offset_tail(TailArgs a) { tail_body(a, blockIdx.x); }
+
+__global__ __launch_bounds__(64) void dcn_offset_tail_combine(const double *__restrict__ partial, int S, float *__restrict__ sums)
+{
+    const int c = blockIdx.x;
+    double t = 0.0;
+    for (int q = threadIdx.x; q < S; q += 64) t += partial[(size_t)c * S + q];
+    t = tail_wave_sum(t);
+    if (threadIdx.x == 0) sums[c] = (float)t;
+}
+
+__host__ inline size_t tail_head_bytes(const Geom &g)
+{
+    const size_t T3 = (size_t)3 * g.dg * g.KK;
+    return T3 * TAIL_SMAX * sizeof(double) + (T3 * sizeof(unsigned) + 255) / 256 * 256;
+}
+__host__ inline size_t tail_workspace_bytes(const Geom &g)
+{
+    const size_t T3 = (size_t)3 * g.dg * g.KK;
+    return tail_head_bytes(g) + ((size_t)g.B * T3 * g.HoWo * sizeof(float) + 255) / 256 * 256 + 256;
+}
+
 #include "dcn_v2_bf16x3.inc"
 #include "dcn_bwd_sweep.inc"
 
@@ -2021,11 +2146,11 @@
 namespace {
 
 template <int V>
-__global__ void dcn_offset_mask_split(const float *__restrict__ out, float *__restrict__ offset, float *__restrict__ mask, int B, int T,
-                                      int64_t HW)
+__device__ __forceinline__ void offset_mask_split_body(const float *__restrict__ out, float *__restrict__ offset, float *__restrict__ mask,
+                                                       int B, int T, int64_t HW, int bid, int nb)
 {
     const int64_t per_img = (int64_t)3 * T * HW / V, n = (int64_t)B * per_img;
-    for (int64_t i = (int64_t)blockIdx.x * blockDim.x + threadIdx.x; i < n; i += (int64_t)gridDim.x * blockDim.x) {
+    for (int64_t i = (int64_t)bid * blockDim.x + threadIdx.x; i < n; i += (int64_t)nb * blockDim.x) {
         const int64_t b = i / per_img, r = (i - b * per_img) * V;
         const bool is_off = r < (int64_t)2 * T * HW;
         float *dst = is_off ? offset + b * 2 * T * HW + r : mask + b * T * HW + (r - (int64_t)2 * T * HW);
@@ -2041,6 +2166,21 @@
             *dst = is_off ? v : 1.f / (1.f + __expf(-v));
         }
     }
+}
+template <int V>
+__global__ void dcn_offset_mask_split(const float *__restrict__ out, float *__restrict__ offset, float *__restrict__ mask, int B, int T,
+                                      int64_t HW)
+{
+    offset_mask_split_body<V>(out, offset, mask, B, T, HW, blockIdx.x, gridDim.x);
+}
+
+template <int V>
+__global__ void dcn_prep_tile_split(const float *__restrict__ w, float *__restrict__ wl, Geom g, int nchunk, int nz,
+                                    unsigned *__restrict__ flags, int nflag_words, float *__restrict__ wf9, int nb_prep,
+                                    const float *__restrict__ conv_out, float *__restrict__ offset, float *__restrict__ mask)
+{
+    if ((int)blockIdx.x < nb_prep) prep_weights_tile_body(w, wl, g, nchunk, nz, flags, nflag_words, wf9, blockIdx.x, nb_prep);
+    else offset_mask_split_body<V>(conv_out, offset, mask, g.B, 9, g.HoWo, blockIdx.x - nb_prep, gridDim.x - nb_prep);
 }
 
 template <int V>
@@ -2107,11 +2247,11 @@
 {
     Geom g;
     if (!make_geom(g, B, Cin, H, W, Cout, kh, kw, sh, sw, ph, pw, dh, dw, dg)) return 0;
-    return base_workspace_bytes(g) + dense_workspace_bytes(g) + sweep_workspace_bytes(g);
-}
-
-int dcd_dcn_v2_forward(void *stream_, const float *input, const float *weight, const float *bias,
-                       const float *offset, const float *mask, float *output, int B, int Cin, int H, int W,
+    return base_workspace_bytes(g) + dense_workspace_bytes(g) + sweep_workspace_bytes(g) + tail_workspace_bytes(g);
+}
+
+static int dcn_forward(void *stream_, const float *input, const float *weight, const float *bias, const float *conv_out,
+                       float *offset, float *mask, float *output, int B, int Cin, int H, int W,
                        int Cout, int kh, int kw, int sh, int sw, int ph, int pw, int dh, int dw, int dg,
                        int precision, void *workspace, size_t workspace_bytes)
 {
@@ -2120,6 +2260,17 @@
     Geom g;
     if (!input || !weight || !bias || !offset || !mask || !output || !workspace) return DCD_ERR_BAD_ARG;
     if (!make_geom(g, B, Cin, H, W, Cout, kh, kw, sh, sw, ph, pw, dh, dw, dg)) return DCD_ERR_BAD_ARG;
+    const bool split_v4 = (g.HoWo & 3) == 0 && (((uintptr_t)conv_out | (uintptr_t)offset | (uintptr_t)mask) & 15) == 0;
+    bool split_done = conv_out == nullptr;
+    auto ensure_split = [&]() {
+        if (split_done) return;
+        split_done = true;
+        const int T = dg * g.KK;
+        const int64_t n = (int64_t)B * 3 * T * g.HoWo / (split_v4 ? 4 : 1);
+        const unsigned grid = (unsigned)((n + 255) / 256 < 8192 ? (n + 255) / 256 : 8192);
+        if (split_v4) hipLaunchKernelGGL(dcn_offset_mask_split<4>, dim3(grid), dim3(256), 0, stream, conv_out, offset, mask, B, T, (int64_t)g.HoWo);
+        else hipLaunchKernelGGL(dcn_offset_mask_split<1>, dim3(grid), dim3(256), 0, stream, conv_out, offset, mask, B, T, (int64_t)g.HoWo);
+    };
     if (precision != DCD_PREC_F32 && precision != DCD_PREC_BF16X3 && precision != DCD_PREC_BF16) return DCD_ERR_BAD_ARG;
     const bool split = precision != DCD_PREC_F32;
     const bool one = precision == DCD_PREC_BF16;
@@ -2127,6 +2278,7 @@
     if (workspace_bytes < nw * sizeof(float) * 2) return DCD_ERR_WORKSPACE;
     if (dense_ok(g, false)) {
         if (workspace_bytes < base_workspace_bytes(g) + dense_workspace_bytes(g)) return DCD_ERR_WORKSPACE;
+        ensure_split();
         dense_forward(stream, input, weight, bias, offset, mask, output, g, (float *)((char *)workspace + base_workspace_bytes(g)),
                       precision);
         return hipGetLastError() == hipSuccess ? DCD_OK : DCD_ERR_LAUNCH;
@@ -2177,12 +2329,24 @@
             const size_t n9 = (size_t)Cin * 9 * g.Cop;
             if (nwl <= nw && n9 <= nw && workspace_bytes >= 2 * nw * sizeof(float) + (size_t)nflag_words * 4) {
                 float *wf9 = wf + nw;
-                if (split)
-                    hipLaunchKernelGGL(dcn_prep_weights_tile_bf16, dim3((unsigned)((nwl + 255) / 256 < 2048 ? (nwl + 255) / 256 : 2048)),
-                                       dim3(256), 0, stream, weight, (unsigned short *)wf, g, nchunk, nz, (unsigned *)flags, nflag_words, wf9);
-                else
-                    hipLaunchKernelGGL(dcn_prep_weights_tile, dim3((unsigned)((nwl + 255) / 256 < 2048 ? (nwl + 255) / 256 : 2048)),
-                                       dim3(256), 0, stream, weight, wf, g, nchunk, nz, (unsigned *)flags, nflag_words, wf9);
+                const unsigned nb_prep = (unsigned)((nwl + 255) / 256 < 2048 ? (nwl + 255) / 256 : 2048);
+                if (split) {
+                    ensure_split();
+                    hipLaunchKernelGGL(dcn_prep_weights_tile_bf16, dim3(nb_prep), dim3(256), 0, stream, weight, (unsigned short *)wf, g,
+                                       nchunk, nz, (unsigned *)flags, nflag_words, wf9);
+                } else if (!split_done) {
+                    split_done = true;
+                    const int64_t n = (int64_t)B * 27 * g.HoWo / (split_v4 ? 4 : 1);
+                    const unsigned nb_split = (unsigned)((n + 255) / 256 < 8192 ? (n + 255) / 256 : 8192);
+                    if (split_v4)
+                        hipLaunchKernelGGL(dcn_prep_tile_split<4>, dim3(nb_prep + nb_split), dim3(256), 0, stream, weight, wf, g, nchunk, nz,
+                                           (unsigned *)flags, nflag_words, wf9, (int)nb_prep, conv_out, offset, mask);
+                    else
+                        hipLaunchKernelGGL(dcn_prep_tile_split<1>, dim3(nb_prep + nb_split), dim3(256), 0, stream, weight, wf, g, nchunk, nz,
+                                           (unsigned *)flags, nflag_words, wf9, (int)nb_prep, conv_out, offset, mask);
+                } else
+                    hipLaunchKernelGGL(dcn_prep_weights_tile, dim3(nb_prep), dim3(256), 0, stream, weight, wf, g, nchunk, nz,
+                                       (unsigned *)flags, nflag_words, wf9);
                 if (!keeps) {
                     int gsz = (int)((ncoord + 4095) / 4096);
                     if (gsz > 512) gsz = 512;
@@ -2226,6 +2390,7 @@
 #ifndef DCN_NO_FWD9
     if (g.KK == 9 && W >= 2 && (size_t)Cin * 9 * g.Cop <= nw) {
         const size_t n9 = (size_t)Cin * 9 * g.Cop;
+        ensure_split();
         hipLaunchKernelGGL(dcn_prep_weights9, dim3((unsigned)((n9 + 255) / 256 < 2048 ? (n9 + 255) / 256 : 2048)), dim3(256), 0,
                            stream, weight, wf, g);
         const int mb9 = mb > 4 ? 4 : mb;
@@ -2238,6 +2403,7 @@
         return hipGetLastError() == hipSuccess ? DCD_OK : DCD_ERR_LAUNCH;
     }
 #endif
+    ensure_split();
     hipLaunchKernelGGL(dcn_prep_weights, dim3((unsigned)((nw + 255) / 256 < 2048 ? (nw + 255) / 256 : 2048)), dim3(256),
                        0, stream, weight, wf, wb, g);
     switch (mb) {
@@ -2249,19 +2415,38 @@
     return hipGetLastError() == hipSuccess ? DCD_OK : DCD_ERR_LAUNCH;
 }
 
-int dcd_dcn_v2_backward(void *stream_, const float *input, const float *weight, const float *bias,
-                        const float *offset, const float *mask, const float *grad_output, float *grad_input,
-                        float *grad_offset, float *grad_mask, float *grad_weight, float *grad_bias, int B,
-                        int Cin, int H, int W, int Cout, int kh, int kw, int sh, int sw, int ph, int pw, int dh,
-                        int dw, int dg, int precision, void *workspace, size_t workspace_bytes)
-{
-    (void)bias;
+int dcd_dcn_v2_forward(void *stream, const float *input, const float *weight, const float *bias,
+                       const float *offset, const float *mask, float *output, int B, int Cin, int H, int W,
+                       int Cout, int kh, int kw, int sh, int sw, int ph, int pw, int dh, int dw, int dg,
+                       int precision, void *workspace, size_t workspace_bytes)
+{
+    return dcn_forward(stream, input, weight, bias, nullptr, const_cast<float *>(offset), const_cast<float *>(mask), output, B, Cin, H, W,
+                       Cout, kh, kw, sh, sw, ph, pw, dh, dw, dg, precision, workspace, workspace_bytes);
+}
+
+int dcd_dcn_v2_forward_conv(void *stream, const float *input, const float *weight, const float *bias, const float *conv_out,
+                            float *offset, float *mask, float *output, int B, int Cin, int H, int W,
+                            int Cout, int kh, int kw, int sh, int sw, int ph, int pw, int dh, int dw, int dg,
+                            int precision, void *workspace, size_t workspace_bytes)
+{
+    if (!conv_out) return DCD_ERR_BAD_ARG;
+    return dcn_forward(stream, input, weight, bias, conv_out, offset, mask, output, B, Cin, H, W, Cout, kh, kw, sh, sw, ph, pw, dh, dw,
+                       dg, precision, workspace, workspace_bytes);
+}
+
+static int dcn_backward(void *stream_, const float *input, const float *weight, const float *offset, const float *mask,
+                        const float *grad_output, float *grad_input, float *grad_offset, float *grad_mask, float *grad_weight,
+                        float *grad_bias, float *grad_conv, float *grad_conv_bias, int B, int Cin, int H, int W, int Cout, int kh, int kw,
+                        int sh, int sw, int ph, int pw, int dh, int dw, int dg, int precision, void *workspace, size_t workspace_bytes)
+{
     hipStream_t stream = (hipStream_t)stream_;
     (void)hipGetLastError();
     Geom g;
-    if (!input || !weight || !offset || !mask || !grad_output || !grad_input || !grad_offset || !grad_mask ||
-        !grad_weight || !grad_bias || !workspace)
+    const bool merged = grad_conv != nullptr;
+    float *const grad_mask_out = merged ? grad_mask : nullptr;
+    if (!input || !weight || !offset || !mask || !grad_output || !grad_input || !grad_weight || !grad_bias || !workspace)
         return DCD_ERR_BAD_ARG;
+    if (merged ? !grad_conv_bias : (!grad_offset || !grad_mask)) return DCD_ERR_BAD_ARG;
     if (!make_geom(g, B, Cin, H, W, Cout, kh, kw, sh, sw, ph, pw, dh, dw, dg)) return DCD_ERR_BAD_ARG;
     if (precision != DCD_PREC_F32 && precision != DCD_PREC_BF16X3 && precision != DCD_PREC_BF16) return DCD_ERR_BAD_ARG;
     const bool split = precision != DCD_PREC_F32;
@@ -2290,6 +2475,42 @@
     inv.flag_ty = (H + 3) / 4;
     const dim3 bm_grid(((g.Ho + 7) / 8) * ((g.Wo + 7) / 8), dg * g.KK, B);
 
+    TailArgs ta;
+    unsigned *tail_arrivals = nullptr;
+    unsigned tail_words = 0;
+    if (merged) {
+        char *tws = (char *)workspace + base_workspace_bytes(g) + dense_workspace_bytes(g) + sweep_workspace_bytes(g);
+        const int T = dg * g.KK;
+        grad_offset = (float *)(tws + tail_head_bytes(g));
+        if (!grad_mask) grad_mask = grad_offset + (size_t)B * 2 * T * g.HoWo;
+        ta.gmsk_out = nullptr;
+        ta.planes = nullptr; ta.goff = grad_offset; ta.gmsk = grad_mask; ta.mask = mask; ta.gout = grad_conv;
+        ta.partial = (double *)tws; ta.sums = grad_conv_bias; ta.plane_stride = 0; ta.nplane = 1;
+        ta.B = B; ta.T = T; ta.HW = g.HoWo;
+        ta.cpp = (g.HoWo + TAIL_CH - 1) / TAIL_CH;
+        long want = (4096 + 3 * T - 1) / (3 * T);
+        if (want > TAIL_SMAX) want = TAIL_SMAX;
+        if (want > (long)B * ta.cpp) want = (long)B * ta.cpp;
+        ta.S = (int)(want < 1 ? 1 : want);
+        ta.arrivals = nullptr;
+        if ((long)ta.S * 3 * T <= 256) {
+            ta.arrivals = tail_arrivals = (unsigned *)(tws + (size_t)3 * T * TAIL_SMAX * sizeof(double));
+            tail_words = (unsigned)(3 * T);
+        }
+        ta.vec = (g.HoWo & 3) == 0 && (((uintptr_t)mask | (uintptr_t)grad_conv | (uintptr_t)grad_offset | (uintptr_t)grad_mask) & 15) == 0;
+    }
+    auto launch_combine = [&]() {
+        if (!ta.arrivals)
+            hipLaunchKernelGGL(dcn_offset_tail_combine, dim3(3 * ta.T), dim3(64), 0, stream, (const double *)ta.partial, ta.S, ta.sums);
+    };
+    auto finish = [&]() -> int {
+        if (merged) {
+            hipLaunchKernelGGL(dcn_offset_tail, dim3(3 * ta.T * ta.S), dim3(TAIL_BT), 0, stream, ta);
+            launch_combine();
+        }
+        return hipGetLastError() == hipSuccess ? DCD_OK : DCD_ERR_LAUNCH;
+    };
+
     const char *sw_e = dcd_env("DCD_SWEEP_WIDE");
     const bool sweep_wide = !(sw_e && atoi(sw_e) == 0);
     const bool use_sweep = sweep_ok(g) && (g.Cop <= 64 || (sweep_wide && (g.Cop <= 128 || !dense_ok(g, true)))) && dense_mode() != 1 &&
@@ -2303,6 +2524,7 @@
         z.p[0] = absmax; z.n[0] = 4;
         z.p[1] = (unsigned *)far_flag; z.n[1] = (unsigned)((ntile + 3) / 4);
         z.p[3] = (unsigned *)grad_bias; z.n[3] = (unsigned)Cout;
+        z.p[2] = tail_arrivals; z.n[2] = tail_words;
         hipLaunchKernelGGL(dcn_zero_ranges, dim3(8), dim3(256), 0, stream, z);
         hipLaunchKernelGGL(dcn_prep_weights, dim3((unsigned)((nw + 255) / 256 < 2048 ? (nw + 255) / 256 : 2048)), dim3(256),
                            0, stream, weight, wf, wb, g);
@@ -2319,7 +2541,7 @@
         hipLaunchKernelGGL(dcn_bias_grad, dim3(Cout, splits), dim3(256), 0, stream, grad_output, grad_bias, B, Cout, g.HoWo);
         dense_backward(stream, input, wb, offset, mask, grad_output, grad_input, grad_offset, grad_mask, grad_weight, g, inv,
                        (float *)((char *)workspace + base_workspace_bytes(g)), precision);
-        return hipGetLastError() == hipSuccess ? DCD_OK : DCD_ERR_LAUNCH;
+        return finish();
     }
     const int tiles = (g.HoWo + 31) / 32;
     const int nblk = g.cpgp / 32;
@@ -2349,6 +2571,7 @@
             z.p[2] = (unsigned *)grad_weight; z.n[2] = (unsigned)((size_t)Cout * Cin * g.KK);
             z.p[3] = (unsigned *)grad_bias; z.n[3] = (unsigned)Cout;
             z.p[4] = (unsigned *)grad_input; z.n[4] = (unsigned)((size_t)B * Cin * H * W);
+            z.p[5] = tail_arrivals; z.n[5] = tail_words;
             const int nb_zero = (int)(z.n[4] / 1024 + 1 < 4096 ? z.n[4] / 1024 + 1 : 4096);
             const int64_t noff = (int64_t)B * 18 * g.HoWo;
             int nb_scan = (int)((noff + 4095) / 4096);
@@ -2390,6 +2613,14 @@
             e.bias_only_if_far = sp.nob == 1 ? fs : (const unsigned *)nullptr;
             const int64_t n4 = (int64_t)B * 27 * g.HoWo / 4;
             e.nb_coord = (int)((n4 + 255) / 256 < 4096 ? (n4 + 255) / 256 : 4096);
+            if (merged && !handover) {
+                e.merged = 1;
+                e.tail = ta;
+                e.tail.planes = cpart; e.tail.plane_stride = (size_t)B * 27 * g.HoWo; e.tail.nplane = sp.nck;
+                e.tail.gmsk_out = grad_mask_out;
+                e.tail.vec = ta.vec && ((uintptr_t)cpart & 15) == 0;
+                e.nb_coord = 27 * ta.S;
+            }
             int splits = (int)(((int64_t)g.HoWo + 4095) / 4096);
             if (splits > 32) splits = 32;
             if (splits < 1) splits = 1;
@@ -2420,7 +2651,10 @@
             }
             hipLaunchKernelGGL(dcn_sweep_epilogue, dim3(e.nb_coord + Cout * splits + nb_dw), dim3(256), 0, stream, e);
         }
-        if (!handover) return hipGetLastError() == hipSuccess ? DCD_OK : DCD_ERR_LAUNCH;
+        if (!handover) {
+            if (merged) launch_combine();
+            return hipGetLastError() == hipSuccess ? DCD_OK : DCD_ERR_LAUNCH;
+        }
         inv.packed = 0;
         inv.tileflag = nullptr;
         hipLaunchKernelGGL(dcn_offset_blockmax, bm_grid, dim3(64), 0, stream, offset, g, blockmax, fs);
@@ -2467,7 +2701,7 @@
             else DCD_LAUNCH_BW_FAR(1);
 #undef DCD_LAUNCH_BW_FAR
         }
-        return hipGetLastError() == hipSuccess ? DCD_OK : DCD_ERR_LAUNCH;
+        return finish();
     }
     int nsplit = 1;
     while ((int64_t)tiles * B * nsplit < 1536 && nsplit * 2 <= nblk) nsplit *= 2;
@@ -2492,6 +2726,7 @@
             z.p[5] = (unsigned *)grad_mask; z.n[5] = (unsigned)((size_t)B * dg * g.KK * g.HoWo);
         }
         z.p[6] = (unsigned *)tileflag; z.n[6] = (unsigned)(tileflag_bytes(g) / 4);
+        z.p[7] = tail_arrivals; z.n[7] = tail_words;
         const size_t most = (size_t)z.n[2] > (size_t)z.n[4] ? z.n[2] : z.n[4];
         hipLaunchKernelGGL(dcn_zero_ranges, dim3((unsigned)(most / 1024 + 1 < 2048 ? most / 1024 + 1 : 2048)), dim3(256), 0, stream, z);
     }
@@ -2653,7 +2888,32 @@
         else DCD_LAUNCH_BW(1);
 #undef DCD_LAUNCH_BW
     }
-    return hipGetLastError() == hipSuccess ? DCD_OK : DCD_ERR_LAUNCH;
+    return finish();
+}
+
+int dcd_dcn_v2_backward(void *stream, const float *input, const float *weight, const float *bias,
+                        const float *offset, const float *mask, const float *grad_output, float *grad_input,
+                        float *grad_offset, float *grad_mask, float *grad_weight, float *grad_bias, int B,
+                        int Cin, int H, int W, int Cout, int kh, int kw, int sh, int sw, int ph, int pw, int dh,
+                        int dw, int dg, int precision, void *workspace, size_t workspace_bytes)
+{
+    (void)bias;
+    if (!grad_offset || !grad_mask) return DCD_ERR_BAD_ARG;
+    return dcn_backward(stream, input, weight, offset, mask, grad_output, grad_input, grad_offset, grad_mask, grad_weight, grad_bias,
+                        nullptr, nullptr, B, Cin, H, W, Cout, kh, kw, sh, sw, ph, pw, dh, dw, dg, precision, workspace, workspace_bytes);
+}
+
+int dcd_dcn_v2_backward_merged(void *stream, const float *input, const float *weight, const float *bias,
+                               const float *offset, const float *mask, const float *grad_output, float *grad_input,
+                               float *grad_conv, float *grad_conv_bias, float *grad_mask, float *grad_weight, float *grad_bias, int B,
+                               int Cin, int H, int W, int Cout, int kh, int kw, int sh, int sw, int ph, int pw, int dh,
+                               int dw, int dg, int precision, void *workspace, size_t workspace_bytes)
+{
+    (void)bias;
+    if (!grad_conv || !grad_conv_bias) return DCD_ERR_BAD_ARG;
+    return dcn_backward(stream, input, weight, offset, mask, grad_output, grad_input, nullptr, grad_mask, grad_weight, grad_bias,
+                        grad_conv, grad_conv_bias, B, Cin, H, W, Cout, kh, kw, sh, sw, ph, pw, dh, dw, dg, precision, workspace,
+                        workspace_bytes);
 }
 
 #ifdef SW_PROFILE
diff --git a/dcd_amd/model/backbone/DCNv2/dcn_v2.py b/dcd_amd/model/backbone/DCNv2/dcn_v2.py
--- a/dcd_amd/model/backbone/DCNv2/dcn_v2.py
+++ b/dcd_amd/model/backbone/DCNv2/dcn_v2.py
@@ -89,25 +89,26 @@
         p = _precision_scope()
         ctx.precision = {} if p == "f32" else {"precision": p}
         out = ops._conv3x3_forward(ctx, input, w_off, b_off.contiguous())
-        offset, mask = _offset_mask_split(out)
         ctx.geometry = geometry
+        B, C3, H, W = out.shape
+        offset = torch.empty((B, C3 // 3 * 2, H, W), dtype=out.dtype, device=out.device)
+        mask = torch.empty((B, C3 // 3, H, W), dtype=out.dtype, device=out.device)
+        output = _backend.dcn_v2_forward(input, weight, bias, offset, mask, *geometry, out, **ctx.precision)
         ctx.save_for_backward(input, offset, mask, weight, bias, w_off)
-        return _backend.dcn_v2_forward(input, weight, bias, offset, mask, *geometry, **ctx.precision)
+        return output
 
     @staticmethod
     @once_differentiable
     def backward(ctx, grad_output):
         from dcd_amd import ops
         input, offset, mask, weight, bias, w_off = ctx.saved_tensors
-        grad_input, grad_offset, grad_mask, grad_weight, grad_bias = _backend.dcn_v2_backward(
-            input, weight, bias, offset, mask, grad_output.contiguous(), *ctx.geometry, **ctx.precision)
-        gout = _offset_mask_merge(grad_offset, grad_mask, mask)
+        grad_input, _, _, grad_weight, grad_bias, gout, gb_off = _backend.dcn_v2_backward(
+            input, weight, bias, offset, mask, grad_output.contiguous(), *ctx.geometry, True, **ctx.precision)
         if ctx.needs_input_grad[0]:
             grad_input = ops._conv3x3_call(gout, w_off, w_off.shape[1], True, residual=grad_input.contiguous(), transformed=ctx.tw_back,
                                            prec=ctx.prec)
         gw_off = ops._conv3x3_wrw_call(input, gout, w_off.shape, ctx.prec) if ctx.needs_input_grad[1] else None
-        gb_off = ops.channel_sums(gout) if ctx.needs_input_grad[2] else None
-        return grad_input, gw_off, gb_off, grad_weight, grad_bias, None
+        return grad_input, gw_off, gb_off if ctx.needs_input_grad[2] else None, grad_weight, grad_bias, None
 
 
 def dcn_v2_conv(input, offset, mask, weight, bias, stride, padding, dilation, deformable_groups):
diff --git a/include/dcd_hip.h b/include/dcd_hip.h
--- a/include/dcd_hip.h
+++ b/include/dcd_hip.h
@@ -27,12 +27,23 @@
                        const float *offset, const float *mask, float *output, int B, int Cin, int H, int W,
                        int Cout, int kh, int kw, int sh, int sw, int ph, int pw, int dh, int dw, int dg,
                        int precision, void *workspace, size_t workspace_bytes);
+
+int dcd_dcn_v2_forward_conv(void *stream, const float *input, const float *weight, const float *bias, const float *conv_out,
+                            float *offset, float *mask, float *output, int B, int Cin, int H, int W,
+                            int Cout, int kh, int kw, int sh, int sw, int ph, int pw, int dh, int dw, int dg,
+                            int precision, void *workspace, size_t workspace_bytes);
 
 int dcd_dcn_v2_backward(void *stream, const float *input, const float *weight, const float *bias,
                         const float *offset, const float *mask, const float *grad_output, float *grad_input,
                         float *grad_offset, float *grad_mask, float *grad_weight, float *grad_bias, int B,
                         int Cin, int H, int W, int Cout, int kh, int kw, int sh, int sw, int ph, int pw, int dh,
                         int dw, int dg, int precision, void *workspace, size_t workspace_bytes);
+
+int dcd_dcn_v2_backward_merged(void *stream, const float *input, const float *weight, const float *bias,
+                               const float *offset, const float *mask, const float *grad_output, float *grad_input,
+                               float *grad_conv, float *grad_conv_bias, float *grad_mask, float *grad_weight, float *grad_bias, int B,
+                               int Cin, int H, int W, int Cout, int kh, int kw, int sh, int sw, int ph, int pw, int dh,
+                               int dw, int dg, int precision, void *workspace, size_t workspace_bytes);
 
 int dcd_dcn_v2_forget(const float *weight);
 int dcd_dcn_v2_policy_state(const float *weight, unsigned *far_count);
```

Measured after the change: 217.7 images/s (median of 2 runs). No clear change (+0.2%).
